# cg-saarland/hagrid

Measured on AMD Instinct MI355X. Metric: Mrays/s (primary traversal) + grid build ms, 1M-tri scene @1/2/4/8 MI355X, higher is better.
Workload: dtype f32

## Files before the change

hagrid_amd/csrc/build.hip:

```cpp
#include "ctx.h"
#include "wave_prims.h"

#include "hagrid/grid.h"
#include "hagrid/prims.h"

#include <cstring>
#include <vector>

using namespace hagrid;
using namespace hagrid_impl;

namespace {

struct BuildK {
    ivec3 dims;
    int shift;
    vec3 bmin, bmax;
    vec3 cell_size;
};

__device__ __forceinline__ Tri load_tri(const float4* __restrict__ tris, int i) {
    const float4* p = tris + 3 * size_t(i);
    const float4 a = p[0], b = p[1], c = p[2];
    return Tri(vec3(a.x, a.y, a.z), a.w, vec3(b.x, b.y, b.z), b.w, vec3(c.x, c.y, c.z), c.w);
}
__device__ __forceinline__ void store_cell(Cell* cells, int i, ivec3 lo, int begin, ivec3 hi, int end) {
    int4* p = reinterpret_cast<int4*>(cells) + 2 * size_t(i);
    p[0] = make_int4(lo.x, lo.y, lo.z, begin);
    p[1] = make_int4(hi.x, hi.y, hi.z, end);
}
__device__ __forceinline__ ivec3 load_cell_min(const Cell* cells, int i) {
    const int4 a = reinterpret_cast<const int4*>(cells)[2 * size_t(i)];
    return ivec3(a.x, a.y, a.z);
}
__device__ __forceinline__ BBox cell_world_box(const BuildK& k, ivec3 lo, ivec3 hi) {
    return BBox(k.bmin + vec3(lo) * k.cell_size, k.bmin + vec3(hi) * k.cell_size);
}

__global__ void __launch_bounds__(kBlock) bbox_partials(const float4* __restrict__ tris, int n, float* __restrict__ partials) {
    __shared__ float lds[kWaves][6];
    float lo[3] = { FLT_MAX, FLT_MAX, FLT_MAX }, hi[3] = { -FLT_MAX, -FLT_MAX, -FLT_MAX };
    for (int i = blockIdx.x * kBlock + threadIdx.x; i < n; i += gridDim.x * kBlock) {
        const BBox b = load_tri(tris, i).bbox();
        lo[0] = min(lo[0], b.min.x); lo[1] = min(lo[1], b.min.y); lo[2] = min(lo[2], b.min.z);
        hi[0] = max(hi[0], b.max.x); hi[1] = max(hi[1], b.max.y); hi[2] = max(hi[2], b.max.z);
    }
#pragma unroll
    for (int c = 0; c < 3; c++) { lo[c] = wave_min_f(lo[c]); hi[c] = wave_max_f(hi[c]); }
    if (lane_id() == 0) for (int c = 0; c < 3; c++) { lds[wave_id()][c] = lo[c]; lds[wave_id()][3 + c] = hi[c]; }
    __syncthreads();
    if (threadIdx.x < 6) {
        float v = lds[0][threadIdx.x];
        for (int w = 1; w < kWaves; w++) v = threadIdx.x < 3 ? min(v, lds[w][threadIdx.x]) : max(v, lds[w][threadIdx.x]);
        partials[blockIdx.x * 6 + threadIdx.x] = v;
    }
}
__global__ void __launch_bounds__(kBlock) bbox_final(const float* __restrict__ partials, int num, float* __restrict__ out) {
    __shared__ float lds[kWaves][6];
    float v[6] = { FLT_MAX, FLT_MAX, FLT_MAX, -FLT_MAX, -FLT_MAX, -FLT_MAX };
    for (int i = threadIdx.x; i < num; i += kBlock)
        for (int c = 0; c < 6; c++) v[c] = c < 3 ? min(v[c], partials[i * 6 + c]) : max(v[c], partials[i * 6 + c]);
#pragma unroll
    for (int c = 0; c < 6; c++) v[c] = c < 3 ? wave_min_f(v[c]) : wave_max_f(v[c]);
    if (lane_id() == 0) for (int c = 0; c < 6; c++) lds[wave_id()][c] = v[c];
    __syncthreads();
    if (threadIdx.x < 6) {
        float r = lds[0][threadIdx.x];
        for (int w = 1; w < kWaves; w++) r = threadIdx.x < 3 ? min(r, lds[w][threadIdx.x]) : max(r, lds[w][threadIdx.x]);
        out[threadIdx.x] = r;
    }
}

constexpr int kCoopCells = 64;


__global__ void __launch_bounds__(kBlock) top_log_dims(const int* __restrict__ refs_per_cell, int num_top, BuildK k, float snd_density,
                                                       int* __restrict__ log_dims, int* __restrict__ max_out) {
    __shared__ int lds[kWaves];
    const int i = blockIdx.x * kBlock + threadIdx.x;
    int ld = 0;
    if (i < num_top) {
        const vec3 ext = BBox(k.bmin, k.bmax).extents() / vec3(k.dims);
        const ivec3 d = compute_grid_dims(BBox(vec3(0, 0, 0), ext), refs_per_cell[i], snd_density);
        const int max_dim = max(d.x, max(d.y, d.z));
        ld = 31 - __clz(max_dim);
        ld = (1 << ld) < max_dim ? ld + 1 : ld;
        log_dims[i] = ld;
    }
    ld = wave_max(ld);
    if (lane_id() == 0) lds[wave_id()] = ld;
    __syncthreads();
    if (threadIdx.x == 0) {
        int m = lds[0];
        for (int w = 1; w < kWaves; w++) m = max(m, lds[w]);
        if (m > 0) atomicMax(max_out, m);
    }
}


__device__ __forceinline__ BuildK with_device_shift(BuildK k, const int* __restrict__ shift_dev, vec3 extents) {
    k.shift = *shift_dev;
    k.cell_size = extents / vec3(k.dims << k.shift);
    return k;
}

struct ChildCountIn {
    const uint32_t* entries;
    __device__ int operator()(int i) const { return (entries[i] & 3u) ? 8 : 0; }
    __device__ void load4(int i, int n, int* v) const {
        if (i + 4 <= n && lb_aligned16(entries + i)) {
            const uint4 e = *reinterpret_cast<const uint4*>(entries + i);
            v[0] = (e.x & 3u) ? 8 : 0; v[1] = (e.y & 3u) ? 8 : 0; v[2] = (e.z & 3u) ? 8 : 0; v[3] = (e.w & 3u) ? 8 : 0;
        } else {
            for (int c = 0; c < 4; c++) v[c] = i + c < n ? (*this)(i + c) : 0;
        }
    }
};
struct UpdateEntriesOut {
    uint32_t* entries;
    __device__ static uint32_t word(uint32_t e, int i, int start) { const uint32_t ld = e & 3u; return ld | (uint32_t(ld ? start : i) << 2); }
    __device__ void operator()(int i, int start) const { entries[i] = word(entries[i], i, start); }
    __device__ void store4(int i, int n, const int* v) const {
        if (i + 4 <= n && lb_aligned16(entries + i)) {
            uint4* p = reinterpret_cast<uint4*>(entries + i);
            const uint4 e = *p;
            *p = make_uint4(word(e.x, i, v[0]), word(e.y, i + 1, v[1]), word(e.z, i + 2, v[2]), word(e.w, i + 3, v[3]));
        } else {
            for (int c = 0; c < 4; c++) if (i + c < n) (*this)(i + c, v[c]);
        }
    }
};

__device__ __forceinline__ int split_mask(const BuildK& k, ivec3 lo, ivec3 hi, const Tri& tri) {
    const vec3 cmin = k.bmin + k.cell_size * vec3(lo);
    const vec3 cmax = k.bmin + k.cell_size * vec3(hi);
    const vec3 mid = (cmin + cmax) * 0.5f;
    int mask = 0xFF;
    const BBox rb = tri.bbox();
    if (rb.min.x > cmax.x || rb.max.x < cmin.x) mask = 0;
    if (rb.min.x > mid.x) mask &= 0xAA;
    if (rb.max.x < mid.x) mask &= 0x55;
    if (rb.min.y > cmax.y || rb.max.y < cmin.y) mask = 0;
    if (rb.min.y > mid.y) mask &= 0xCC;
    if (rb.max.y < mid.y) mask &= 0x33;
    if (rb.min.z > cmax.z || rb.max.z < cmin.z) mask = 0;
    if (rb.min.z > mid.z) mask &= 0xF0;
    if (rb.max.z < mid.z) mask &= 0x0F;
    int todo = mask;
    while (todo) {
        const int i = __ffs(todo) - 1;
        todo &= todo - 1;
        const BBox b(vec3(i & 1 ? mid.x : cmin.x, i & 2 ? mid.y : cmin.y, i & 4 ? mid.z : cmin.z),
                     vec3(i & 1 ? cmax.x : mid.x, i & 2 ? cmax.y : mid.y, i & 4 ? cmax.z : mid.z));
        if (!intersect_prim_cell(tri, b)) mask &= ~(1 << i);
    }
    return mask;
}


struct LeafIn {
    const uint32_t* entries; const int* cell_counts;
    __device__ static Int2 item(uint32_t e, int count) { const bool leaf = (e & 3u) == 0; return Int2{ leaf ? 1 : 0, leaf ? count : 0 }; }
    __device__ Int2 operator()(int i) const { return item(entries[i], cell_counts[i]); }
    __device__ void load4(int i, int n, Int2* v) const {
        if (i + 4 <= n && lb_aligned16(entries + i) && lb_aligned16(cell_counts + i)) {
            const uint4 e = *reinterpret_cast<const uint4*>(entries + i);
            const int4 c = *reinterpret_cast<const int4*>(cell_counts + i);
            v[0] = item(e.x, c.x); v[1] = item(e.y, c.y); v[2] = item(e.z, c.z); v[3] = item(e.w, c.w);
        } else {
            for (int k = 0; k < 4; k++) v[k] = i + k < n ? (*this)(i + k) : Int2{0, 0};
        }
    }
};
struct LeafOut {
    int* start_cell; int* ref_begin;
    __device__ void operator()(int i, Int2 v) const { start_cell[i] = v.a; ref_begin[i] = v.b; }
    __device__ void store4(int i, int n, const Int2* v) const {
        if (i + 4 <= n && lb_aligned16(start_cell + i) && lb_aligned16(ref_begin + i)) {
            *reinterpret_cast<int4*>(start_cell + i) = make_int4(v[0].a, v[1].a, v[2].a, v[3].a);
            *reinterpret_cast<int4*>(ref_begin + i) = make_int4(v[0].b, v[1].b, v[2].b, v[3].b);
        } else {
            for (int k = 0; k < 4; k++) if (i + k < n) (*this)(i + k, v[k]);
        }
    }
};


#ifndef HG_TILE_REFS
#define HG_TILE_REFS 1024
#endif
#ifndef HG_CHUNK_CELLS
#define HG_CHUNK_CELLS 256
#endif
#ifndef HG_EMIT_CHUNK
#define HG_EMIT_CHUNK 256
#endif
#ifndef HG_STAGE
#define HG_STAGE 1024
#endif
constexpr int kTileRefs = HG_TILE_REFS;
constexpr int kChunkCells = HG_CHUNK_CELLS;
constexpr int kEmitChunk = HG_EMIT_CHUNK;
constexpr int kStage = HG_STAGE;

__device__ __forceinline__ void mark_tiles(int* __restrict__ tile_first, int i, int start, int count) {
    for (int t = start / kTileRefs + 1; t <= (start + count) / kTileRefs; t++) tile_first[t] = i + 1;
}
struct SegIn {
    const int* counts;
    __device__ int operator()(int i) const { return counts[i]; }
};
struct SegOut {
    const int* counts; int* seg_begin; int* tile_first;
    Cell* cells; uint32_t* entries; int* cell_counts; const int* log_dims; const int* shift_dev; ivec3 dims;
    __device__ void operator()(int i, int start) const {
        seg_begin[i] = start; mark_tiles(tile_first, i, start, counts[i]);
        const int shift = *shift_dev;
        entries[i] = 0u; cell_counts[i] = 0;
        const int x = i % dims.x, y = (i / dims.x) % dims.y, z = i / (dims.x * dims.y);
        const ivec3 lo(x << shift, y << shift, z << shift);
        store_cell(cells, i, lo, log_dims[i], lo + ivec3(1 << shift), 0);
    }
};
struct ChildSegIn {
    const int* counts; const uint32_t* entries;
    __device__ Int2 operator()(int i) const { return Int2{counts[i], (entries[i] & 3u) ? 8 : 0}; }
    __device__ void load4(int i, int n, Int2* v) const {
        if (i + 4 <= n && lb_aligned16(counts + i) && lb_aligned16(entries + i)) {
            const int4 c = *reinterpret_cast<const int4*>(counts + i);
            const uint4 e = *reinterpret_cast<const uint4*>(entries + i);
            v[0] = Int2{c.x, (e.x & 3u) ? 8 : 0}; v[1] = Int2{c.y, (e.y & 3u) ? 8 : 0}; v[2] = Int2{c.z, (e.z & 3u) ? 8 : 0}; v[3] = Int2{c.w, (e.w & 3u) ? 8 : 0};
        } else {
            for (int k = 0; k < 4; k++) v[k] = i + k < n ? (*this)(i + k) : Int2{0, 0};
        }
    }
};
struct ChildSegOut {
    const int* counts; uint32_t* entries; int* seg_begin; int* tile_first;
    __device__ void operator()(int i, Int2 v) const {
        seg_begin[i] = v.a;
        entries[i] = UpdateEntriesOut::word(entries[i], i, v.b);
        mark_tiles(tile_first, i, v.a, counts[i]);
    }
    __device__ void store4(int i, int n, const Int2* v) const {
        if (i + 4 <= n && lb_aligned16(counts + i) && lb_aligned16(entries + i) && lb_aligned16(seg_begin + i)) {
            const int4 c = *reinterpret_cast<const int4*>(counts + i);
            uint4* pe = reinterpret_cast<uint4*>(entries + i);
            const uint4 e = *pe;
            *reinterpret_cast<int4*>(seg_begin + i) = make_int4(v[0].a, v[1].a, v[2].a, v[3].a);
            *pe = make_uint4(UpdateEntriesOut::word(e.x, i, v[0].b), UpdateEntriesOut::word(e.y, i + 1, v[1].b), UpdateEntriesOut::word(e.z, i + 2, v[2].b), UpdateEntriesOut::word(e.w, i + 3, v[3].b));
            if (v[0].a / kTileRefs != (v[3].a + c.w) / kTileRefs) {
                mark_tiles(tile_first, i, v[0].a, c.x); mark_tiles(tile_first, i + 1, v[1].a, c.y); mark_tiles(tile_first, i + 2, v[2].a, c.z); mark_tiles(tile_first, i + 3, v[3].a, c.w);
            }
        } else {
            for (int k = 0; k < 4; k++) if (i + k < n) (*this)(i + k, v[k]);
        }
    }
};

__global__ void __launch_bounds__(kBlock) top_range_sizes(const float4* __restrict__ tris, int n, BuildK k, int* __restrict__ counts, int* __restrict__ big_list, int* __restrict__ big_count) {
    const int i = blockIdx.x * kBlock + threadIdx.x;
    int size = 0;
    if (i < n) { size = max(0, compute_range(k.dims, BBox(k.bmin, k.bmax), load_tri(tris, i).bbox()).size()); counts[i] = size; }
    const bool big = size >= kCoopCells;
    const int at = wave_append(big ? 1 : 0, big_count);
    if (big) big_list[at] = i;
}
__device__ __forceinline__ int wave_shared_increment(int* __restrict__ counters, int index, bool active) {
    int rank = 0;
    unsigned long long todo = __ballot(active);
    const unsigned long long below = (1ull << lane_id()) - 1ull;
    for (int round = 0; todo && round < 16; round++) {
        const int leader = __ffsll((long long)todo) - 1;
        const int c = __shfl(index, leader, 64);
        const unsigned long long same = __ballot(active && index == c) & todo;
        if (round == 0 && (same & (same - 1)) == 0ull) break;
        int base = 0;
        if (lane_id() == leader) base = atomicAdd(counters + c, __popcll(same));
        base = __shfl(base, leader, 64);
        if ((same >> lane_id()) & 1ull) rank = base + __popcll(same & below);
        todo &= ~same;
    }
    if ((todo >> lane_id()) & 1ull) rank = atomicAdd(counters + index, 1);
    return rank;
}

__global__ void __launch_bounds__(kBlock) count_top_refs(const float4* __restrict__ tris, int n, BuildK k, const int* __restrict__ start_emit,
                                                                int* __restrict__ refs_per_cell, int* __restrict__ pair_rank,
                                                                const int* __restrict__ big_list, const int* __restrict__ big_count, int first_big_block) {
    if (int(blockIdx.x) >= first_big_block) {
        const int nb = *big_count;
        for (int b = int(blockIdx.x) - first_big_block; b < nb; b += int(gridDim.x) - first_big_block) {
            const int prim = big_list[b];
            const Range r = compute_range(k.dims, BBox(k.bmin, k.bmax), load_tri(tris, prim).bbox());
            const int total = r.size(), first = start_emit[prim], sx = r.hx - r.lx + 1, sy = r.hy - r.ly + 1;
            for (int c = threadIdx.x; c < total; c += kBlock) {
                const int x = r.lx + c % sx, y = r.ly + (c / sx) % sy, z = r.lz + c / (sx * sy);
                pair_rank[first + c] = atomicAdd(refs_per_cell + (x + k.dims.x * (y + k.dims.y * z)), 1);
            }
        }
        return;
    }
    const int i = blockIdx.x * kBlock + threadIdx.x;
    Range r(0, 0, 0, -1, -1, -1);
    int size = 0, start = 0;
    if (i < n) {
        r = compute_range(k.dims, BBox(k.bmin, k.bmax), load_tri(tris, i).bbox());
        size = max(0, r.size());
        start = start_emit[i];
    }
    const bool coop = size >= kCoopCells;
    {
        const bool mine = size > 0 && !coop;
        const int c0 = mine ? r.lx + k.dims.x * (r.ly + k.dims.y * r.lz) : -1 - lane_id();
        const unsigned long long any = __ballot(mine);
        const bool crowd = any != 0ull && __popcll(__ballot(c0 == __shfl(c0, __ffsll((long long)any) - 1, 64))) >= 2;
        if (!crowd) {
            if (mine) {
                int cur = start;
                for (int z = r.lz; z <= r.hz; z++)
                    for (int y = r.ly; y <= r.hy; y++)
                        for (int x = r.lx; x <= r.hx; x++) pair_rank[cur++] = atomicAdd(refs_per_cell + (x + k.dims.x * (y + k.dims.y * z)), 1);
            }
        } else {
            const int rounds = wave_max(mine ? size : 0);
            int x = r.lx, y = r.ly, z = r.lz;
            for (int j = 0; j < rounds; j++) {
                const bool act = mine && j < size;
                const int rank = wave_shared_increment(refs_per_cell, act ? x + k.dims.x * (y + k.dims.y * z) : 0, act);
                if (act) pair_rank[start + j] = rank;
                if (++x > r.hx) { x = r.lx; if (++y > r.hy) { y = r.ly; z++; } }
            }
        }
    }
}
__device__ __forceinline__ void place_top_ref(const BuildK& k, const Tri& tri, int prim, int x, int y, int z, int rank, const int* __restrict__ seg_begin,
                                              int2* __restrict__ refs, const int* __restrict__ log_dims, uint32_t* __restrict__ entries) {
    const int inc = 1 << k.shift;
    const ivec3 lo(x << k.shift, y << k.shift, z << k.shift);
    const bool hit = intersect_prim_cell(tri, cell_world_box(k, lo, lo + ivec3(inc)));
    const int cell = x + k.dims.x * (y + k.dims.y * z);
    refs[seg_begin[cell] + rank] = make_int2(hit ? prim : -1, cell);
    if (hit && log_dims[cell] > 0) entries[cell] = 1u;
}
__global__ void __launch_bounds__(kBlock) emit_top_refs(const float4* __restrict__ tris, int n, BuildK k0, const int* __restrict__ shift_dev, vec3 extents,
                                                                const int* __restrict__ start_emit,
                                                                const int* __restrict__ pair_rank, const int* __restrict__ seg_begin, int2* __restrict__ refs,
                                                                const int* __restrict__ log_dims, uint32_t* __restrict__ entries,
                                                                const int* __restrict__ big_list, const int* __restrict__ big_count, int first_big_block) {
    const BuildK k = with_device_shift(k0, shift_dev, extents);
    if (int(blockIdx.x) >= first_big_block) {
        const int nb = *big_count;
        for (int b = int(blockIdx.x) - first_big_block; b < nb; b += int(gridDim.x) - first_big_block) {
            const int prim = big_list[b];
            const Tri t = load_tri(tris, prim);
            const Range r = compute_range(k.dims, BBox(k.bmin, k.bmax), t.bbox());
            const int total = r.size(), first = start_emit[prim], sx = r.hx - r.lx + 1, sy = r.hy - r.ly + 1;
            for (int c = threadIdx.x; c < total; c += kBlock)
                place_top_ref(k, t, prim, r.lx + c % sx, r.ly + (c / sx) % sy, r.lz + c / (sx * sy), pair_rank[first + c], seg_begin, refs, log_dims, entries);
        }
        return;
    }
    const int i = blockIdx.x * kBlock + threadIdx.x;
    Range r(0, 0, 0, -1, -1, -1);
    int size = 0, start = 0;
    Tri tri;
    if (i < n) {
        tri = load_tri(tris, i);
        r = compute_range(k.dims, BBox(k.bmin, k.bmax), tri.bbox());
        size = max(0, r.size());
        start = start_emit[i];
    }
    const bool coop = size >= kCoopCells;
    if (size > 0 && !coop) {
        int cur = start;
        for (int z = r.lz; z <= r.hz; z++)
            for (int y = r.ly; y <= r.hy; y++)
                for (int x = r.lx; x <= r.hx; x++) { place_top_ref(k, tri, i, x, y, z, pair_rank[cur], seg_begin, refs, log_dims, entries); cur++; }
    }
}

struct TileRange { int c0, c1; };
__device__ __forceinline__ TileRange tile_cells(const int* __restrict__ tile_first, int t, int num_tiles, int num_cells) {
    return TileRange{ t == 0 ? 0 : tile_first[t], t + 1 >= num_tiles ? num_cells : tile_first[t + 1] };
}
struct LaneRun { unsigned long long run; int first; bool head; };
__device__ __forceinline__ LaneRun lane_run(int cell) {
    const int l = lane_id();
    const int prev = __shfl_up(cell, 1, 64);
    LaneRun r;
    r.head = l == 0 || prev != cell;
    const unsigned long long heads = __ballot(r.head);
    const unsigned long long upto = heads & (~0ull >> (63 - l));
    r.first = 63 - __clzll((long long)upto);
    const unsigned long long above = l == 63 ? 0ull : heads >> (l + 1);
    const int next = above ? l + 1 + (__ffsll((long long)above) - 1) : 64;
    const unsigned long long below_next = next == 64 ? ~0ull : ((1ull << next) - 1ull);
    r.run = below_next & ~((1ull << r.first) - 1ull);
    return r;
}

#ifndef HG_CLASSIFY_WAVES
#define HG_CLASSIFY_WAVES 8
#endif
__global__ void __launch_bounds__(kBlock, HG_CLASSIFY_WAVES) classify_refs(const int2* __restrict__ refs, const int* __restrict__ seg_begin,
                                                           int num_cells, int num_refs, const int* __restrict__ tile_first, int num_tiles, int top,
                                                           const float4* __restrict__ tris, const Cell* __restrict__ cells, const uint32_t* __restrict__ entries, BuildK k,
                                                           unsigned char* __restrict__ masks, int* __restrict__ cell_counts,
                                                           Cell* __restrict__ new_cells, int* __restrict__ new_counts, uint32_t* __restrict__ new_entries, int* __restrict__ totals) {
    __shared__ int hist[kChunkCells * 9];
    __shared__ int lds[kWaves];
    int kept = 0;
    for (int t = xcd_block(blockIdx.x, gridDim.x); t < num_tiles; t += gridDim.x) {
        const TileRange tr = tile_cells(tile_first, t, num_tiles, num_cells);
        for (int cc = tr.c0; cc < tr.c1; cc += kChunkCells) {
            const int ce = min(cc + kChunkCells, tr.c1);
            const int r0 = seg_begin[cc], r1 = ce >= num_cells ? num_refs : seg_begin[ce];
            if (r0 == r1) continue;
            for (int j = threadIdx.x; j < (ce - cc) * 9; j += kBlock) hist[j] = 0;
            __syncthreads();
            for (int base = r0 + wave_id() * 64; base < r1; base += kBlock) {
                const int i = base + lane_id();
                int2 rc = make_int2(-1, 0x7fffffff);
                if (i < r1) rc = refs[i];
                const int ref = rc.x, c = rc.y;
                int m = 0;
                bool keeps = false;
                if (ref >= 0) {
                    const uint32_t e = entries[c];
                    if ((e & 3u) == 0) keeps = true;
                    else {
                        const int4* p = reinterpret_cast<const int4*>(cells) + 2 * size_t(c);
                        const int4 a = p[0], b = p[1];
                        m = split_mask(k, ivec3(a.x, a.y, a.z), ivec3(b.x, b.y, b.z), load_tri(tris, ref));
                    }
                }
                if (i < r1) masks[i] = (unsigned char)m;
                kept += keeps ? 1 : 0;
                const LaneRun run = lane_run(c);
                int* h = hist + (c - cc) * 9;
                const unsigned long long any = __ballot(m != 0);
                if (any) {
#pragma unroll
                    for (int child = 0; child < 8; child++) {
                        const unsigned long long with = __ballot((m >> child) & 1);
                        if (run.head && i < r1) { const int n = __popcll(with & run.run); if (n) atomicAdd(h + child, n); }
                    }
                }
                if (top) {
                    const unsigned long long with = __ballot(keeps);
                    if (run.head && i < r1) { const int n = __popcll(with & run.run); if (n) atomicAdd(h + 8, n); }
                }
            }
            __syncthreads();
            for (int j = threadIdx.x; j < (ce - cc) * 8; j += kBlock) {
                const int c = cc + (j >> 3), child = j & 7;
                const uint32_t e = entries[c];
                if (e & 3u) {
                    const int n = hist[(j >> 3) * 9 + child];
                    const int4* p = reinterpret_cast<const int4*>(cells) + 2 * size_t(c);
                    const int4 a = p[0], b = p[1];
                    const int inc = (b.x - a.x) >> 1;
                    const ivec3 lo(a.x + (child & 1) * inc, a.y + ((child >> 1) & 1) * inc, a.z + (child >> 2) * inc);
                    store_cell(new_cells, int(e >> 2) + child, lo, a.w - 1, lo + ivec3(inc), 0);
                    new_counts[(e >> 2) + child] = n;
                    new_entries[(e >> 2) + child] = (n > 0 && a.w > 1) ? 1u : 0u;
                } else if (top && child == 0) cell_counts[c] = hist[(j >> 3) * 9 + 8];
            }
            __syncthreads();
        }
    }
    kept = block_sum(kept, lds);
    if (threadIdx.x == 0 && kept) atomicAdd(totals, kept);
}

__global__ void __launch_bounds__(kBlock) emit_child_refs(const int2* __restrict__ refs, const int* __restrict__ seg_begin,
                                                                  int num_cells, int num_refs, const int* __restrict__ tile_first, int num_tiles,
                                                                  const unsigned char* __restrict__ masks, const uint32_t* __restrict__ entries,
                                                                  const int* __restrict__ new_seg_begin, int2* __restrict__ new_refs) {
    __shared__ int cursor[kEmitChunk * 8];
    __shared__ int2 stage[kStage];
    __shared__ int region[2];
    for (int t = blockIdx.x; t < num_tiles; t += gridDim.x) {
        const TileRange tr = tile_cells(tile_first, t, num_tiles, num_cells);
        for (int cc = tr.c0; cc < tr.c1; cc += kEmitChunk) {
            const int ce = min(cc + kEmitChunk, tr.c1);
            const int r0 = seg_begin[cc], r1 = ce >= num_cells ? num_refs : seg_begin[ce];
            if (r0 == r1) continue;
            if (threadIdx.x == 0) { region[0] = 0x7fffffff; region[1] = 0; }
            __syncthreads();
            int lo = 0x7fffffff;
            for (int j = threadIdx.x; j < (ce - cc) * 8; j += kBlock) {
                const uint32_t e = entries[cc + (j >> 3)];
                const int at = (e & 3u) ? new_seg_begin[(e >> 2) + (j & 7)] : 0x7fffffff;
                cursor[j] = at;
                lo = min(lo, at);
            }
            lo = -wave_max(-lo);
            if (lane_id() == 0 && lo != 0x7fffffff) atomicMin(&region[0], lo);
            __syncthreads();
            const int base = region[0];
            int hi = 0;
            for (int rb = r0 + wave_id() * 64; rb < r1; rb += kBlock) {
                const int i = rb + lane_id();
                int m = 0;
                int2 rc = make_int2(-1, 0x7fffffff);
                if (i < r1) { m = masks[i]; rc = refs[i]; }
                if (__ballot(m != 0) == 0ull) continue;
                const int c = rc.y;
                const int first_child = m ? int(entries[c] >> 2) : 0;
                const LaneRun run = lane_run(c);
                int* cur = cursor + (c - cc) * 8;
                const unsigned long long below = (1ull << lane_id()) - 1ull;
#pragma unroll
                for (int child = 0; child < 8; child++) {
                    const unsigned long long with = __ballot((m >> child) & 1);
                    if (!with) continue;
                    int at = 0;
                    if (run.head && i < r1) { const int n = __popcll(with & run.run); if (n) at = atomicAdd(cur + child, n); }
                    at = __shfl(at, run.first, 64);
                    if ((m >> child) & 1) {
                        const int slot = at + __popcll(with & run.run & below);
                        hi = max(hi, slot + 1);
                        const int2 v = make_int2(rc.x, first_child + child);
                        if (slot - base < kStage) stage[slot - base] = v;
                        else new_refs[slot] = v;
                    }
                }
            }
            hi = wave_max(hi);
            if (lane_id() == 0 && hi) atomicMax(&region[1], hi);
            __syncthreads();
            const int staged = min(region[1] - base, kStage);
            for (int q = threadIdx.x; q < staged; q += kBlock) new_refs[base + q] = stage[q];
            __syncthreads();
        }
    }
}

constexpr int kCoopListMin = 9, kCoopListMax = 1024;
__global__ void __launch_bounds__(kBlock) concat_level(const uint32_t* __restrict__ entries, const Cell* __restrict__ cells, const int* __restrict__ cell_counts,
                                                               const int* __restrict__ start_cell, const int* __restrict__ ref_begin, int num_cells, int level_off,
                                                               const int2* __restrict__ refs, const int* __restrict__ seg_begin, int num_refs, int top,
                                                               Cell* __restrict__ out_cells, uint32_t* __restrict__ out_entries, int* __restrict__ out_refs) {
    __shared__ int long_cells[kBlock];
    __shared__ int num_long;
    __shared__ int stage[kWaves][kCoopListMax];
    if (threadIdx.x == 0) num_long = 0;
    __syncthreads();
    const int i = blockIdx.x * kBlock + threadIdx.x;
    if (i < num_cells) {
        const uint32_t e = entries[i];
        if (e & 3u) out_entries[level_off + i] = (e & 3u) | (((e >> 2) + uint32_t(level_off + num_cells)) << 2);
        else {
            const int dst = start_cell[i], cnt = cell_counts[i], rb = ref_begin[i];
            const int4* p = reinterpret_cast<const int4*>(cells) + 2 * size_t(i);
            const int4 a = p[0], b = p[1];
            store_cell(out_cells, dst, ivec3(a.x, a.y, a.z), cnt ? rb : 0, ivec3(b.x, b.y, b.z), cnt ? rb + cnt : 0);
            out_entries[level_off + i] = uint32_t(dst) << 2;
            int* r = out_refs + rb;
            const int2* src = refs + seg_begin[i];
            if (cnt == 0) { }
            else if (!top && cnt <= 4) {
                const int big = 0x7fffffff;
                int v0 = src[0].x, v1 = cnt > 1 ? src[1].x : big, v2 = cnt > 2 ? src[2].x : big, v3 = cnt > 3 ? src[3].x : big;
                int t;
                if (v0 > v1) { t = v0; v0 = v1; v1 = t; }
                if (v2 > v3) { t = v2; v2 = v3; v3 = t; }
                if (v0 > v2) { t = v0; v0 = v2; v2 = t; }
                if (v1 > v3) { t = v1; v1 = v3; v3 = t; }
                if (v1 > v2) { t = v1; v1 = v2; v2 = t; }
                r[0] = v0;
                if (cnt > 1) r[1] = v1;
                if (cnt > 2) r[2] = v2;
                if (cnt > 3) r[3] = v3;
            } else if (cnt >= kCoopListMin && cnt <= kCoopListMax) {
                long_cells[atomicAdd(&num_long, 1)] = i;
            } else {
                int n = 0;
                if (top) { for (int j = 0; n < cnt; j++) { const int v = src[j].x; if (v >= 0) r[n++] = v; } }
                else for (; n < cnt; n++) r[n] = src[n].x;
                if (cnt > 24) {
                    const int gaps[8] = { 1750, 701, 301, 132, 57, 23, 10, 4 };
                    for (int g = 0; g < 8; g++) {
                        const int gap = gaps[g];
                        for (int x = gap; x < cnt; x++) {
                            const int v = r[x];
                            int y = x - gap;
                            while (y >= 0 && r[y] > v) { r[y + gap] = r[y]; y -= gap; }
                            r[y + gap] = v;
                        }
                    }
                }
                for (int x = 1; x < cnt; x++) {
                    const int v = r[x];
                    int y = x - 1;
                    while (y >= 0 && r[y] > v) { r[y + 1] = r[y]; y--; }
                    r[y + 1] = v;
                }
            }
        }
    }
    __syncthreads();
    const int nl = num_long, lane = lane_id();
    int* buf = stage[wave_id()];
    for (int q = wave_id(); q < nl; q += kWaves) {
        const int c = long_cells[q];
        const int cnt = cell_counts[c];
        int* r = out_refs + ref_begin[c];
        const int2* src = refs + seg_begin[c];
        if (top) {
            int found = 0;
            for (int base = 0; found < cnt; base += 64) {
                const int v = seg_begin[c] + base + lane < num_refs ? src[base + lane].x : -1;
                const unsigned long long ok = __ballot(v >= 0);
                const int at = found + __popcll(ok & ((1ull << lane) - 1ull));
                if (v >= 0 && at < cnt) buf[at] = v;
                found += __popcll(ok);
            }
        } else {
            for (int x = lane; x < cnt; x += 64) buf[x] = src[x].x;
        }
        __builtin_amdgcn_wave_barrier();
        for (int x = lane; x < cnt; x += 64) {
            const int v = buf[x];
            int rank = 0;
            for (int y = 0; y < cnt; y++) rank += buf[y] < v ? 1 : 0;
            r[rank] = v;
        }
        __builtin_amdgcn_wave_barrier();
    }
}

struct PlainIn { const int* v; __device__ int operator()(int i) const { return v[i]; } };
struct PlainOut { int* v; __device__ void operator()(int i, int s) const { v[i] = s; } };

using Temps = PoolTemps;

struct GLevel {
    int2* refs = nullptr; int num_refs = 0;
    Cell* cells = nullptr; uint32_t* entries = nullptr; int num_cells = 0;
    int* cell_counts = nullptr;
    int* seg_begin = nullptr;
    int* tile_first = nullptr; int num_tiles = 0;
    int* start_cell = nullptr; int* ref_begin = nullptr;
};

struct Arena {
    hagrid_ctx* ctx; Temps& tmp; char* base = nullptr; size_t size = 0, used = 0, wanted = 0; int num_tris;
    Arena(hagrid_ctx* c, Temps& t, int n_tris) : ctx(c), tmp(t), num_tris(n_tris) {
        size_t want = c->build_arena_hint;
        if (want && c->build_arena_tris > 0 && 2ll * n_tris < c->build_arena_tris)
            want = size_t(double(want) * 1.25 * double(std::max(n_tris, 1)) / double(c->build_arena_tris)) + 4096;
        if (want) {
            base = pool_try_alloc<char>(c, want);
            if (base) { t.ptrs.push_back(base); size = want; }
        }
    }
    ~Arena() { ctx->build_arena_hint = wanted; ctx->build_arena_tris = num_tris; }
    template <typename T> T* get(size_t n) {
        const size_t bytes = (std::max(n, size_t(1)) * sizeof(T) + 255) & ~size_t(255);
        wanted += bytes;
        if (base && used + bytes <= size) { T* p = reinterpret_cast<T*>(base + used); used += bytes; return p; }
        return tmp.get<T>(n);
    }
    void drop(void* p) { if (!base || p < base || p >= base + size) tmp.drop(p); }
};

int build_levels(hagrid_ctx* ctx, const float4* tris, int num_tris, hagrid_grid* grid, BuildK k, const BBox& gb, float snd_density, Temps& tmp) {
    hipStream_t st = ctx->stream;
    int* dsc = ctx->dscratch;
    Arena ar(ctx, tmp, num_tris);
    const ivec3 dims = k.dims;
    const int num_top = dims.x * dims.y * dims.z;

    int* counts = ar.get<int>(size_t(num_tris));
    int* start_emit = ar.get<int>(size_t(num_tris));
    int* refs_per_cell = ar.get<int>(size_t(num_top));
    int* log_dims = ar.get<int>(size_t(num_top));
    int* const partials = nullptr;
    if (!counts || !start_emit || !refs_per_cell || !log_dims) return HAGRID_ENOMEM;
    HG_HIP(ctx, hipMemsetAsync(refs_per_cell, 0, size_t(num_top) * sizeof(int), st));
    int* big_list = ar.get<int>(size_t(num_tris));
    if (!big_list) return HAGRID_ENOMEM;
    top_range_sizes<<<grid_blocks(num_tris, kBlock), kBlock, 0, st>>>(tris, num_tris, k, counts, big_list, dsc + 2); HG_DBG(ctx);
    if (!ctx_scan<int>(ctx, PlainIn{counts}, PlainOut{start_emit}, num_tris, partials, (const int*)nullptr, dsc + 0)) return HAGRID_ENOMEM;
    int R0 = 0, num_big = 0;
    {
        int h[3];
        HG_TRY(read_back(ctx, dsc, h, sizeof(h)));
        R0 = h[0]; num_big = h[2];
    }
    if (R0 < 0 || R0 > 0x3fffffff) HG_FAIL(ctx, HAGRID_ERANGE, "build_grid: too many top-level references");
    ar.drop(counts);
    int* pair_rank = ar.get<int>(size_t(R0) + 1);
    if (!pair_rank) return HAGRID_ENOMEM;
    const int prim_blocks = grid_blocks(num_tris, kBlock), big_blocks = std::min(num_big, 2048);
    count_top_refs<<<prim_blocks + big_blocks, kBlock, 0, st>>>(tris, num_tris, k, start_emit, refs_per_cell, pair_rank, big_list, dsc + 2, prim_blocks); HG_DBG(ctx);
    top_log_dims<<<grid_blocks(num_top, kBlock), kBlock, 0, st>>>(refs_per_cell, num_top, k, snd_density, log_dims, dsc + 1); HG_DBG(ctx);

    std::vector<GLevel> levels;
    GLevel L;
    L.num_refs = R0; L.num_cells = num_top;
    L.num_tiles = grid_blocks(R0, kTileRefs);
    L.refs = ar.get<int2>(size_t(R0) + 1);
    L.cells = ar.get<Cell>(size_t(num_top)); L.entries = ar.get<uint32_t>(size_t(num_top) + 1);
    L.cell_counts = ar.get<int>(size_t(num_top)); L.seg_begin = ar.get<int>(size_t(num_top) + 1);
    L.tile_first = ar.get<int>(size_t(L.num_tiles) + 2);
    L.start_cell = ar.get<int>(size_t(num_top)); L.ref_begin = ar.get<int>(size_t(num_top));
    if (!L.refs || !L.cells || !L.entries || !L.cell_counts || !L.seg_begin || !L.tile_first || !L.start_cell || !L.ref_begin) return HAGRID_ENOMEM;
    if (!ctx_scan<int>(ctx, SegIn{refs_per_cell}, SegOut{refs_per_cell, L.seg_begin, L.tile_first, L.cells, L.entries, L.cell_counts, log_dims, dsc + 1, dims}, num_top, partials,
                       (const int*)nullptr, (int*)nullptr)) return HAGRID_ENOMEM;
    hagrid_build_counts& bc = ctx->counts;
    memset(&bc, 0, sizeof(bc));
    bc.num_tris = num_tris; bc.top_cells = num_top; bc.top_refs = R0;
    emit_top_refs<<<prim_blocks + big_blocks, kBlock, 0, st>>>(tris, num_tris, k, dsc + 1, gb.extents(), start_emit, pair_rank, L.seg_begin, L.refs, log_dims, L.entries, big_list, dsc + 2, prim_blocks); HG_DBG(ctx);
    levels.push_back(L);

    {
        if (!ctx_scan<int>(ctx, ChildCountIn{L.entries}, UpdateEntriesOut{L.entries}, num_top, (int*)nullptr, (const int*)nullptr, dsc + 8)) return HAGRID_ENOMEM;
    }
    int num_new_cells = 0, shift = 0;
    {
        int h[8];
        HG_TRY(read_back(ctx, dsc + 1, h, sizeof(h)));
        shift = h[0]; num_new_cells = h[7];
    }
    if (shift >= 24) HG_FAIL(ctx, HAGRID_ERANGE, "build_grid: too many levels");
    k.shift = shift;
    k.cell_size = gb.extents() / vec3(dims << shift);
    ar.drop(start_emit); ar.drop(pair_rank); ar.drop(refs_per_cell);
    for (int level = 0;; level++) {
        GLevel& P = levels.back();
        int* tot = dsc + 8 + 4 * level;
        if (num_new_cells < 0) HG_FAIL(ctx, HAGRID_ERANGE, "build_grid: level too large");
        if ((int)levels.size() >= 24) HG_FAIL(ctx, HAGRID_ERANGE, "build_grid: too many levels");
        const bool last = num_new_cells == 0;
        if (last && level > 0) {
            if (level < HAGRID_MAX_LEVELS) { bc.level_refs[level] = P.num_refs; bc.level_cells[level] = P.num_cells; bc.level_kept[level] = P.num_refs; bc.num_levels = level + 1; }
            break;
        }
        GLevel N;
        N.num_cells = num_new_cells;
        unsigned char* masks = ar.get<unsigned char>(size_t(P.num_refs) + 1);
        if (!masks) return HAGRID_ENOMEM;
        if (!last) {
            N.cells = ar.get<Cell>(size_t(num_new_cells)); N.entries = ar.get<uint32_t>(size_t(num_new_cells) + 1);
            N.cell_counts = ar.get<int>(size_t(num_new_cells)); N.seg_begin = ar.get<int>(size_t(num_new_cells) + 1);
            N.tile_first = ar.get<int>(size_t(grid_blocks(8ll * P.num_refs, kTileRefs)) + 2);
            N.start_cell = ar.get<int>(size_t(num_new_cells)); N.ref_begin = ar.get<int>(size_t(num_new_cells));
            if (!N.cells || !N.entries || !N.cell_counts || !N.seg_begin || !N.tile_first || !N.start_cell || !N.ref_begin) return HAGRID_ENOMEM;
        }
        if (P.num_refs > 0) {
            classify_refs<<<std::min(P.num_tiles, 4096), kBlock, 0, st>>>(P.refs, P.seg_begin, P.num_cells, P.num_refs, P.tile_first, P.num_tiles, level == 0 ? 1 : 0,
                                                                             tris, P.cells, P.entries, k, masks, P.cell_counts, N.cells, N.cell_counts, N.entries, tot + 1); HG_DBG(ctx);
        }
        Int2* next = reinterpret_cast<Int2*>(tot + 2);
        if (!last) {
            if (!ctx_scan<Int2>(ctx, ChildSegIn{N.cell_counts, N.entries}, ChildSegOut{N.cell_counts, N.entries, N.seg_begin, N.tile_first}, num_new_cells, (Int2*)nullptr,
                                (const Int2*)nullptr, next)) return HAGRID_ENOMEM;
        }
        int h3[3] = {0, 0, 0};
        HG_TRY(read_back(ctx, tot + 1, h3, sizeof(h3)));
        if (level < HAGRID_MAX_LEVELS) { bc.level_refs[level] = P.num_refs; bc.level_cells[level] = P.num_cells; bc.level_kept[level] = h3[0]; bc.num_levels = level + 1; }
        if (last) { ar.drop(masks); break; }
        const int num_children = h3[1];
        if (num_children < 0 || num_children > 0x3fffffff) HG_FAIL(ctx, HAGRID_ERANGE, "build_grid: level too large");
        N.num_refs = num_children; N.num_tiles = grid_blocks(num_children, kTileRefs);
        N.refs = ar.get<int2>(size_t(num_children) + 1);
        if (!N.refs) return HAGRID_ENOMEM;
        if (P.num_refs > 0 && num_children > 0) {
            emit_child_refs<<<std::min(P.num_tiles, 4096), kBlock, 0, st>>>(P.refs, P.seg_begin, P.num_cells, P.num_refs, P.tile_first, P.num_tiles,
                                                                                   masks, P.entries, N.seg_begin, N.refs); HG_DBG(ctx);
        }
        ar.drop(masks);
        num_new_cells = h3[2];
        levels.push_back(N);
    }
    ar.drop(log_dims);

    const int num_levels = (int)levels.size();
    long long total_cells_ll = 0;
    int max_cells = 0;
    for (auto& V : levels) { total_cells_ll += V.num_cells; max_cells = std::max(max_cells, V.num_cells); }
    if (total_cells_ll > 0x3fffffff) HG_FAIL(ctx, HAGRID_ERANGE, "build_grid: too many voxel map entries");
    const int total_cells = int(total_cells_ll);
    Int2* const part2 = nullptr;
    Int2* carry = reinterpret_cast<Int2*>(dsc + 128);
    for (int l = 0; l < num_levels; l++) {
        GLevel& V = levels[l];
        if (!ctx_scan<Int2>(ctx, LeafIn{V.entries, V.cell_counts}, LeafOut{V.start_cell, V.ref_begin}, V.num_cells, part2,
                            l ? carry + (l - 1) : (const Int2*)nullptr, carry + l)) return HAGRID_ENOMEM;
    }
    int hf[2];
    HG_TRY(read_back(ctx, carry + (num_levels - 1), hf, sizeof(hf)));
    const int new_total_cells = hf[0], total_refs = hf[1];
    if (new_total_cells <= 0 || total_refs < 0) HG_FAIL(ctx, HAGRID_ERANGE, "build_grid: inconsistent totals");

    Cell* out_cells = pool_alloc<Cell>(ctx, size_t(new_total_cells));
    uint32_t* out_entries = pool_alloc<uint32_t>(ctx, size_t(total_cells));
    int* out_refs = pool_alloc<int>(ctx, size_t(total_refs));
    if (!out_cells || !out_entries || !out_refs) {
        hagrid_mem_free(ctx, out_cells); hagrid_mem_free(ctx, out_entries); hagrid_mem_free(ctx, out_refs);
        return HAGRID_ENOMEM;
    }
    for (int l = 0, off = 0; l < num_levels; off += levels[l].num_cells, l++) {
        GLevel& V = levels[l];
        concat_level<<<grid_blocks(V.num_cells, kBlock), kBlock, 0, st>>>(V.entries, V.cells, V.cell_counts, V.start_cell, V.ref_begin, V.num_cells, off,
                                                                                  V.refs, V.seg_begin, V.num_refs, l == 0 ? 1 : 0, out_cells, out_entries, out_refs); HG_DBG(ctx);
    }
    hipError_t e = hipGetLastError();
    if (e == hipSuccess) e = hipStreamSynchronize(st);
    if (e != hipSuccess) {
        hagrid_mem_free(ctx, out_cells); hagrid_mem_free(ctx, out_entries); hagrid_mem_free(ctx, out_refs);
        HG_FAIL(ctx, HAGRID_EHIP, hipGetErrorString(e));
    }
    memset(grid, 0, sizeof(*grid));
    grid->entries = out_entries; grid->ref_ids = out_refs; grid->cells = out_cells; grid->small_cells = nullptr;
    grid->bbox_min[0] = gb.min.x; grid->bbox_min[1] = gb.min.y; grid->bbox_min[2] = gb.min.z;
    grid->bbox_max[0] = gb.max.x; grid->bbox_max[1] = gb.max.y; grid->bbox_max[2] = gb.max.z;
    grid->dims[0] = dims.x; grid->dims[1] = dims.y; grid->dims[2] = dims.z;
    grid->num_cells = new_total_cells; grid->num_entries = total_cells; grid->num_refs = total_refs;
    bc.build_cells = new_total_cells; bc.build_entries = total_cells; bc.build_refs = total_refs;
    grid->shift = shift;
    grid->num_offsets = shift + 1;
    for (int i = 0, off = 0; i <= shift; i++) {
        if (i < num_levels) off += levels[i].num_cells;
        grid->offsets[i] = off;
    }
    return HAGRID_OK;
}

}

extern "C" int hagrid_build_grid(hagrid_ctx* ctx, const void* tris_v, int num_tris, hagrid_grid* grid,
                                 float top_density, float snd_density) {
    if (!ctx || !grid) return HAGRID_EINVAL;
    trav_image_drop(ctx);
    if (!tris_v || num_tris <= 0) HG_FAIL(ctx, HAGRID_EINVAL, "build_grid: no triangles");
    HG_HIP(ctx, hipSetDevice(ctx->device));
    const float4* tris = static_cast<const float4*>(tris_v);
    hipStream_t st = ctx->stream;
    Temps tmp(ctx);
    int* dsc = ctx->dscratch;
    HG_HIP(ctx, hipMemsetAsync(dsc, 0, 256 * sizeof(int), st));

    const int bb_blocks = std::min(grid_blocks(num_tris, kBlock), 1024);
    float* bb_part = tmp.get<float>(size_t(bb_blocks) * 6 + 8);
    if (!bb_part) return HAGRID_ENOMEM;
    float* bb_out = bb_part + size_t(bb_blocks) * 6;
    bbox_partials<<<bb_blocks, kBlock, 0, st>>>(tris, num_tris, bb_part); HG_DBG(ctx);
    bbox_final<<<1, kBlock, 0, st>>>(bb_part, bb_blocks, bb_out); HG_DBG(ctx);
    float hb[6];
    HG_TRY(read_back(ctx, bb_out, hb, sizeof(hb)));
    BBox gb(vec3(hb[0], hb[1], hb[2]), vec3(hb[3], hb[4], hb[5]));
    ivec3 dims = compute_grid_dims(gb, num_tris, top_density);
    dims.x += dims.x & 1; dims.y += dims.y & 1; dims.z += dims.z & 1;
    const vec3 ext = gb.extents();
    gb.min -= ext * 0.001f;
    gb.max += ext * 0.001f;
    const long long num_top_ll = (long long)dims.x * dims.y * dims.z;
    if (num_top_ll > 0x3fffffff) HG_FAIL(ctx, HAGRID_ERANGE, "build_grid: top-level grid too large");

    BuildK k;
    k.dims = dims; k.shift = 0; k.bmin = gb.min; k.bmax = gb.max; k.cell_size = vec3(0.0f);

    return build_levels(ctx, tris, num_tris, grid, k, gb, snd_density, tmp);
}
```

hagrid_amd/csrc/ctx.h:

```cpp
#pragma once

#include <hip/hip_runtime.h>

#include <atomic>
#include <cstdio>
#include <memory>
#include <string>
#include <unordered_map>
#include <vector>

#include "hagrid_amd.h"

namespace hagrid_impl {

struct Slot {
    void* ptr = nullptr;
    size_t size = 0;
    bool in_use = false;
    int refs = 0;
};

}

namespace hagrid_impl {

struct TravImageCache {
    void* table = nullptr;
    size_t table_bytes = 0;
    int wide_records = 0;
    void* blocks = nullptr;
    size_t block_bytes = 0;
    bool valid = false;
    bool uniform = false;
    bool general = false;
    int slim = 0;
    int vtop_k = 0;
    uint32_t vtop_base = 0;
    bool detached = false;
    bool borrowed = false;
    std::shared_ptr<std::atomic<bool>> alive;
    const void* entries = nullptr; const void* cells = nullptr; const void* refs = nullptr;
    int num_cells = 0, num_entries = 0, num_refs = 0, shift = 0, dims[3] = {0, 0, 0}, cell_bytes = 32;
    int max_ref = -1;
    void* alt_blocks = nullptr; void* alt_table = nullptr; size_t alt_block_bytes = 0, alt_table_bytes = 0; int alt_wide_records = 0, alt_slim = 0;
};

}

namespace hagrid_impl {
enum MailboxWord : int {
    kMbxRowLen = 300,
    kMbxOrderStale = 304,
    kMbxReadBackEpoch = 310,
    kMbxHeadSuggest = 312,
    kMbxPriorStats = 316,
};
enum ScratchWord : int {
    kScrRowLenBinned = 232,
    kScrRowLen = 236,
    kScrMaxRef = 240,
    kScrBlobFlag = 250,
};
}

struct hagrid_ctx {
    int device = 0;
    hipStream_t stream = nullptr;
    bool keep = false;
    int num_cus = 0;

    std::vector<hagrid_impl::Slot> slots;
    std::unordered_map<void*, int> tracker;
    size_t usage = 0, max_usage = 0;

    hipEvent_t ev_begin = nullptr, ev_end = nullptr;

    int* mailbox = nullptr;
    int* dscratch = nullptr;
    unsigned long long* lb_state = nullptr;
    size_t lb_words = 0;
    unsigned lb_epoch = 0;
    int* row_scores = nullptr;
    int* bin_diff = nullptr;

    int ray_binning = 0;
    int opt_variant = 0;
    int opt_lookback = 1;
    int opt_merge_inplace = 1;
    int opt_merge_inplace_iters = 0;
    int opt_merge_inplace_div = 0;
    int opt_merge_inplace_room = 0;
    int opt_merge_narrow = 1;
    int opt_expand_voxel_map = 1;
    int opt_expand_subset_only = 1;
    int opt_image_width = 0;
    int opt_band_rows = 0;
    int opt_super_log2 = 3;
    int opt_xcd_chunk_log2 = -2;
    int opt_narrow = 1;
    int opt_image_max_mb = 0;
    int opt_quad_head = 20;
    int opt_image_vtop = 1;
    int opt_image_uniform = 1;
    int opt_row_cache = 1;
    struct RayHints {
        const void* key_rays = nullptr; int key_n = 0;
        const void* rowlen_rays = nullptr; int rowlen_n = 0, rowlen_age = 0, rowlen_known = -1, rowlen_seen = 0; bool rows_from_origins = false ;
        hipEvent_t rowlen_evt = nullptr; bool rowlen_pending = false;
        int* lpt_buf = nullptr; int lpt_cap = 0; const void* lpt_rays = nullptr; int lpt_n = 0, lpt_blocks = 0, lpt_age = 0, lpt_period = 32, lpt_rot = 0 ; bool rot_adopted = false ;
        hipEvent_t trial_evt[2] = {nullptr, nullptr}; bool trial_pending = false, trial_with_head = false, head_disabled = false;
        float t_base = 0.0f, t_head = 0.0f; int n_base = 0, n_head = 0, trial_opt = -1 ; unsigned head_serial = 0 ; bool lpt_valid = false;
        int lpt_epoch = 1 , relearn_streak = 0, cooldown = 0, cooldown_len = 64; unsigned long long relearn_clock = 0;
        hipEvent_t share_evt[12][2] = {}; int share_issued = 0, share_done = 0, share_choice = -1 , share_ncand = 0 , share_shape_nc = 0 , share_cands[4] = {0, 0, 0, 0} ,
            share_last = -1 , share_launches = 0; float share_t[4] = {0.0f, 0.0f, 0.0f, 0.0f}; unsigned share_serial = 0 ;
        int trial_kind = 0 , n_all = 0, all_stage = 0 ; float t_all = 0.0f; bool learned_all = false;
        bool learned_once = false;
        unsigned order_serial = 0;
        bool cmp_pending = false, cmp_done = false; int n_conf = 0; float t_conf = 0.0f;
        bool order_loses = false;
        int last_report = -1;
        unsigned long long used = 0;
    };
    static constexpr int kRayHints = 4;
    RayHints hints[kRayHints];
    unsigned long long hint_clock = 0;
    int opt_mailbox = -1;
    int opt_tail = 1;
    int opt_lds_pad = 0;
    int opt_tail_dual = -1;
    int opt_share_trial = 1;
    int opt_order_gate = 1;
    int opt_tile_order = -1;
    int opt_quad_tail = -1;
    int opt_image_slim = 1;
    int opt_image_general = 1;
    int opt_image = 2;

    int opt_id_is_steps = 0;

    hagrid_impl::TravImageCache image;
    unsigned image_serial = 0;
    int readback_epoch = 0;
    int opt_fast_readback = 1;
    int build_arena_tris = 0;
    size_t build_arena_hint = 0;
    hagrid_build_counts counts = {};

    std::string err;
};

namespace hagrid_impl {

inline int fail(hagrid_ctx* ctx, int code, const char* file, int line, const char* msg) {
    if (ctx) {
        char buf[512];
        snprintf(buf, sizeof(buf), "%s(%d): %s", file, line, msg);
        ctx->err = buf;
    }
    return code;
}

#define HG_FAIL(ctx, code, msg) return ::hagrid_impl::fail((ctx), (code), __FILE__, __LINE__, (msg))
#define HG_HIP(ctx, call)                                                                         \
    do {                                                                                          \
        hipError_t e_ = (call);                                                                   \
        if (e_ != hipSuccess) return ::hagrid_impl::fail((ctx), HAGRID_EHIP, __FILE__, __LINE__, hipGetErrorString(e_)); \
    } while (0)
#define HG_TRY(expr)                                                                              \
    do {                                                                                          \
        int rc_ = (expr);                                                                         \
        if (rc_ < 0) return rc_;                                                                  \
    } while (0)

void debug_sync(hagrid_ctx* ctx, const char* file, int line);
#ifdef HAGRID_DEBUG_SYNC
#define HG_DBG(ctx) ::hagrid_impl::debug_sync((ctx), __FILE__, __LINE__)
#else
#define HG_DBG(ctx) do { } while (0)
#endif

template <typename T>
inline T* pool_alloc(hagrid_ctx* ctx, size_t n) {
    return static_cast<T*>(hagrid_mem_alloc(ctx, (n ? n : 1) * sizeof(T)));
}

template <typename T>
inline T* pool_try_alloc(hagrid_ctx* ctx, size_t n) {
    const std::string saved = ctx->err;
    T* p = pool_alloc<T>(ctx, n);
    if (!p) { (void)hipGetLastError(); ctx->err = saved; }
    return p;
}

struct PoolTemps {
    hagrid_ctx* ctx;
    std::vector<void*> ptrs;
    explicit PoolTemps(hagrid_ctx* c) : ctx(c) {}
    PoolTemps(const PoolTemps&) = delete;
    PoolTemps& operator=(const PoolTemps&) = delete;
    template <typename T> T* get(size_t n) { T* p = pool_alloc<T>(ctx, n); if (p) ptrs.push_back(p); return p; }
    void drop(void* p) { for (auto& q : ptrs) if (q == p && p) { hagrid_mem_free(ctx, p); q = nullptr; } }
    void* keep(void* p) { for (auto& q : ptrs) if (q == p) q = nullptr; return p; }
    ~PoolTemps() { for (void* p : ptrs) if (p) hagrid_mem_free(ctx, p); }
};

int pool_split(hagrid_ctx* ctx, void* base, void* const* parts, int n);

int read_back(hagrid_ctx* ctx, const void* dptr, void* hptr, size_t bytes);

inline int grid_blocks(long long n, int block) { return (int)((n + block - 1) / block); }

unsigned long long* lookback_state(hagrid_ctx* ctx, int tiles, int words_per_tile, unsigned* epoch);

int trav_image_build(hagrid_ctx* ctx, const hagrid_grid* grid);
void trav_image_drop(hagrid_ctx* ctx);
bool trav_image_matches(const hagrid_ctx* ctx, const hagrid_grid* grid);
bool trav_image_stale(const hagrid_ctx* ctx);
void trav_image_source_touched(hagrid_ctx* ctx, const void* ptr, size_t bytes);

}
```

hagrid_amd/csrc/ctx.hip:

```cpp
#include "ctx.h"

#include <chrono>

#include <algorithm>
#include <cstring>
#include <iostream>

using namespace hagrid_impl;

extern "C" int hagrid_abi_version(void) { return HAGRID_ABI_VERSION; }

extern "C" int hagrid_ctx_create(hagrid_ctx** out, int device, int keep) {
    if (!out) return HAGRID_EINVAL;
    *out = nullptr;
    int count = 0;
    if (hipGetDeviceCount(&count) != hipSuccess || count <= 0 || device < 0 || device >= count) return HAGRID_ENODEV;
    hagrid_ctx* ctx = new hagrid_ctx();
    ctx->device = device;
    ctx->keep = keep != 0;
    if (hipSetDevice(device) != hipSuccess) { delete ctx; return HAGRID_ENODEV; }
    hipDeviceProp_t prop;
    if (hipGetDeviceProperties(&prop, device) != hipSuccess) { delete ctx; return HAGRID_ENODEV; }
    ctx->num_cus = prop.multiProcessorCount;
    if (hipEventCreate(&ctx->ev_begin) != hipSuccess || hipEventCreate(&ctx->ev_end) != hipSuccess ||
        hipHostMalloc((void**)&ctx->mailbox, 320 * sizeof(int), hipHostMallocDefault) != hipSuccess ||
        hipMalloc((void**)&ctx->dscratch, 256 * sizeof(int)) != hipSuccess) {
        hagrid_ctx_destroy(ctx);
        return HAGRID_EHIP;
    }
    memset(ctx->mailbox, 0, 320 * sizeof(int));
    *out = ctx;
    return HAGRID_OK;
}

extern "C" void hagrid_ctx_destroy(hagrid_ctx* ctx) {
    if (!ctx) return;
    (void)hipSetDevice(ctx->device);
    (void)hipStreamSynchronize(ctx->stream);
    for (auto& h : ctx->hints) h.rowlen_pending = false;
    if (!ctx->image.borrowed && ctx->image.alive) ctx->image.alive->store(false);
    for (auto& s : ctx->slots)
        if (s.ptr) (void)hipFree(s.ptr);
    if (ctx->ev_begin) (void)hipEventDestroy(ctx->ev_begin);
    if (ctx->ev_end) (void)hipEventDestroy(ctx->ev_end);
    for (auto& h : ctx->hints) { if (h.rowlen_evt) (void)hipEventDestroy(h.rowlen_evt); if (h.lpt_buf) (void)hipFree(h.lpt_buf); for (auto& e : h.trial_evt) if (e) (void)hipEventDestroy(e); for (auto& pr : h.share_evt) for (auto& e : pr) if (e) (void)hipEventDestroy(e); }
    if (ctx->mailbox) (void)hipHostFree(ctx->mailbox);
    if (ctx->dscratch) (void)hipFree(ctx->dscratch);
    if (ctx->bin_diff) (void)hipFree(ctx->bin_diff);
    if (ctx->row_scores) (void)hipFree(ctx->row_scores);
    if (ctx->lb_state) (void)hipFree(ctx->lb_state);
    delete ctx;
}

extern "C" int hagrid_ctx_set_stream(hagrid_ctx* ctx, void* stream) {
    if (!ctx) return HAGRID_EINVAL;
    hipStream_t next = static_cast<hipStream_t>(stream);
    if (next == ctx->stream) return HAGRID_OK;
    HG_HIP(ctx, hipSetDevice(ctx->device));
    HG_HIP(ctx, hipStreamSynchronize(ctx->stream));
    ctx->stream = next;
    return HAGRID_OK;
}

extern "C" int hagrid_ctx_synchronize(hagrid_ctx* ctx) {
    if (!ctx) return HAGRID_EINVAL;
    HG_HIP(ctx, hipSetDevice(ctx->device));
    HG_HIP(ctx, hipStreamSynchronize(ctx->stream));
    return HAGRID_OK;
}

extern "C" int hagrid_get_build_counts(const hagrid_ctx* ctx, hagrid_build_counts* out) {
    if (!ctx || !out) return HAGRID_EINVAL;
    *out = ctx->counts;
    return HAGRID_OK;
}

extern "C" const char* hagrid_last_error(const hagrid_ctx* ctx) { return ctx ? ctx->err.c_str() : "no context"; }

extern "C" int hagrid_device_info(const hagrid_ctx* ctx, char* name, int name_len, int* compute_units, int64_t* total_mem) {
    if (!ctx) return HAGRID_EINVAL;
    hipDeviceProp_t prop;
    if (hipGetDeviceProperties(&prop, ctx->device) != hipSuccess) return HAGRID_EHIP;
    if (name && name_len > 0) { strncpy(name, prop.gcnArchName, (size_t)name_len - 1); name[name_len - 1] = 0; }
    if (compute_units) *compute_units = prop.multiProcessorCount;
    if (total_mem) *total_mem = (int64_t)prop.totalGlobalMem;
    return HAGRID_OK;
}


static void release_slot_memory(hagrid_ctx* ctx, Slot& s) {
    if (s.ptr) (void)hipFree(s.ptr);
    ctx->usage -= s.size;
    s.ptr = nullptr;
    s.size = 0;
}

extern "C" void* hagrid_mem_alloc(hagrid_ctx* ctx, size_t bytes) {
    if (!ctx) return nullptr;
    if (bytes == 0) bytes = 4;
    bytes = (bytes + 255) & ~size_t(255);
    int fit = -1, biggest = -1, empty = -1;
    for (int i = 0, n = (int)ctx->slots.size(); i < n; i++) {
        const Slot& s = ctx->slots[i];
        if (s.in_use) continue;
        if (!s.ptr) { if (empty < 0) empty = i; continue; }
        if (s.size >= bytes && (fit < 0 || s.size < ctx->slots[fit].size)) fit = i;
        if (biggest < 0 || s.size > ctx->slots[biggest].size) biggest = i;
    }
    int idx = fit;
    if (idx >= 0 && ctx->slots[idx].size > 4 * bytes && ctx->slots[idx].size > (size_t(64) << 20)) idx = -1;
    if (idx < 0) {
        idx = fit < 0 ? (biggest >= 0 && ctx->keep ? biggest : empty) : empty;
        if (idx < 0) { idx = (int)ctx->slots.size(); ctx->slots.emplace_back(); }
        Slot& s = ctx->slots[idx];
        if (s.ptr) release_slot_memory(ctx, s);
        void* p = nullptr;
        (void)hipSetDevice(ctx->device);
        if (hipMalloc(&p, bytes) != hipSuccess) {
            for (auto& t : ctx->slots) if (!t.in_use && t.ptr) release_slot_memory(ctx, t);
            if (hipMalloc(&p, bytes) != hipSuccess) { fail(ctx, HAGRID_ENOMEM, __FILE__, __LINE__, "hipMalloc failed"); return nullptr; }
        }
        s.ptr = p; s.size = bytes;
        ctx->usage += bytes;
        ctx->max_usage = std::max(ctx->max_usage, ctx->usage);
    }
    Slot& s = ctx->slots[idx];
    s.in_use = true;
    s.refs = 1;
    ctx->tracker[s.ptr] = idx;
    return s.ptr;
}

int hagrid_impl::pool_split(hagrid_ctx* ctx, void* base, void* const* parts, int n) {
    auto it = ctx->tracker.find(base);
    if (it == ctx->tracker.end() || n <= 0) HG_FAIL(ctx, HAGRID_EINVAL, "pool_split: not a pool buffer");
    const int idx = it->second;
    Slot& s = ctx->slots[idx];
    if (s.refs != 1 || s.ptr != base) HG_FAIL(ctx, HAGRID_EINVAL, "pool_split: buffer is already split");
    for (int i = 0; i < n; i++) {
        const char* p = static_cast<const char*>(parts[i]);
        if (p < static_cast<const char*>(base) || p >= static_cast<const char*>(base) + s.size) HG_FAIL(ctx, HAGRID_EINVAL, "pool_split: part outside the buffer");
        for (int j = 0; j < i; j++) if (parts[j] == parts[i]) HG_FAIL(ctx, HAGRID_EINVAL, "pool_split: parts coincide");
    }
    ctx->tracker.erase(it);
    for (int i = 0; i < n; i++) ctx->tracker[parts[i]] = idx;
    s.refs = n;
    return HAGRID_OK;
}

extern "C" int hagrid_mem_free(hagrid_ctx* ctx, void* ptr) {
    if (!ctx) return HAGRID_EINVAL;
    if (!ptr) return HAGRID_OK;
    auto it = ctx->tracker.find(ptr);
    if (it == ctx->tracker.end()) HG_FAIL(ctx, HAGRID_EINVAL, "free of a pointer that does not come from this MemManager");
    trav_image_source_touched(ctx, ptr, 1);
    it = ctx->tracker.find(ptr);
    Slot& s = ctx->slots[it->second];
    ctx->tracker.erase(it);
    if (--s.refs > 0) return HAGRID_OK;
    s.in_use = false;
    if (!ctx->keep) {
        HG_HIP(ctx, hipStreamSynchronize(ctx->stream));
        release_slot_memory(ctx, s);
    }
    return HAGRID_OK;
}

extern "C" int hagrid_mem_copy_h2d(hagrid_ctx* ctx, void* dst, const void* src, size_t bytes) {
    if (!ctx) return HAGRID_EINVAL;
    if (!bytes) return HAGRID_OK;
    trav_image_source_touched(ctx, dst, bytes);
    HG_HIP(ctx, hipSetDevice(ctx->device));
    HG_HIP(ctx, hipMemcpyAsync(dst, src, bytes, hipMemcpyHostToDevice, ctx->stream));
    HG_HIP(ctx, hipStreamSynchronize(ctx->stream));
    return HAGRID_OK;
}
extern "C" int hagrid_mem_copy_d2h(hagrid_ctx* ctx, void* dst, const void* src, size_t bytes) {
    if (!ctx) return HAGRID_EINVAL;
    if (!bytes) return HAGRID_OK;
    HG_HIP(ctx, hipSetDevice(ctx->device));
    HG_HIP(ctx, hipMemcpyAsync(dst, src, bytes, hipMemcpyDeviceToHost, ctx->stream));
    HG_HIP(ctx, hipStreamSynchronize(ctx->stream));
    return HAGRID_OK;
}
extern "C" int hagrid_mem_copy_d2d(hagrid_ctx* ctx, void* dst, const void* src, size_t bytes) {
    if (!ctx) return HAGRID_EINVAL;
    if (!bytes) return HAGRID_OK;
    trav_image_source_touched(ctx, dst, bytes);
    HG_HIP(ctx, hipSetDevice(ctx->device));
    HG_HIP(ctx, hipMemcpyAsync(dst, src, bytes, hipMemcpyDeviceToDevice, ctx->stream));
    return HAGRID_OK;
}
extern "C" int hagrid_mem_zero(hagrid_ctx* ctx, void* ptr, size_t bytes) {
    if (!ctx) return HAGRID_EINVAL;
    if (!bytes) return HAGRID_OK;
    trav_image_source_touched(ctx, ptr, bytes);
    HG_HIP(ctx, hipSetDevice(ctx->device));
    HG_HIP(ctx, hipMemsetAsync(ptr, 0, bytes, ctx->stream));
    return HAGRID_OK;
}
extern "C" int hagrid_mem_one(hagrid_ctx* ctx, void* ptr, size_t bytes) {
    if (!ctx) return HAGRID_EINVAL;
    if (!bytes) return HAGRID_OK;
    trav_image_source_touched(ctx, ptr, bytes);
    HG_HIP(ctx, hipSetDevice(ctx->device));
    HG_HIP(ctx, hipMemsetAsync(ptr, 0xFF, bytes, ctx->stream));
    return HAGRID_OK;
}
extern "C" size_t hagrid_mem_usage(const hagrid_ctx* ctx) { return ctx ? ctx->usage : 0; }
extern "C" size_t hagrid_mem_max_usage(const hagrid_ctx* ctx) { return ctx ? ctx->max_usage : 0; }

extern "C" void hagrid_mem_debug_slots(const hagrid_ctx* ctx) {
    if (!ctx) return;
    size_t total = 0;
    std::cout << "SLOTS: " << std::endl;
    for (const auto& s : ctx->slots) {
        std::cout << "[" << (s.in_use ? 'X' : ' ') << "] " << (double)s.size / (1024.0 * 1024.0) << "MB" << std::endl;
        total += s.size;
    }
    std::cout << (double)total / (1024.0 * 1024.0) << "MB total" << std::endl;
}


extern "C" int hagrid_profile_begin(hagrid_ctx* ctx) {
    if (!ctx) return HAGRID_EINVAL;
    HG_HIP(ctx, hipSetDevice(ctx->device));
    HG_HIP(ctx, hipEventRecord(ctx->ev_begin, ctx->stream));
    return HAGRID_OK;
}
extern "C" float hagrid_profile_end(hagrid_ctx* ctx) {
    if (!ctx) return -1.0f;
    float ms = -1.0f;
    if (hipEventRecord(ctx->ev_end, ctx->stream) != hipSuccess) return -1.0f;
    if (hipEventSynchronize(ctx->ev_end) != hipSuccess) return -1.0f;
    if (hipEventElapsedTime(&ms, ctx->ev_begin, ctx->ev_end) != hipSuccess) return -1.0f;
    return ms;
}

namespace {
typedef float f32x4_t __attribute__((ext_vector_type(4)));
__global__ void __launch_bounds__(256) bw_copy_kernel(const f32x4_t* __restrict__ a, f32x4_t* __restrict__ c, size_t n) {
    const size_t base = size_t(blockIdx.x) * 1024 + threadIdx.x;
    f32x4_t v[4];
#pragma unroll
    for (int j = 0; j < 4; j++) if (base + j * 256 < n) v[j] = __builtin_nontemporal_load(a + base + j * 256);
#pragma unroll
    for (int j = 0; j < 4; j++) if (base + j * 256 < n) __builtin_nontemporal_store(v[j], c + base + j * 256);
}
__global__ void __launch_bounds__(256) bw_triad_kernel(const f32x4_t* __restrict__ a, const f32x4_t* __restrict__ b, f32x4_t* __restrict__ c, size_t n) {
    const size_t base = size_t(blockIdx.x) * 1024 + threadIdx.x;
    f32x4_t v[4], w[4];
#pragma unroll
    for (int j = 0; j < 4; j++) if (base + j * 256 < n) { v[j] = __builtin_nontemporal_load(a + base + j * 256); w[j] = __builtin_nontemporal_load(b + base + j * 256); }
#pragma unroll
    for (int j = 0; j < 4; j++) if (base + j * 256 < n) __builtin_nontemporal_store(v[j] + 3.0f * w[j], c + base + j * 256);
}
}

extern "C" int hagrid_bandwidth_probe(hagrid_ctx* ctx, size_t bytes, int iters, float* copy_gbps, float* triad_gbps) {
    if (!ctx || iters <= 0 || bytes < (size_t(1) << 20)) return HAGRID_EINVAL;
    HG_HIP(ctx, hipSetDevice(ctx->device));
    const size_t n = bytes / 16;
    f32x4_t* a = pool_alloc<f32x4_t>(ctx, n);
    f32x4_t* b = pool_alloc<f32x4_t>(ctx, n);
    f32x4_t* c = pool_alloc<f32x4_t>(ctx, n);
    int rc = HAGRID_OK;
    if (!a || !b || !c) rc = HAGRID_ENOMEM;
    if (rc == HAGRID_OK) {
        (void)hipMemsetAsync(a, 0, n * 16, ctx->stream); (void)hipMemsetAsync(b, 0, n * 16, ctx->stream);
        const int blocks = int((n + 1023) / 1024);
        float best_copy = 0.0f, best_triad = 0.0f;
        for (int it = 0; it < iters + 1 && rc == HAGRID_OK; it++) {
            float ms = -1.0f;
            if (hagrid_profile_begin(ctx) != HAGRID_OK) { rc = HAGRID_EHIP; break; }
            bw_copy_kernel<<<blocks, 256, 0, ctx->stream>>>(a, c, n); HG_DBG(ctx);
            ms = hagrid_profile_end(ctx);
            if (ms > 0.0f && it) best_copy = std::max(best_copy, float(2.0 * double(n) * 16.0 / (double(ms) * 1e6)));
            if (hagrid_profile_begin(ctx) != HAGRID_OK) { rc = HAGRID_EHIP; break; }
            bw_triad_kernel<<<blocks, 256, 0, ctx->stream>>>(a, b, c, n); HG_DBG(ctx);
            ms = hagrid_profile_end(ctx);
            if (ms > 0.0f && it) best_triad = std::max(best_triad, float(3.0 * double(n) * 16.0 / (double(ms) * 1e6)));
        }
        if (copy_gbps) *copy_gbps = best_copy;
        if (triad_gbps) *triad_gbps = best_triad;
        if (hipGetLastError() != hipSuccess) rc = HAGRID_EHIP;
    }
    hagrid_mem_free(ctx, a); hagrid_mem_free(ctx, b); hagrid_mem_free(ctx, c);
    return rc;
}

unsigned long long* hagrid_impl::lookback_state(hagrid_ctx* ctx, int tiles, int words_per_tile, unsigned* epoch) {
    const size_t need = size_t(tiles > 0 ? tiles : 1) * size_t(words_per_tile);
    if (need > ctx->lb_words || ctx->lb_epoch >= (1u << 30) - 2u) {
        (void)hipStreamSynchronize(ctx->stream);
        if (need > ctx->lb_words) {
            if (ctx->lb_state) (void)hipFree(ctx->lb_state);
            ctx->lb_state = nullptr; ctx->lb_words = 0;
            const size_t words = need + need / 2 + 1024;
            if (hipMalloc((void**)&ctx->lb_state, words * sizeof(unsigned long long)) != hipSuccess) { (void)hipGetLastError(); return nullptr; }
            ctx->lb_words = words;
        }
        (void)hipMemsetAsync(ctx->lb_state, 0, ctx->lb_words * sizeof(unsigned long long), ctx->stream);
        ctx->lb_epoch = 0;
    }
    *epoch = ++ctx->lb_epoch;
    return ctx->lb_state;
}

void hagrid_impl::debug_sync(hagrid_ctx* ctx, const char* file, int line) {
    hipError_t e = hipStreamSynchronize(ctx->stream);
    if (e == hipSuccess) e = hipGetLastError();
    if (e != hipSuccess) {
        fprintf(stderr, "%s(%d): %s\n", file, line, hipGetErrorString(e));
        abort();
    }
}

extern "C" int hagrid_debug_sync_enabled(void) {
#ifdef HAGRID_DEBUG_SYNC
    return 1;
#else
    return 0;
#endif
}

namespace {
__global__ void __launch_bounds__(256) publish_words(const int* __restrict__ src, int n, int* dst, int* flag, int epoch) {
    if (int(threadIdx.x) < n) dst[threadIdx.x] = src[threadIdx.x];
    __threadfence_system();
    __syncthreads();
    if (threadIdx.x == 0) __hip_atomic_store(flag, epoch, __ATOMIC_RELEASE, __HIP_MEMORY_SCOPE_SYSTEM);
}
}

int hagrid_impl::read_back(hagrid_ctx* ctx, const void* dptr, void* hptr, size_t bytes) {
    if (ctx->opt_fast_readback && bytes > 0 && bytes <= 256 * sizeof(int) && (bytes & 3u) == 0 && (reinterpret_cast<uintptr_t>(dptr) & 3u) == 0) {
        int* flag = ctx->mailbox + kMbxReadBackEpoch;
        const int epoch = ++ctx->readback_epoch;
        publish_words<<<1, 256, 0, ctx->stream>>>(static_cast<const int*>(dptr), int(bytes / 4), ctx->mailbox, flag, epoch);
        HG_HIP(ctx, hipGetLastError());
        const auto t0 = std::chrono::steady_clock::now();
        for (unsigned spins = 0;; spins++) {
            if (__atomic_load_n(flag, __ATOMIC_ACQUIRE) == epoch) break;
            if ((spins & 1023u) == 1023u && std::chrono::steady_clock::now() - t0 > std::chrono::milliseconds(20)) {
                HG_HIP(ctx, hipStreamSynchronize(ctx->stream));
                if (__atomic_load_n(flag, __ATOMIC_ACQUIRE) != epoch) HG_FAIL(ctx, HAGRID_EHIP, "read_back: the words never arrived");
                break;
            }
        }
        memcpy(hptr, ctx->mailbox, bytes);
        return HAGRID_OK;
    }
    if (bytes <= 256 * sizeof(int)) {
        HG_HIP(ctx, hipMemcpyAsync(ctx->mailbox, dptr, bytes, hipMemcpyDeviceToHost, ctx->stream));
        HG_HIP(ctx, hipStreamSynchronize(ctx->stream));
        memcpy(hptr, ctx->mailbox, bytes);
    } else {
        HG_HIP(ctx, hipMemcpyAsync(hptr, dptr, bytes, hipMemcpyDeviceToHost, ctx->stream));
        HG_HIP(ctx, hipStreamSynchronize(ctx->stream));
    }
    return HAGRID_OK;
}
```

hagrid_amd/csrc/expand.hip:

```cpp
#include "ctx.h"
#include "wave_prims.h"

#include "hagrid/grid.h"
#include "hagrid/prims.h"

using namespace hagrid;
using namespace hagrid_impl;

namespace {

struct ExpandK { ivec3 dims; ivec3 top; int shift; vec3 gmin, cell_size, grid_inv; const int* voxel_cells; };
constexpr int kChanged = 1 << 3;
struct CellRec { ivec3 lo; int begin; ivec3 hi; int end; };

__device__ __forceinline__ CellRec load_cell(const Cell* cells, int i) {
    const int4* p = reinterpret_cast<const int4*>(cells) + 2 * size_t(i);
    const int4 a = p[0], b = p[1];
    CellRec c; c.lo = ivec3(a.x, a.y, a.z); c.begin = a.w; c.hi = ivec3(b.x, b.y, b.z); c.end = b.w;
    return c;
}
__device__ __forceinline__ int comp(const ivec3& v, int axis) { return axis == 0 ? v.x : (axis == 1 ? v.y : v.z); }


__device__ __forceinline__ int lower_bound_in(const int* __restrict__ a, int n, int x) {
    int lo = 0, hi = n;
    while (lo < hi) {
        const int mid = (lo + hi) >> 1;
        if (a[mid] < x) lo = mid + 1; else hi = mid;
    }
    return lo;
}

__device__ __forceinline__ bool contains_all(const int* __restrict__ big, int nbig, const int* __restrict__ small, int nsmall) {
    if (nsmall > nbig) return false;
    if (nsmall == 0) return true;
    if (nbig <= 4) {
        const int b0 = big[0], b1 = nbig > 1 ? big[1] : -1, b2 = nbig > 2 ? big[2] : -1, b3 = nbig > 3 ? big[3] : -1;
        const int s0 = small[0], s1 = nsmall > 1 ? small[1] : s0, s2 = nsmall > 2 ? small[2] : s0, s3 = nsmall > 3 ? small[3] : s0;
        auto in_big = [&](int x) { return (x == b0) | (x == b1) | (x == b2) | (x == b3); };
        return in_big(s0) & in_big(s1) & in_big(s2) & in_big(s3);
    }
    for (int j = 0; j < nsmall; j++) {
        const int x = small[j], at = lower_bound_in(big, nbig, x);
        if (at == nbig || big[at] != x) return false;
    }
    return true;
}

__device__ __forceinline__ Tri load_tri(const float4* __restrict__ tris, int i) {
    const float4* p = tris + 3 * size_t(i);
    const float4 a = p[0], b = p[1], c = p[2];
    return Tri(vec3(a.x, a.y, a.z), a.w, vec3(b.x, b.y, b.z), b.w, vec3(c.x, c.y, c.z), c.w);
}

__global__ void __launch_bounds__(kBlock) fill_voxel_cells(ExpandK k, const Entry* __restrict__ entries, int* __restrict__ voxel_cells, int voxels) {
    const int v = blockIdx.x * kBlock + threadIdx.x;
    if (v >= voxels) return;
    const int s = k.shift, m = (1 << s) - 1, top = v >> (3 * s), local = v & ((1 << (3 * s)) - 1);
    const int tx = top % k.top.x, ty = (top / k.top.x) % k.top.y, tz = top / (k.top.x * k.top.y);
    const ivec3 at((tx << s) + (local & m), (ty << s) + ((local >> s) & m), (tz << s) + (local >> (2 * s)));
    voxel_cells[v] = int(lookup_entry(entries, s, k.top, at));
}
__device__ __forceinline__ int cell_of_voxel(const ExpandK& k, const Entry* __restrict__ entries, const ivec3& at) {
    if (!k.voxel_cells) return int(lookup_entry(entries, k.shift, k.top, at));
    const int s = k.shift, m = (1 << s) - 1;
    const int top = (at.x >> s) + k.top.x * ((at.y >> s) + k.top.y * (at.z >> s));
    return k.voxel_cells[(top << (3 * s)) + (at.x & m) + (((at.y & m) + ((at.z & m) << s)) << s)];
}

template <int AXIS>
__device__ __forceinline__ int room_before_prim(const ExpandK& k, const Tri& prim, const CellRec& cell, const BBox& cross, int room, bool UP) {
    constexpr int A1 = (AXIS + 1) % 3, A2 = (AXIS + 2) % 3;
    const BBox pb = prim.bbox();
    const bool overlaps = get<A1>(pb.min) <= get<A1>(cross.max) && get<A1>(pb.max) >= get<A1>(cross.min) &&
                          get<A2>(pb.min) <= get<A2>(cross.max) && get<A2>(pb.max) >= get<A2>(cross.min);
    if (!overlaps) return room;
    const int layer = int(((UP ? get<AXIS>(pb.min) : get<AXIS>(pb.max)) - get<AXIS>(k.gmin)) * get<AXIS>(k.grid_inv));
    const int free_layers = UP ? layer - comp(cell.hi, AXIS) : comp(cell.lo, AXIS) - layer - 1;
    return max(min(room, free_layers), 0);
}

template <int AXIS, bool SUBSET_ONLY>
__device__ __forceinline__ int face_growth(const ExpandK& k, const Entry* __restrict__ entries, const int* __restrict__ refs, const float4* __restrict__ tris,
                                           const Cell* __restrict__ cells, const CellRec& cell, bool UP, bool& again) {
    constexpr int A1 = (AXIS + 1) % 3, A2 = (AXIS + 2) % 3;
    const int face = UP ? comp(cell.hi, AXIS) : comp(cell.lo, AXIS);
    const int extent = comp(k.dims, AXIS);
    if (UP ? face >= extent : face <= 0) return 0;
    const int layer = UP ? face : face - 1;
    const int lo1 = comp(cell.lo, A1), hi1 = comp(cell.hi, A1), lo2 = comp(cell.lo, A2), hi2 = comp(cell.hi, A2);
    const int own = cell.end - cell.begin;
    int reach = extent, room = extent;
    int u = lo1, v = lo2, row_step = comp(k.dims, A2);
    for (;;) {
        const ivec3 at = AXIS == 0 ? ivec3(layer, u, v) : (AXIS == 1 ? ivec3(v, layer, u) : ivec3(u, v, layer));
        const CellRec nb = load_cell(cells, cell_of_voxel(k, entries, at));
        reach = min(reach, UP ? comp(nb.hi, AXIS) - face : face - comp(nb.lo, AXIS));
        room = min(room, reach);
        const int theirs = nb.end - nb.begin;
        if (SUBSET_ONLY) {
            if (!contains_all(refs + cell.begin, own, refs + nb.begin, theirs)) { room = 0; break; }
        } else if (theirs > 0) {
            const BBox cross(k.gmin + k.cell_size * vec3(cell.lo), k.gmin + k.cell_size * vec3(cell.hi));
            int mine = 0;
            for (int j = 0; j < theirs && room > 0; j++) {
                const int id = refs[nb.begin + j];
                while (mine < own && refs[cell.begin + mine] < id) mine++;
                if (mine < own && refs[cell.begin + mine] == id) continue;
                room = room_before_prim<AXIS>(k, load_tri(tris, id), cell, cross, room, UP);
            }
            if (room == 0) break;
        }
        row_step = min(row_step, comp(nb.hi, A2) - v);
        u = comp(nb.hi, A1);
        if (u >= hi1) {
            u = lo1; v += row_step; row_step = comp(k.dims, A2);
            if (v >= hi2) break;
        }
    }
    again |= room == reach;
    return UP ? room : -room;
}

template <int axis, bool SUBSET_ONLY, bool PAIRED>
__device__ __forceinline__ void grow_cell(const ExpandK& k, const Entry* __restrict__ entries, const int* __restrict__ refs, const float4* __restrict__ tris,
                                          const Cell* __restrict__ cells, Cell* __restrict__ new_cells, unsigned char* __restrict__ cell_flags, int id, int flags, bool up) {
    CellRec cell = load_cell(cells, id);
    bool flag = false;
    int ov1, ov2;
    if (PAIRED) {
        bool again = false;
        const int mine = face_growth<axis, SUBSET_ONLY>(k, entries, refs, tris, cells, cell, up, again);
        const int other = __shfl_xor(mine, 1, 64);
        flag = again | (__shfl_xor(int(again), 1, 64) != 0);
        if (up) return;
        ov1 = mine; ov2 = other;
    } else {
        ov1 = face_growth<axis, SUBSET_ONLY>(k, entries, refs, tris, cells, cell, false, flag);
        ov2 = face_growth<axis, SUBSET_ONLY>(k, entries, refs, tris, cells, cell, true, flag);
    }
    if (axis == 0) { cell.lo.x += ov1; cell.hi.x += ov2; }
    if (axis == 1) { cell.lo.y += ov1; cell.hi.y += ov2; }
    if (axis == 2) { cell.lo.z += ov1; cell.hi.z += ov2; }
    cell_flags[id] = (unsigned char)((flag ? 1 << axis : 0) | (flags & ~((1 << axis) | kChanged)) | ((ov1 | ov2) ? kChanged : 0));
    int4* out = reinterpret_cast<int4*>(new_cells) + 2 * size_t(id);
    out[0] = make_int4(cell.lo.x, cell.lo.y, cell.lo.z, cell.begin);
    out[1] = make_int4(cell.hi.x, cell.hi.y, cell.hi.z, cell.end);
}

template <int axis, bool SUBSET_ONLY>
__global__ void __launch_bounds__(kBlock) overlap_step(ExpandK k, const Entry* __restrict__ entries, const int* __restrict__ refs,
                                                       const float4* __restrict__ tris, const Cell* __restrict__ cells, Cell* __restrict__ new_cells,
                                                       unsigned char* __restrict__ cell_flags, int num_cells) {
    const int id = xcd_block(blockIdx.x, gridDim.x) * kBlock + threadIdx.x;
    if (id >= num_cells) return;
    const int flags = cell_flags[id];
    if ((flags & (1 << axis)) == 0) {
        const int4* p = reinterpret_cast<const int4*>(cells) + 2 * size_t(id);
        int4* out = reinterpret_cast<int4*>(new_cells) + 2 * size_t(id);
        const int4 a = p[0], b = p[1];
        out[0] = a; out[1] = b;
        if (flags & kChanged) cell_flags[id] = (unsigned char)(flags & ~kChanged);
        return;
    }
    grow_cell<axis, SUBSET_ONLY, false>(k, entries, refs, tris, cells, new_cells, cell_flags, id, flags, false);
}

constexpr int kSelectItems = 16;
constexpr int kSelectTile = kBlock * kSelectItems;

template <int axis>
__global__ void __launch_bounds__(kBlock) expand_select(const Cell* __restrict__ cells, Cell* __restrict__ new_cells, unsigned char* __restrict__ cell_flags,
                                                        int num_cells, int* __restrict__ list, int* __restrict__ count) {
    __shared__ int tile_list[kSelectTile];
    __shared__ int tile_count, tile_base;
    if (threadIdx.x == 0) tile_count = 0;
    __syncthreads();
    const int base = blockIdx.x * kSelectTile;
    int fl[kSelectItems];
    #pragma unroll
    for (int j = 0; j < kSelectItems; j++) {
        const int id = base + j * kBlock + threadIdx.x;
        fl[j] = id < num_cells ? cell_flags[id] : 0;
    }
    #pragma unroll
    for (int j = 0; j < kSelectItems; j++) {
        const int id = base + j * kBlock + threadIdx.x;
        const int flags = fl[j];
        const bool listed = (flags & (1 << axis)) != 0;
        const unsigned long long m = __ballot(listed);
        int wbase = 0;
        if (lane_id() == 0 && m) wbase = atomicAdd(&tile_count, __popcll(m));
        wbase = __shfl(wbase, 0, 64);
        if (listed) {
            tile_list[wbase + __popcll(m & ((1ull << lane_id()) - 1ull))] = id;
        } else if (flags & kChanged) {
            const int4* p = reinterpret_cast<const int4*>(cells) + 2 * size_t(id);
            int4* out = reinterpret_cast<int4*>(new_cells) + 2 * size_t(id);
            const int4 a = p[0], b = p[1];
            out[0] = a; out[1] = b;
            cell_flags[id] = (unsigned char)(flags & ~kChanged);
        }
    }
    __syncthreads();
    if (threadIdx.x == 0) tile_base = tile_count ? atomicAdd(count, tile_count) : 0;
    __syncthreads();
    for (int i = threadIdx.x; i < tile_count; i += kBlock) list[tile_base + i] = tile_list[i];
}

template <int axis, bool SUBSET_ONLY>
__global__ void __launch_bounds__(kBlock) expand_listed(ExpandK k, const Entry* __restrict__ entries, const int* __restrict__ refs,
                                                        const float4* __restrict__ tris, const Cell* __restrict__ cells, Cell* __restrict__ new_cells,
                                                        unsigned char* __restrict__ cell_flags, const int* __restrict__ list, const int* __restrict__ count) {
    const int n = *count, active = (2 * n + kBlock - 1) / kBlock;
    if (int(blockIdx.x) >= active) return;
    const int t = xcd_block(blockIdx.x, active) * kBlock + threadIdx.x;
    const int i = t >> 1;
    if (i >= n) return;
    const int id = list[i];
    grow_cell<axis, SUBSET_ONLY, true>(k, entries, refs, tris, cells, new_cells, cell_flags, id, cell_flags[id], (t & 1) != 0);
}

template <int axis, bool SUBSET_ONLY>
void listed_step(hipStream_t st, const ExpandK& k, const Entry* entries, const int* refs, const float4* tris, const Cell* cells, Cell* other,
                 unsigned char* flags, int n, int* list, int* count) {
    expand_select<axis><<<grid_blocks(n, kSelectTile), kBlock, 0, st>>>(cells, other, flags, n, list, count);
    expand_listed<axis, SUBSET_ONLY><<<grid_blocks(2ll * n, kBlock), kBlock, 0, st>>>(k, entries, refs, tris, cells, other, flags, list, count);
}

}

extern "C" int hagrid_expand_grid(hagrid_ctx* ctx, hagrid_grid* grid, const void* tris_v, int iters) {
    if (!ctx || !grid) return HAGRID_EINVAL;
    const bool subset_only = ctx->opt_expand_subset_only != 0;
    if (!subset_only && !tris_v && iters > 0) HG_FAIL(ctx, HAGRID_EINVAL, "expand_grid: the precise mode needs the triangles");
    const float4* tris = static_cast<const float4*>(tris_v);
    if (iters <= 0) return HAGRID_OK;
    if (!grid->cells || !grid->entries || !grid->ref_ids) HG_FAIL(ctx, HAGRID_EINVAL, "expand_grid: incomplete (or compressed) grid");
    trav_image_drop(ctx);
    HG_HIP(ctx, hipSetDevice(ctx->device));
    hipStream_t st = ctx->stream;
    ExpandK k;
    k.top = ivec3(grid->dims[0], grid->dims[1], grid->dims[2]);
    k.dims = k.top << grid->shift;
    k.shift = grid->shift;
    {
        const vec3 lo(grid->bbox_min[0], grid->bbox_min[1], grid->bbox_min[2]), ext = vec3(grid->bbox_max[0], grid->bbox_max[1], grid->bbox_max[2]) - lo;
        k.gmin = lo; k.cell_size = ext / vec3(k.dims); k.grid_inv = vec3(k.dims) / ext;
    }
    const int n = grid->num_cells;
    Cell* cells = static_cast<Cell*>(grid->cells);
    Cell* other = pool_alloc<Cell>(ctx, size_t(n));
    unsigned char* flags = pool_alloc<unsigned char>(ctx, size_t(n));
    if (!other || !flags) { hagrid_mem_free(ctx, other); hagrid_mem_free(ctx, flags); return HAGRID_ENOMEM; }
    (void)hipMemsetAsync(flags, 0xFF, size_t(n), st);
    const Entry* entries = static_cast<const Entry*>(grid->entries);
    const int* refs = static_cast<const int*>(grid->ref_ids);
    const int blocks = grid_blocks(n, kBlock);
    int* list = iters > 1 ? pool_try_alloc<int>(ctx, size_t(n)) : nullptr;
    const long long voxels = (long long)k.dims.x * k.dims.y * k.dims.z;
    int* voxel_cells = (ctx->opt_expand_voxel_map && voxels <= (1ll << 28)) ? pool_try_alloc<int>(ctx, size_t(voxels)) : nullptr;
    k.voxel_cells = voxel_cells;
    if (voxel_cells) { ExpandK kf = k; kf.voxel_cells = nullptr; fill_voxel_cells<<<grid_blocks(voxels, kBlock), kBlock, 0, st>>>(kf, entries, voxel_cells, int(voxels)); HG_DBG(ctx); }
    int* counts = ctx->dscratch + 160;
    const int max_listed = 48;
    if (list) (void)hipMemsetAsync(counts, 0, max_listed * sizeof(int), st);
    int listed = 0;
    for (int it = 0; it < iters; it++) {
        if (it > 0 && list && listed + 3 <= max_listed) {
            if (subset_only) {
                listed_step<0, true>(st, k, entries, refs, tris, cells, other, flags, n, list, counts + listed++); std::swap(cells, other);
                listed_step<1, true>(st, k, entries, refs, tris, cells, other, flags, n, list, counts + listed++); std::swap(cells, other);
                listed_step<2, true>(st, k, entries, refs, tris, cells, other, flags, n, list, counts + listed++); std::swap(cells, other);
            } else {
                listed_step<0, false>(st, k, entries, refs, tris, cells, other, flags, n, list, counts + listed++); std::swap(cells, other);
                listed_step<1, false>(st, k, entries, refs, tris, cells, other, flags, n, list, counts + listed++); std::swap(cells, other);
                listed_step<2, false>(st, k, entries, refs, tris, cells, other, flags, n, list, counts + listed++); std::swap(cells, other);
            }
            continue;
        }
        if (subset_only) {
            overlap_step<0, true><<<blocks, kBlock, 0, st>>>(k, entries, refs, tris, cells, other, flags, n); HG_DBG(ctx); std::swap(cells, other);
            overlap_step<1, true><<<blocks, kBlock, 0, st>>>(k, entries, refs, tris, cells, other, flags, n); HG_DBG(ctx); std::swap(cells, other);
            overlap_step<2, true><<<blocks, kBlock, 0, st>>>(k, entries, refs, tris, cells, other, flags, n); HG_DBG(ctx); std::swap(cells, other);
        } else {
            overlap_step<0, false><<<blocks, kBlock, 0, st>>>(k, entries, refs, tris, cells, other, flags, n); HG_DBG(ctx); std::swap(cells, other);
            overlap_step<1, false><<<blocks, kBlock, 0, st>>>(k, entries, refs, tris, cells, other, flags, n); HG_DBG(ctx); std::swap(cells, other);
            overlap_step<2, false><<<blocks, kBlock, 0, st>>>(k, entries, refs, tris, cells, other, flags, n); HG_DBG(ctx); std::swap(cells, other);
        }
    }
    hipError_t e = hipGetLastError();
    if (e == hipSuccess) e = hipStreamSynchronize(st);
    ctx->counts.expand_passes = 3 * iters; ctx->counts.expand_cells = n;
    hagrid_mem_free(ctx, flags);
    hagrid_mem_free(ctx, other);
    hagrid_mem_free(ctx, list);
    hagrid_mem_free(ctx, voxel_cells);
    grid->cells = cells;
    if (e != hipSuccess) HG_FAIL(ctx, HAGRID_EHIP, hipGetErrorString(e));
    return HAGRID_OK;
}
```

hagrid_amd/csrc/flatten.hip:

```cpp
#include "ctx.h"
#include "wave_prims.h"

#include "hagrid/grid.h"

using namespace hagrid;
using namespace hagrid_impl;

namespace {

constexpr int kFlatLevels = 3;

__global__ void __launch_bounds__(kBlock) collapse_and_depth(uint32_t* __restrict__ entries, int* __restrict__ depths, int first, int num) {
    const int id = blockIdx.x * kBlock + threadIdx.x;
    if (id >= num) return;
    uint32_t e = entries[first + id];
    int d = 0;
    if (e & 3u) {
        const uint4* p = reinterpret_cast<const uint4*>(entries + (e >> 2));
        const uint4 a = p[0], b = p[1];
        if (a.x == a.y && a.x == a.z && a.x == a.w && a.x == b.x && b.x == b.y && b.x == b.z && b.x == b.w) {
            e = a.x;
            entries[first + id] = e;
        }
    }
    if (e & 3u) {
        const int4* q = reinterpret_cast<const int4*>(depths + (e >> 2));
        const int4 a = q[0], b = q[1];
        d = 1 + max(max(max(a.x, b.x), max(a.y, b.y)), max(max(a.z, b.z), max(a.w, b.w)));
    }
    depths[first + id] = d;
}

struct BlockSizeIn {
    const int* depths;
    __device__ int operator()(int i) const { const int d = depths[i]; return d > 0 ? 1 << (min(d, kFlatLevels) * 3) : 0; }
};
struct StartOut {
    int* start;
    __device__ void operator()(int i, int s) const { start[i] = s; }
};

__global__ void __launch_bounds__(kBlock) copy_top(const uint32_t* __restrict__ entries, const int* __restrict__ start, const int* __restrict__ depths,
                                                   uint32_t* __restrict__ out, int num) {
    const int id = blockIdx.x * kBlock + threadIdx.x;
    if (id >= num) return;
    uint32_t e = entries[id];
    if (e & 3u) e = uint32_t(min(depths[id], kFlatLevels)) | (uint32_t(start[id]) << 2);
    out[id] = e;
}

__global__ void __launch_bounds__(kBlock) flatten_level(const uint32_t* __restrict__ entries, const int* __restrict__ start, const int* __restrict__ depths,
                                                        uint32_t* __restrict__ out, int first, int num) {
    const int id = blockIdx.x * kWaves + wave_id();
    if (id >= num) return;
    const int d = min(depths[first + id], kFlatLevels);
    if (d == 0) return;
    const int nsub = 1 << (3 * d);
    const int base = start[first + id];
    const uint32_t root = entries[first + id];
    for (int m = lane_id(); m < nsub; m += 64) {
        int x = 0, y = 0, z = 0, next_id = first + id;
        uint32_t e = root;
        for (int cur = d - 1; cur >= 0; cur--) {
            const int pos = m >> (cur * 3);
            x += (pos & 1) << cur;
            y += ((pos >> 1) & 1) << cur;
            z += ((pos >> 2) & 1) << cur;
            if (e & 3u) { next_id = int(e >> 2) + (pos & 7); e = entries[next_id]; }
        }
        if (e & 3u) e = uint32_t(min(depths[next_id], kFlatLevels)) | (uint32_t(start[next_id]) << 2);
        out[base + x + ((y + (z << d)) << d)] = e;
    }
}

}

extern "C" int hagrid_flatten_grid(hagrid_ctx* ctx, hagrid_grid* grid) {
    if (!ctx || !grid) return HAGRID_EINVAL;
    if (!grid->entries || grid->num_offsets != grid->shift + 1) HG_FAIL(ctx, HAGRID_EINVAL, "flatten_grid: needs the un-flattened voxel map of build_grid/merge_grid");
    trav_image_drop(ctx);
    HG_HIP(ctx, hipSetDevice(ctx->device));
    hipStream_t st = ctx->stream;
    const int shift = grid->shift, num_entries = grid->num_entries;
    uint32_t* entries = static_cast<uint32_t*>(grid->entries);
    auto first_of = [&](int i) { return i > 0 ? grid->offsets[i - 1] : 0; };

    int* depths = pool_alloc<int>(ctx, size_t(num_entries) + 8);
    int* start = pool_alloc<int>(ctx, size_t(num_entries) + 8);
    int max_level = 0;
    for (int i = 0; i <= shift; i++) max_level = std::max(max_level, grid->offsets[i] - first_of(i));
    int* partials = pool_alloc<int>(ctx, size_t(scan_num_tiles(max_level)) + 1);
    auto release = [&]() { hagrid_mem_free(ctx, depths); hagrid_mem_free(ctx, start); hagrid_mem_free(ctx, partials); };
    if (!depths || !start || !partials) { release(); return HAGRID_ENOMEM; }

    for (int i = shift; i >= 0; i--) {
        const int first = first_of(i), num = grid->offsets[i] - first;
        if (num > 0) collapse_and_depth<<<grid_blocks(num, kBlock), kBlock, 0, st>>>(entries, depths, first, num);
    }
    int* carry = ctx->dscratch;
    const int top_entries = grid->offsets[0];
    HG_HIP(ctx, hipMemcpyAsync(carry, &top_entries, sizeof(int), hipMemcpyHostToDevice, st));
    int groups = 0;
    for (int i = 0; i < shift; i += kFlatLevels, groups++) {
        const int first = first_of(i), num = grid->offsets[i] - first;
        if (!ctx_scan<int>(ctx, BlockSizeIn{depths + first}, StartOut{start + first}, num, partials, carry + groups, carry + groups + 1)) { release(); return HAGRID_ENOMEM; }
    }
    int h[HAGRID_MAX_LEVELS + 2];
    int rc = read_back(ctx, carry, h, sizeof(int) * size_t(groups + 1));
    if (rc != HAGRID_OK) { release(); return rc; }
    const int total_entries = h[groups];
    if (total_entries < top_entries || total_entries > 0x3fffffff) { release(); HG_FAIL(ctx, HAGRID_ERANGE, "flatten_grid: voxel map too large"); }

    uint32_t* out = pool_alloc<uint32_t>(ctx, size_t(total_entries));
    if (!out) { release(); return HAGRID_ENOMEM; }
    copy_top<<<grid_blocks(top_entries, kBlock), kBlock, 0, st>>>(entries, start, depths, out, top_entries); HG_DBG(ctx);
    int new_offsets[HAGRID_MAX_LEVELS], num_new = 0;
    for (int i = 0, g = 0; i < shift; i += kFlatLevels, g++) {
        const int first = first_of(i), num = grid->offsets[i] - first;
        if (num > 0) flatten_level<<<grid_blocks(num, kWaves), kBlock, 0, st>>>(entries, start, depths, out, first, num);
        new_offsets[num_new++] = h[g];
    }
    new_offsets[num_new++] = total_entries;
    hipError_t e = hipGetLastError();
    if (e == hipSuccess) e = hipStreamSynchronize(st);
    if (e != hipSuccess) { release(); hagrid_mem_free(ctx, out); HG_FAIL(ctx, HAGRID_EHIP, hipGetErrorString(e)); }
    release();
    hagrid_mem_free(ctx, entries);
    ctx->counts.flatten_entries_in = num_entries; ctx->counts.flatten_entries_out = total_entries;
    grid->entries = out;
    grid->num_entries = total_entries;
    grid->num_offsets = num_new;
    for (int i = 0; i < num_new; i++) grid->offsets[i] = new_offsets[i];
    return HAGRID_OK;
}
```

hagrid_amd/csrc/merge.hip:

```cpp
#include "ctx.h"
#include "wave_prims.h"

#include "hagrid/grid.h"

using namespace hagrid;
using namespace hagrid_impl;

namespace {

struct MergeK {
    ivec3 dims;
    ivec3 top;
    vec3 cell_size;
    int shift;
};

struct CellRec { ivec3 lo; int begin; ivec3 hi; int end; };

template <bool NARROW> struct CellFmt;
template <> struct CellFmt<false> {
    static __device__ __forceinline__ CellRec load(const void* cells, int i) {
        const int4* p = reinterpret_cast<const int4*>(cells) + 2 * size_t(i);
        const int4 a = p[0], b = p[1];
        CellRec c; c.lo = ivec3(a.x, a.y, a.z); c.begin = a.w; c.hi = ivec3(b.x, b.y, b.z); c.end = b.w;
        return c;
    }
    static __device__ __forceinline__ void finish(const void*, int, CellRec&) {}
    static __device__ __forceinline__ void store(void* cells, int i, ivec3 lo, int begin, ivec3 hi, int end) {
        int4* p = reinterpret_cast<int4*>(cells) + 2 * size_t(i);
        p[0] = make_int4(lo.x, lo.y, lo.z, begin);
        p[1] = make_int4(hi.x, hi.y, hi.z, end);
    }
    static __device__ __forceinline__ void store_end(void*, int, int) {}
};
template <> struct CellFmt<true> {
    static __device__ __forceinline__ CellRec load(const void* cells, int i) {
        const uint4 v = reinterpret_cast<const uint4*>(cells)[i];
        CellRec c;
        c.lo = ivec3(int(v.x & 0xffffu), int(v.x >> 16), int(v.y & 0xffffu));
        c.hi = ivec3(int(v.y >> 16), int(v.z & 0xffffu), int(v.z >> 16));
        c.begin = int(v.w); c.end = int(v.w);
        return c;
    }
    static __device__ __forceinline__ void finish(const void* cells, int i, CellRec& c) { c.end = int(reinterpret_cast<const uint4*>(cells)[size_t(i) + 1].w); }
    static __device__ __forceinline__ void store(void* cells, int i, ivec3 lo, int begin, ivec3 hi, int) {
        reinterpret_cast<uint4*>(cells)[i] = make_uint4(uint32_t(lo.x) | uint32_t(lo.y) << 16, uint32_t(lo.z) | uint32_t(hi.x) << 16,
                                                        uint32_t(hi.y) | uint32_t(hi.z) << 16, uint32_t(begin));
    }
    static __device__ __forceinline__ void store_end(void* cells, int num_cells, int num_refs) {
        reinterpret_cast<uint4*>(cells)[num_cells] = make_uint4(0u, 0u, 0u, uint32_t(num_refs));
    }
};
__device__ __forceinline__ int comp(const ivec3& v, int axis) { return axis == 0 ? v.x : (axis == 1 ? v.y : v.z); }
__device__ __forceinline__ float comp(const vec3& v, int axis) { return axis == 0 ? v.x : (axis == 1 ? v.y : v.z); }

__device__ __forceinline__ bool aligned(int axis, const CellRec& c1, const CellRec& c2) {
    const int a1 = (axis + 1) % 3, a2 = (axis + 2) % 3;
    return comp(c1.hi, axis) == comp(c2.lo, axis) &&
           comp(c1.lo, a1) == comp(c2.lo, a1) && comp(c1.lo, a2) == comp(c2.lo, a2) &&
           comp(c1.hi, a1) == comp(c2.hi, a1) && comp(c1.hi, a2) == comp(c2.hi, a2);
}
__device__ __forceinline__ bool merge_allowed(const MergeK& k, int empty_mask, int pos) {
    const int top_level_mask = (1 << k.shift) - 1;
    const int is_shifted = (pos >> k.shift) & empty_mask;
    const bool is_top_level = !(pos & top_level_mask);
    return !is_shifted || !is_top_level;
}
__device__ __forceinline__ ivec3 next_cell_pos(int axis, const ivec3& lo, const ivec3& hi) {
    return ivec3(axis == 0 ? hi.x : lo.x, axis == 1 ? hi.y : lo.y, axis == 2 ? hi.z : lo.z);
}
__device__ __forceinline__ int lower_bound_in(const int* __restrict__ a, int n, int x) {
    int lo = 0, hi = n;
    while (lo < hi) {
        const int mid = (lo + hi) >> 1;
        if (a[mid] < x) lo = mid + 1; else hi = mid;
    }
    return lo;
}
__device__ __forceinline__ int union_size(const int* __restrict__ a, int na, const int* __restrict__ b, int nb) {
    if (na == 0 || nb == 0) return na + nb;
    int common = 0;
    if (na <= 4 && nb <= 4) {
        const int a0 = a[0], a1 = na > 1 ? a[1] : -1, a2 = na > 2 ? a[2] : -1, a3 = na > 3 ? a[3] : -1;
        const int b0 = b[0], b1 = nb > 1 ? b[1] : -2, b2 = nb > 2 ? b[2] : -2, b3 = nb > 3 ? b[3] : -2;
        auto hits = [&](int x) { return int(x == b0) + int(x == b1) + int(x == b2) + int(x == b3); };
        common = hits(a0) + hits(a1) + hits(a2) + hits(a3);
    } else {
        if (nb > na) { const int* t = a; a = b; b = t; const int n = na; na = nb; nb = n; }
        for (int j = 0; j < nb; j++) {
            const int x = b[j], at = lower_bound_in(a, na, x);
            common += at < na && a[at] == x;
        }
    }
    return na + nb - common;
}
__device__ __forceinline__ void write_union(const int* __restrict__ a, int na, const int* __restrict__ b, int nb, int* __restrict__ out, int n_out) {
    const int inf = 0x7fffffff;
    int i = 0, j = 0;
    int x = na > 0 ? a[0] : inf, y = nb > 0 ? b[0] : inf;
    for (int o = 0; o < n_out; o++) {
        const int m = min(x, y);
        out[o] = m;
        if (x == m) { i++; x = i < na ? a[i] : inf; }
        if (y == m) { j++; y = j < nb ? b[j] : inf; }
    }
}

__device__ __forceinline__ int merged_size_if_cheaper(const MergeK& k, int axis, const CellRec& c1, const CellRec& c2, const int* __restrict__ refs) {
    const float unit_cost = 1.0f;
    const vec3 e1 = vec3(c1.hi - c1.lo) * k.cell_size;
    const vec3 e2 = vec3(c2.hi - c2.lo) * k.cell_size;
    const float a1 = e1.x * (e1.y + e1.z) + e1.y * e1.z;
    const float a2 = e2.x * (e2.y + e2.z) + e2.y * e2.z;
    const float a = a1 + a2 - comp(e1, (axis + 1) % 3) * comp(e1, (axis + 2) % 3);
    const int n1 = c1.end - c1.begin, n2 = c2.end - c2.begin;
    const float cc1 = a1 * (n1 + unit_cost), cc2 = a2 * (n2 + unit_cost);
    if (a * (max(n1, n2) + unit_cost) <= cc1 + cc2) {
        const int n = union_size(refs + c1.begin, n1, refs + c2.begin, n2);
        const float c = a * (n + unit_cost);
        if (c <= cc1 + cc2) return n;
    }
    return -1;
}

template <bool NARROW>
__global__ void __launch_bounds__(kBlock) merge_counts_kernel(int axis, MergeK k, const Entry* __restrict__ entries, const void* __restrict__ cells,
                                                              const int* __restrict__ refs, int* __restrict__ merge_counts,
                                                              int* __restrict__ nexts, unsigned char* __restrict__ has_prev, int pass_tag, int empty_mask, int num_cells,
                                                              const int* __restrict__ n_dev) {
    using F = CellFmt<NARROW>;
    const int n = n_dev ? *n_dev : num_cells, active = (n + kBlock - 1) / kBlock;
    if (int(blockIdx.x) >= active) return;
    const int id = xcd_block(blockIdx.x, active) * kBlock + threadIdx.x;
    if (id >= n) return;
    CellRec c1 = F::load(cells, id);
    F::finish(cells, id, c1);
    const ivec3 np = next_cell_pos(axis, c1.lo, c1.hi);
    int count = -(c1.end - c1.begin + 1);
    int next_id = -1;
    if (merge_allowed(k, empty_mask, comp(c1.lo, axis)) && comp(np, axis) < comp(k.dims, axis)) {
        next_id = int(lookup_entry(entries, k.shift, k.top, np));
        CellRec c2 = F::load(cells, next_id);
        if (aligned(axis, c1, c2)) {
            F::finish(cells, next_id, c2);
            const int n = merged_size_if_cheaper(k, axis, c1, c2, refs);
            if (n >= 0) count = n;
        }
    }
    merge_counts[id] = count;
    next_id = count >= 0 ? next_id : -1;
    nexts[id] = next_id;
    if (next_id >= 0) has_prev[next_id] = (unsigned char)pass_tag;
}

__global__ void __launch_bounds__(kBlock) cell_flags_kernel(const int* __restrict__ nexts, const unsigned char* __restrict__ has_prev, int pass_tag,
                                                            unsigned char* __restrict__ cell_flags, int num_cells, const int* __restrict__ n_dev) {
    const int id = (blockIdx.x * kBlock + threadIdx.x) * 4;
    const int n = n_dev ? *n_dev : num_cells;
    if (id >= n) return;
    int hp[4], nx[4];
    if (id + 4 <= n) {
        const uchar4 h = *reinterpret_cast<const uchar4*>(has_prev + id);
        const int4 x = *reinterpret_cast<const int4*>(nexts + id);
        hp[0] = h.x; hp[1] = h.y; hp[2] = h.z; hp[3] = h.w; nx[0] = x.x; nx[1] = x.y; nx[2] = x.z; nx[3] = x.w;
    } else {
        for (int c = 0; c < 4; c++) { hp[c] = id + c < n ? has_prev[id + c] : pass_tag; nx[c] = id + c < n ? nexts[id + c] : -1; }
    }
#pragma unroll
    for (int c = 0; c < 4; c++) {
        if (hp[c] == pass_tag) continue;
        int next_id = nx[c];
        cell_flags[id + c] = 1;
        int count = 1;
        while (next_id >= 0) {
            cell_flags[next_id] = (count & 1) ? 0 : 1;
            next_id = nexts[next_id];
            count++;
        }
    }
}

constexpr int kMergeTile = kBlock;
__device__ __forceinline__ Int2 keep_item(int flag, int count) { return Int2{ flag ? 1 : 0, flag ? (count >= 0 ? count : -(count + 1)) : 0 }; }

__global__ void __launch_bounds__(kBlock) merge_tile_sums(const unsigned char* __restrict__ cell_flags, const int* __restrict__ merge_counts, int num_cells,
                                                          const int* __restrict__ n_dev, Int2* __restrict__ sums, int num_tiles) {
    static_assert(kMergeTile == 64 * 4, "a wavefront covers one tile with four cells per lane");
    const int tile = blockIdx.x * kWaves + wave_id();
    if (tile >= num_tiles) return;
    const int n = n_dev ? min(num_cells, *n_dev) : num_cells;
    const int i = tile * kMergeTile + lane_id() * 4;
    Int2 s{0, 0};
    if (i + 4 <= n) {
        const uchar4 f = *reinterpret_cast<const uchar4*>(cell_flags + i);
        const int4 m = *reinterpret_cast<const int4*>(merge_counts + i);
        s = keep_item(f.x, m.x) + keep_item(f.y, m.y) + keep_item(f.z, m.z) + keep_item(f.w, m.w);
    } else {
        for (int c = 0; c < 4; c++) if (i + c < n) s = s + keep_item(cell_flags[i + c], merge_counts[i + c]);
    }
    s = Int2{wave_sum(s.a), wave_sum(s.b)};
    if (lane_id() == 0) sums[tile] = s;
}
struct SumsIn { const Int2* v; __device__ Int2 operator()(int i) const { return v[i]; } };
struct SumsOut { Int2* v; __device__ void operator()(int i, Int2 s) const { v[i] = s; } };

template <bool IN_NARROW, bool OUT_NARROW>
__global__ void __launch_bounds__(kBlock) merge_kernel(int axis, MergeK k, const Entry* __restrict__ entries, const void* __restrict__ cells,
                                                       const int* __restrict__ refs, const unsigned char* __restrict__ cell_flags,
                                                       const Int2* __restrict__ tile_prefix, const int* __restrict__ merge_counts,
                                                       int* new_cell_ids ,
                                                       void* __restrict__ new_cells, int* __restrict__ new_refs, int num_cells, const int* __restrict__ n_dev,
                                                       const Int2* __restrict__ totals,
                                                       const unsigned char* __restrict__ stamp_in, unsigned char* __restrict__ stamp_out, int stamp) {
    using FI = CellFmt<IN_NARROW>;
    using FO = CellFmt<OUT_NARROW>;
    __shared__ Int2 lds[kWaves];
    const int n = n_dev ? min(num_cells, *n_dev) : num_cells, active = (n + kBlock - 1) / kBlock;
    if (int(blockIdx.x) >= active && blockIdx.x != 0) return;
    const int tile = int(blockIdx.x) < active ? xcd_block(blockIdx.x, active) : 0;
    const int id = tile * kBlock + threadIdx.x;
    if (id == 0) FO::store_end(new_cells, totals->a, totals->b);
    const bool inside = id < n;
    const int flag = inside ? cell_flags[id] : 0;
    const int mc = inside ? merge_counts[id] : 0;
    const Int2 item = keep_item(flag, mc);
    const Int2 incl = wave_inclusive_scan(item);
    if (lane_id() == 63) lds[wave_id()] = incl;
    __syncthreads();
    if (!flag) return;
    Int2 at = tile_prefix[tile];
    for (int w = 0; w < wave_id(); w++) at = at + lds[w];
    const int new_id = at.a + incl.a - item.a, nb = at.b + incl.b - item.b;
    CellRec cell = FI::load(cells, id);
    FI::finish(cells, id, cell);
    const int next_id = new_cell_ids[id];
    new_cell_ids[id] = new_id;
    if (stamp_out) stamp_out[new_id] = (unsigned char)(mc >= 0 ? stamp : (stamp_in ? stamp_in[id] : 0));
    const int n1 = cell.end - cell.begin;
    if (mc >= 0) {
        CellRec nc = FI::load(cells, next_id);
        FI::finish(cells, next_id, nc);
        new_cell_ids[next_id] = new_id;
        FO::store(new_cells, new_id, min(nc.lo, cell.lo), nb, max(nc.hi, cell.hi), nb + mc);
        if (nc.begin < nc.end) {
            write_union(refs + cell.begin, n1, refs + nc.begin, nc.end - nc.begin, new_refs + nb, mc);
            return;
        }
    } else {
        FO::store(new_cells, new_id, cell.lo, nb, cell.hi, nb + n1);
    }
    for (int i = 0; i < n1; i++) new_refs[nb + i] = refs[cell.begin + i];
}


constexpr uint32_t kTombLo = 0xffffu;
__device__ __forceinline__ bool ip_is_tomb(const uint4& v) { return (v.x & 0xffffu) == kTombLo; }
__device__ __forceinline__ int ip_live(const void* cells, int id) {
    for (;;) {
        const uint4 v = reinterpret_cast<const uint4*>(cells)[id];
        if (!ip_is_tomb(v)) return id;
        id = int(v.w);
    }
}
__device__ __forceinline__ CellRec ip_load(const void* cells, const int* list_end, int id) {
    CellRec c = CellFmt<true>::load(cells, id);
    c.end = list_end[id];
    return c;
}

constexpr int kIpPer = 4;
constexpr int kIpTile = kBlock * kIpPer;
__device__ __forceinline__ uint32_t ip_flags4(const unsigned char* __restrict__ f, int id4, int slots) {
    if (id4 + 4 <= slots) return *reinterpret_cast<const uint32_t*>(f + id4);
    uint32_t v = 0;
    for (int c = 0; c < 4; c++) if (id4 + c < slots) v |= uint32_t(f[id4 + c]) << (8 * c);
    return v;
}
__device__ __forceinline__ uint32_t ip_match4(uint32_t flags, int tag) {
    uint32_t m = 0;
    for (int c = 0; c < 4; c++) if (int((flags >> (8 * c)) & 0xffu) == tag) m |= 1u << (8 * c);
    return m;
}

__device__ __forceinline__ int ip_compact_tile(uint32_t mask4 , int id4, int* __restrict__ list, int* __restrict__ count) {
    if (threadIdx.x == 0) *count = 0;
    __syncthreads();
    const int n = int((mask4 & 1u) + ((mask4 >> 8) & 1u) + ((mask4 >> 16) & 1u) + ((mask4 >> 24) & 1u));
    const int incl = wave_inclusive_scan(n);
    const int total = __shfl(incl, 63, 64);
    int base = 0;
    if (lane_id() == 63 && total) base = atomicAdd(count, total);
    base = __shfl(base, 63, 64) + incl - n;
    for (int c = 0; c < 4; c++) if (mask4 & (1u << (8 * c))) list[base++] = id4 + c;
    __syncthreads();
    return *count;
}

__global__ void __launch_bounds__(kBlock) ip_begin(const void* __restrict__ cells, int slots, int* __restrict__ list_end, unsigned char* __restrict__ dirty,
                                                   const unsigned char* __restrict__ stamps, int since_x, int since_y, int since_z,
                                                   unsigned char* __restrict__ evaluated, unsigned char* __restrict__ absorbs, int* __restrict__ books, int num_refs, size_t dstride) {
    const int id = blockIdx.x * kBlock + threadIdx.x;
    if (id == 0) { books[0] = num_refs; books[1] = slots; books[2] = num_refs; books[3] = 0; }
    if (id >= slots) return;
    evaluated[id] = 0; absorbs[id] = 0;
    list_end[id] = int(reinterpret_cast<const uint4*>(cells)[size_t(id) + 1].w);
    const int st = stamps ? stamps[id] : 255;
    dirty[id] = st >= since_x; dirty[dstride + id] = st >= since_y; dirty[2 * dstride + id] = st >= since_z;
}
__global__ void __launch_bounds__(kBlock) ip_mark_entry(MergeK k, const Entry* __restrict__ entries, const void* __restrict__ cells, int slots,
                                                        unsigned char* __restrict__ dirty, const unsigned char* __restrict__ stamps, int since_x, int since_y, int since_z, size_t dstride) {
    __shared__ int list[kIpTile];
    __shared__ int count;
    const int id4 = (blockIdx.x * kBlock + threadIdx.x) * kIpPer;
    const int since_min = min(since_x, min(since_y, since_z));
    uint32_t recent = 0;
    if (id4 < slots) {
        const uint32_t f = ip_flags4(stamps, id4, slots);
        for (int c = 0; c < 4; c++) if (id4 + c < slots && int((f >> (8 * c)) & 0xffu) >= since_min) recent |= 1u << (8 * c);
    }
    const int n = ip_compact_tile(recent, id4, list, &count);
    for (int i = threadIdx.x; i < n; i += kBlock) {
        const int id = list[i], st = stamps[id];
        const CellRec cell = CellFmt<true>::load(cells, id);
        for (int axis = 0; axis < 3; axis++) {
            if (st < (axis == 0 ? since_x : (axis == 1 ? since_y : since_z))) continue;
            ivec3 p = cell.lo;
            if (axis == 0) p.x--; else if (axis == 1) p.y--; else p.z--;
            if (comp(p, axis) < 0) continue;
            dirty[size_t(axis) * dstride + int(lookup_entry(entries, k.shift, k.top, p))] = 1;
        }
    }
}

__device__ __forceinline__ void ip_count_one(int id, int axis, const MergeK& k, const Entry* __restrict__ entries, const void* __restrict__ cells, const int* __restrict__ list_end,
                                             const int* __restrict__ refs, Int2* __restrict__ minfo, int* __restrict__ nexts, unsigned char* __restrict__ evaluated,
                                             unsigned char* __restrict__ has_prev, int pass_tag, int empty_mask) {
    if (ip_is_tomb(reinterpret_cast<const uint4*>(cells)[id])) return;
    const CellRec c1 = ip_load(cells, list_end, id);
    const ivec3 np = next_cell_pos(axis, c1.lo, c1.hi);
    if (!merge_allowed(k, empty_mask, comp(c1.lo, axis)) || comp(np, axis) >= comp(k.dims, axis)) return;
    const int next_id = ip_live(cells, int(lookup_entry(entries, k.shift, k.top, np)));
    const CellRec c2 = ip_load(cells, list_end, next_id);
    if (!aligned(axis, c1, c2)) return;
    const int n = merged_size_if_cheaper(k, axis, c1, c2, refs);
    if (n < 0) return;
    minfo[id] = Int2{ n, (c1.end - c1.begin) + (c2.end - c2.begin) - n };
    nexts[id] = next_id;
    evaluated[id] = (unsigned char)pass_tag;
    has_prev[next_id] = (unsigned char)pass_tag;
}
__global__ void __launch_bounds__(kBlock) ip_counts(int axis, MergeK k, const Entry* __restrict__ entries, const void* __restrict__ cells, const int* __restrict__ list_end,
                                                    const int* __restrict__ refs, int slots, unsigned char* __restrict__ dirty_axis,
                                                    Int2* __restrict__ minfo, int* __restrict__ nexts, unsigned char* __restrict__ evaluated,
                                                    unsigned char* __restrict__ has_prev, int pass_tag, int empty_mask) {
    __shared__ int list[kIpTile];
    __shared__ int count;
    const int id4 = (xcd_block(blockIdx.x, gridDim.x) * kBlock + threadIdx.x) * kIpPer;
    uint32_t mask = 0;
    if (id4 < slots) {
        const uint32_t f = ip_flags4(dirty_axis, id4, slots);
        for (int c = 0; c < 4; c++) if ((f >> (8 * c)) & 0xffu) { mask |= 1u << (8 * c); dirty_axis[id4 + c] = 0; }
    }
    const int n = ip_compact_tile(mask, id4, list, &count);
    for (int i = threadIdx.x; i < n; i += kBlock)
        ip_count_one(list[i], axis, k, entries, cells, list_end, refs, minfo, nexts, evaluated, has_prev, pass_tag, empty_mask);
}

__global__ void __launch_bounds__(kBlock) ip_chains(int slots, const int* __restrict__ nexts, const unsigned char* __restrict__ evaluated,
                                                    const unsigned char* __restrict__ has_prev, unsigned char* __restrict__ absorbs, int pass_tag) {
    const int id4 = (blockIdx.x * kBlock + threadIdx.x) * kIpPer;
    if (id4 >= slots) return;
    const uint32_t heads = ip_match4(ip_flags4(evaluated, id4, slots), pass_tag) & ~ip_match4(ip_flags4(has_prev, id4, slots), pass_tag);
    if (!heads) return;
    for (int c = 0; c < 4; c++) {
        if (!(heads & (1u << (8 * c)))) continue;
        int cur = id4 + c, pos = 0;
        for (;;) {
            const int nxt = evaluated[cur] == pass_tag ? nexts[cur] : -1;
            if (nxt < 0) break;
            if (!(pos & 1)) absorbs[cur] = (unsigned char)pass_tag;
            cur = nxt; pos++;
        }
    }
}

__global__ void __launch_bounds__(kBlock) ip_tile_sums(const unsigned char* __restrict__ absorbs, int pass_tag, const Int2* __restrict__ minfo, int slots,
                                                       Int2* __restrict__ sums, int* __restrict__ removed) {
    __shared__ int lds[kWaves];
    const int id4 = (blockIdx.x * kBlock + threadIdx.x) * kIpPer;
    int need = 0, merges = 0, gone = 0;
    if (id4 < slots) {
        const uint32_t m = ip_match4(ip_flags4(absorbs, id4, slots), pass_tag);
        for (int c = 0; c < 4; c++) if (m & (1u << (8 * c))) { const Int2 v = minfo[id4 + c]; need += v.a; merges++; gone += v.b; }
    }
    need = block_sum(need, lds); merges = block_sum(merges, lds); gone = block_sum(gone, lds);
    if (threadIdx.x == 0) { sums[blockIdx.x] = Int2{need, merges}; removed[blockIdx.x] = gone; }
}

__global__ void __launch_bounds__(kBlock) ip_apply(void* cells, int* list_end, int* refs, const unsigned char* __restrict__ absorbs, int pass_tag,
                                                   const Int2* __restrict__ minfo, const int* __restrict__ nexts, const Int2* __restrict__ tile_prefix,
                                                   int slots, int* __restrict__ books, const Int2* __restrict__ pass_total, int capacity, int axis) {
    __shared__ int lds[kWaves];
    const int id4 = (blockIdx.x * kBlock + threadIdx.x) * kIpPer;
    const int* cursor = books;
    const int overflow = __hip_atomic_load(books + 3, __ATOMIC_RELAXED, __HIP_MEMORY_SCOPE_AGENT);
    if (overflow > 0 || (long long)*cursor + pass_total->a > (long long)capacity) {
        if (id4 == 0 && overflow <= 0) __hip_atomic_store(books + 3, -(1 + axis), __ATOMIC_RELAXED, __HIP_MEMORY_SCOPE_AGENT);
        return;
    }
    const uint32_t mine = id4 < slots ? ip_match4(ip_flags4(absorbs, id4, slots), pass_tag) : 0u;
    int m[4], total = 0;
    for (int c = 0; c < 4; c++) { m[c] = (mine & (1u << (8 * c))) ? minfo[id4 + c].a : 0; total += m[c]; }
    const int incl = wave_inclusive_scan(total);
    if (lane_id() == 63) lds[wave_id()] = incl;
    __syncthreads();
    if (!mine) return;
    int at = *cursor + tile_prefix[blockIdx.x].a + incl - total;
    for (int w = 0; w < wave_id(); w++) at += lds[w];
    for (int c = 0; c < 4; c++) {
        if (!(mine & (1u << (8 * c)))) continue;
        const int id = id4 + c, other = nexts[id];
        const CellRec a = ip_load(cells, list_end, id), n = ip_load(cells, list_end, other);
        write_union(refs + a.begin, a.end - a.begin, refs + n.begin, n.end - n.begin, refs + at, m[c]);
        CellFmt<true>::store(cells, id, min(n.lo, a.lo), at, max(n.hi, a.hi), 0);
        list_end[id] = at + m[c];
        reinterpret_cast<uint4*>(cells)[other] = make_uint4(kTombLo, 0u, 0u, uint32_t(id));
        at += m[c];
    }
}

__global__ void __launch_bounds__(kBlock) ip_mark(MergeK k, const Entry* __restrict__ entries, const void* __restrict__ cells, const unsigned char* __restrict__ absorbs,
                                                  int pass_tag, int slots, unsigned char* __restrict__ dirty, const Int2* __restrict__ pass_total,
                                                  const int* __restrict__ removed, int num_tiles, int* __restrict__ books ,
                                                  int* __restrict__ snap, size_t dstride) {
    __shared__ int lds[kWaves];
    const int id4 = (blockIdx.x * kBlock + threadIdx.x) * kIpPer;
    const int overflow = books[3];
    if (blockIdx.x == 0) {
        int gone = 0;
        for (int i = threadIdx.x; i < num_tiles; i += kBlock) gone += removed[i];
        gone = block_sum(gone, lds);
        if (threadIdx.x == 0) {
            if (overflow == 0) { books[0] += pass_total->a; books[1] -= pass_total->b; books[2] -= gone; }
            else if (overflow < 0) books[3] = -overflow;
            snap[0] = books[1]; snap[1] = books[2];
        }
    }
    __shared__ int list[kIpTile];
    __shared__ int count;
    const uint32_t mine = (overflow == 0 && id4 < slots) ? ip_match4(ip_flags4(absorbs, id4, slots), pass_tag) : 0u;
    const int n = ip_compact_tile(mine, id4, list, &count);
    for (int i = threadIdx.x; i < n; i += kBlock) {
        const int id = list[i];
        const CellRec cell = CellFmt<true>::load(cells, id);
        for (int axis = 0; axis < 3; axis++) {
            dirty[size_t(axis) * dstride + id] = 1;
            ivec3 p = cell.lo;
            if (axis == 0) p.x--; else if (axis == 1) p.y--; else p.z--;
            if (comp(p, axis) < 0) continue;
            dirty[size_t(axis) * dstride + ip_live(cells, int(lookup_entry(entries, k.shift, k.top, p)))] = 1;
        }
    }
}

__global__ void __launch_bounds__(kBlock) ip_live_sums(const void* __restrict__ cells, const int* __restrict__ list_end, int slots, Int2* __restrict__ sums, int num_tiles) {
    const int tile = blockIdx.x * kWaves + wave_id();
    if (tile >= num_tiles) return;
    Int2 s{0, 0};
    for (int c = 0; c < 4; c++) {
        const int i = tile * kMergeTile + c * 64 + lane_id();
        if (i < slots) {
            const uint4 v = reinterpret_cast<const uint4*>(cells)[i];
            if (!ip_is_tomb(v)) s = s + Int2{1, list_end[i] - int(v.w)};
        }
    }
    s = Int2{wave_sum(s.a), wave_sum(s.b)};
    if (lane_id() == 0) sums[tile] = s;
}
__global__ void __launch_bounds__(kBlock) ip_compact(const void* __restrict__ cells, const int* __restrict__ list_end, const int* __restrict__ refs, int slots,
                                                     const Int2* __restrict__ tile_prefix, Cell* __restrict__ out_cells, int* __restrict__ out_refs, int* __restrict__ new_ids) {
    __shared__ Int2 lds[kWaves];
    const int id = blockIdx.x * kBlock + threadIdx.x;
    uint4 v = make_uint4(kTombLo, 0u, 0u, 0u);
    if (id < slots) v = reinterpret_cast<const uint4*>(cells)[id];
    const bool live = id < slots && !ip_is_tomb(v);
    const int end = live ? list_end[id] : 0;
    const Int2 item = live ? Int2{1, end - int(v.w)} : Int2{0, 0};
    const Int2 incl = wave_inclusive_scan(item);
    if (lane_id() == 63) lds[wave_id()] = incl;
    __syncthreads();
    if (id >= slots) return;
    if (!live) { new_ids[id] = -1 - int(v.w); return; }
    Int2 at = tile_prefix[blockIdx.x];
    for (int w = 0; w < wave_id(); w++) at = at + lds[w];
    const int new_id = at.a + incl.a - 1, nb = at.b + incl.b - item.b;
    const CellRec c = CellFmt<true>::load(cells, id);
    CellFmt<false>::store(out_cells, new_id, c.lo, nb, c.hi, nb + item.b);
    for (int i = 0; i < item.b; i++) out_refs[nb + i] = refs[c.begin + i];
    new_ids[id] = new_id;
}
__global__ void __launch_bounds__(kBlock) ip_resolve_tombs(int* __restrict__ new_ids, int slots) {
    const int id = blockIdx.x * kBlock + threadIdx.x;
    if (id >= slots) return;
    int v = new_ids[id];
    if (v >= 0) return;
    int cur = -1 - v;
    for (;;) {
        const int w = __hip_atomic_load(new_ids + cur, __ATOMIC_RELAXED, __HIP_MEMORY_SCOPE_AGENT);
        if (w >= 0) { v = w; break; }
        cur = -1 - w;
    }
    new_ids[id] = v;
}

__global__ void __launch_bounds__(kBlock) widen_cells_kernel(const void* __restrict__ narrow, Cell* __restrict__ cells, const Int2* __restrict__ totals) {
    const int id = blockIdx.x * kBlock + threadIdx.x;
    if (id >= totals->a) return;
    CellRec c = CellFmt<true>::load(narrow, id);
    CellFmt<true>::finish(narrow, id, c);
    CellFmt<false>::store(cells, id, c.lo, c.begin, c.hi, c.end);
}

__global__ void __launch_bounds__(kBlock) remap_entries_kernel(uint32_t* __restrict__ entries, const int* __restrict__ new_cell_ids, int num_entries) {
    const int id = (blockIdx.x * kBlock + threadIdx.x) * 4;
    if (id >= num_entries) return;
    auto remap = [&](uint32_t e) { return (e & 3u) == 0 ? uint32_t(new_cell_ids[e >> 2]) << 2 : e; };
    if (id + 4 <= num_entries && lb_aligned16(entries + id)) {
        uint4* p = reinterpret_cast<uint4*>(entries + id);
        const uint4 e = *p;
        *p = make_uint4(remap(e.x), remap(e.y), remap(e.z), remap(e.w));
    } else {
        for (int i = id; i < min(id + 4, num_entries); i++) entries[i] = remap(entries[i]);
    }
}

}

extern "C" int hagrid_merge_grid(hagrid_ctx* ctx, hagrid_grid* grid, float alpha) {
    if (!ctx || !grid) return HAGRID_EINVAL;
    if (!grid->cells || !grid->entries || !grid->ref_ids) HG_FAIL(ctx, HAGRID_EINVAL, "merge_grid: incomplete (or compressed) grid");
    trav_image_drop(ctx);
    ctx->counts.merge_passes = 0;
    ctx->counts.merged_cells = grid->num_cells; ctx->counts.merged_refs = grid->num_refs;
    if (!(alpha > 0)) return HAGRID_OK;
    HG_HIP(ctx, hipSetDevice(ctx->device));
    hipStream_t st = ctx->stream;

    MergeK k;
    k.top = ivec3(grid->dims[0], grid->dims[1], grid->dims[2]);
    k.dims = k.top << grid->shift;
    k.shift = grid->shift;
    k.cell_size = (vec3(grid->bbox_max[0], grid->bbox_max[1], grid->bbox_max[2]) - vec3(grid->bbox_min[0], grid->bbox_min[1], grid->bbox_min[2])) / vec3(k.dims);

    const size_t nc0 = size_t(grid->num_cells), nr0 = size_t(grid->num_refs);
    Cell* cells_b = pool_alloc<Cell>(ctx, nc0);
    int* refs_b = pool_alloc<int>(ctx, nr0);
    int* merge_counts = pool_alloc<int>(ctx, nc0 + 1);
    int* nexts = pool_alloc<int>(ctx, nc0 + 1);
    unsigned char* prevs = pool_alloc<unsigned char>(ctx, nc0 + 4);
    unsigned char* cell_flags = pool_alloc<unsigned char>(ctx, nc0 + 4);
    const size_t stamp_stride = (nc0 + 4 + 255) & ~size_t(255);
    unsigned char* stamps = pool_alloc<unsigned char>(ctx, 2 * stamp_stride);
    unsigned char* stamps_other = stamps ? stamps + stamp_stride : nullptr;
    unsigned char* const stamps_base = stamps;
    const int max_tiles = grid_blocks(grid->num_cells, kMergeTile);
    Int2* tile_sums = pool_alloc<Int2>(ctx, size_t(max_tiles) + 1);
    Int2* partials = pool_alloc<Int2>(ctx, size_t(scan_num_tiles(max_tiles)) + 1);
    Int2* total = reinterpret_cast<Int2*>(ctx->dscratch);
    auto release = [&]() {
        hagrid_mem_free(ctx, merge_counts); hagrid_mem_free(ctx, nexts); hagrid_mem_free(ctx, prevs); hagrid_mem_free(ctx, cell_flags);
        hagrid_mem_free(ctx, tile_sums); hagrid_mem_free(ctx, partials); hagrid_mem_free(ctx, stamps_base);
    };
    if (!cells_b || !refs_b || !merge_counts || !nexts || !prevs || !cell_flags || !tile_sums || !partials || !stamps) {
        release(); hagrid_mem_free(ctx, cells_b); hagrid_mem_free(ctx, refs_b);
        return HAGRID_ENOMEM;
    }

    void* cells = grid->cells;
    void* cells_other = cells_b;
    int* refs = static_cast<int*>(grid->ref_ids);
    uint32_t* entries = static_cast<uint32_t*>(grid->entries);
    int num_cells = grid->num_cells, num_refs = grid->num_refs;
    const int num_entries = grid->num_entries;
    const bool narrow = ctx->opt_merge_narrow && std::max(k.dims.x, std::max(k.dims.y, k.dims.z)) < 65536;

    int rc = HAGRID_OK;
    int prev_num_cells = 0, iter = 0, pass_tag = 0;
    bool in_narrow = false;
    (void)hipMemsetAsync(prevs, 0, nc0, st);
    hagrid_build_counts& bc = ctx->counts;
    auto record = [&](int c, int r) {
        if (bc.merge_passes < HAGRID_MAX_MERGE_PASSES) { bc.merge_cells[bc.merge_passes] = c; bc.merge_refs[bc.merge_passes] = r; bc.merge_passes++; }
    };

    int global_pass = 0;
    bool have_stamps = false;
    int since[3] = {0, 0, 0};
    bool in_place = false;
    int ip_slots = 0, ip_iters = 0, prev_mask = 0;
    int* list_end = merge_counts;
    Int2* minfo = nullptr; unsigned char* dirty = nullptr; unsigned char* evaluated = nullptr;
    int* books = ctx->dscratch + 16;
    int* snap = ctx->dscratch + 20;
    Int2* ip_total = reinterpret_cast<Int2*>(ctx->dscratch + 26);
    int* tile_removed = nullptr;
    const int ip_capacity = int(std::min<size_t>(nr0, 0x7fffffff));
    size_t ip_dstride = 0;
    auto ip_enter = [&]() -> bool {
        const auto r256 = [](size_t n) { return (n + 255) & ~size_t(255); };
        const size_t slots = size_t(num_cells), dstride = r256(slots);
        const size_t off_dirty = r256(slots * 8), off_eval = off_dirty + 3 * dstride, off_removed = off_eval + r256(slots);
        if (off_removed + r256(size_t(grid_blocks(num_cells, kIpTile)) * sizeof(int)) > nc0 * sizeof(Cell)) return false;
        ip_slots = num_cells; ip_dstride = dstride;
        char* scratch = static_cast<char*>(cells_other);
        minfo = reinterpret_cast<Int2*>(scratch);
        dirty = reinterpret_cast<unsigned char*>(scratch + off_dirty);
        evaluated = reinterpret_cast<unsigned char*>(scratch + off_eval);
        tile_removed = reinterpret_cast<int*>(scratch + off_removed);
        const unsigned char* stp = have_stamps ? stamps : nullptr;
        ip_begin<<<grid_blocks(ip_slots, kBlock), kBlock, 0, st>>>(cells, ip_slots, list_end, dirty, stp, since[0], since[1], since[2],
                                                                   evaluated, cell_flags , books, num_refs, ip_dstride); HG_DBG(ctx);
        if (stp) ip_mark_entry<<<grid_blocks(ip_slots, kIpTile), kBlock, 0, st>>>(k, reinterpret_cast<const Entry*>(entries), cells, ip_slots, dirty, stp, since[0], since[1], since[2], ip_dstride); HG_DBG(ctx);
        in_place = true;
        return true;
    };
    auto ip_leave = [&]() -> int {
        const int tiles = grid_blocks(ip_slots, kMergeTile);
        ip_live_sums<<<grid_blocks(tiles, kWaves), kBlock, 0, st>>>(cells, list_end, ip_slots, tile_sums, tiles); HG_DBG(ctx);
        if (!ctx_scan<Int2>(ctx, SumsIn{tile_sums}, SumsOut{tile_sums}, tiles, partials, (const Int2*)nullptr, ip_total)) return HAGRID_ENOMEM;
        ip_compact<<<tiles, kBlock, 0, st>>>(cells, list_end, refs, ip_slots, tile_sums, static_cast<Cell*>(cells_other), refs_b, nexts); HG_DBG(ctx);
        ip_resolve_tombs<<<grid_blocks(ip_slots, kBlock), kBlock, 0, st>>>(nexts, ip_slots); HG_DBG(ctx);
        remap_entries_kernel<<<grid_blocks((num_entries + 3) / 4, kBlock), kBlock, 0, st>>>(entries, nexts, num_entries); HG_DBG(ctx);
        std::swap(cells, cells_other);
        std::swap(refs, refs_b);
        int h[2];
        HG_TRY(read_back(ctx, ip_total, h, sizeof(h)));
        if (h[0] != num_cells) return fail(ctx, HAGRID_EHIP, __FILE__, __LINE__, "merge_grid: the books of the in-place iterations do not add up");
        num_refs = h[1];
        in_place = false; in_narrow = false; ip_iters = 0;
        have_stamps = false;
        return HAGRID_OK;
    };
    int last_pass_in = 0, last_pass_out = 0;
    auto compacting_passes = [&](int first_axis, int mask) -> int {
        for (int axis = first_axis; axis < 3; axis++) {
            const int blocks = grid_blocks(num_cells, kBlock);
            Int2* tot = total + axis;
            const int* n_dev = axis > first_axis ? &total[axis - 1].a : nullptr;
            const Entry* ent = reinterpret_cast<const Entry*>(entries);
            if (++pass_tag == 256) { pass_tag = 1; (void)hipMemsetAsync(prevs, 0, nc0, st); }
            if (in_narrow) merge_counts_kernel<true><<<blocks, kBlock, 0, st>>>(axis, k, ent, cells, refs, merge_counts, nexts, prevs, pass_tag, mask, num_cells, n_dev);
            else           merge_counts_kernel<false><<<blocks, kBlock, 0, st>>>(axis, k, ent, cells, refs, merge_counts, nexts, prevs, pass_tag, mask, num_cells, n_dev);
            HG_DBG(ctx);
            cell_flags_kernel<<<grid_blocks((num_cells + 3) / 4, kBlock), kBlock, 0, st>>>(nexts, prevs, pass_tag, cell_flags, num_cells, n_dev); HG_DBG(ctx);
            const int tiles = grid_blocks(num_cells, kMergeTile);
            merge_tile_sums<<<grid_blocks(tiles, kWaves), kBlock, 0, st>>>(cell_flags, merge_counts, num_cells, n_dev, tile_sums, tiles); HG_DBG(ctx);
            if (!ctx_scan<Int2>(ctx, SumsIn{tile_sums}, SumsOut{tile_sums}, tiles, partials, (const Int2*)nullptr, tot)) return HAGRID_ENOMEM;
            global_pass++;
            const bool stamping = global_pass < 250 && (have_stamps || global_pass == 1);
            const unsigned char* st_in = stamping && have_stamps ? stamps : nullptr;
            unsigned char* st_out = stamping ? stamps_other : nullptr;
            if (in_narrow)   merge_kernel<true, true><<<tiles, kBlock, 0, st>>>(axis, k, ent, cells, refs, cell_flags, tile_sums, merge_counts, nexts, cells_other, refs_b, num_cells, n_dev, tot, st_in, st_out, global_pass);
            else if (narrow) merge_kernel<false, true><<<tiles, kBlock, 0, st>>>(axis, k, ent, cells, refs, cell_flags, tile_sums, merge_counts, nexts, cells_other, refs_b, num_cells, n_dev, tot, st_in, st_out, global_pass);
            else             merge_kernel<false, false><<<tiles, kBlock, 0, st>>>(axis, k, ent, cells, refs, cell_flags, tile_sums, merge_counts, nexts, cells_other, refs_b, num_cells, n_dev, tot, st_in, st_out, global_pass);
            HG_DBG(ctx);
            have_stamps = stamping; since[axis] = global_pass;
            std::swap(stamps, stamps_other);
            in_narrow = narrow;
            remap_entries_kernel<<<grid_blocks((num_entries + 3) / 4, kBlock), kBlock, 0, st>>>(entries, nexts, num_entries); HG_DBG(ctx);
            std::swap(cells, cells_other);
            std::swap(refs, refs_b);
        }
        int h[6];
        HG_TRY(read_back(ctx, total, h, sizeof(int) * 6));
        for (int axis = first_axis; axis < 3; axis++) {
            record(num_cells, num_refs);
            if (axis == 2) { last_pass_in = num_cells; last_pass_out = h[4]; }
            num_cells = h[2 * axis]; num_refs = h[2 * axis + 1];
        }
        return HAGRID_OK;
    };

    do {
        prev_num_cells = num_cells;
        const int mask = iter > 3 ? 0 : (1 << (iter + 1)) - 1;
        if (in_place && ctx->opt_merge_inplace_iters > 0 && ip_iters >= ctx->opt_merge_inplace_iters) {
            rc = ip_leave();
            if (rc != HAGRID_OK) break;
        }
        int first_compacting_axis = 0;
        if (in_place) {
            if (prev_mask & ~mask) (void)hipMemsetAsync(dirty, 1, 3 * ip_dstride, st);
            const int blocks = grid_blocks(ip_slots, kIpTile), tiles = blocks;
            const Entry* ent = reinterpret_cast<const Entry*>(entries);
            for (int axis = 0; axis < 3 && rc == HAGRID_OK; axis++) {
                global_pass++;
                if (++pass_tag == 256) {
                    pass_tag = 1;
                    (void)hipMemsetAsync(prevs, 0, nc0, st); (void)hipMemsetAsync(evaluated, 0, size_t(ip_slots), st); (void)hipMemsetAsync(cell_flags, 0, size_t(ip_slots), st);
                }
                ip_counts<<<blocks, kBlock, 0, st>>>(axis, k, ent, cells, list_end, refs, ip_slots, dirty + size_t(axis) * ip_dstride, minfo, nexts, evaluated, prevs, pass_tag, mask); HG_DBG(ctx);
                ip_chains<<<blocks, kBlock, 0, st>>>(ip_slots, nexts, evaluated, prevs, cell_flags, pass_tag); HG_DBG(ctx);
                ip_tile_sums<<<tiles, kBlock, 0, st>>>(cell_flags, pass_tag, minfo, ip_slots, tile_sums, tile_removed); HG_DBG(ctx);
                if (!ctx_scan<Int2>(ctx, SumsIn{tile_sums}, SumsOut{tile_sums}, tiles, partials, (const Int2*)nullptr, ip_total)) { rc = HAGRID_ENOMEM; break; }
                ip_apply<<<tiles, kBlock, 0, st>>>(cells, list_end, refs, cell_flags, pass_tag, minfo, nexts, tile_sums, ip_slots, books, ip_total,
                                                    ctx->opt_merge_inplace_room > 0 ? std::min(ip_capacity, ctx->opt_merge_inplace_room) : ip_capacity, axis); HG_DBG(ctx);
                ip_mark<<<blocks, kBlock, 0, st>>>(k, ent, cells, cell_flags, pass_tag, ip_slots, dirty, ip_total, tile_removed, tiles, books, snap + 2 * axis, ip_dstride); HG_DBG(ctx);
            }
            if (rc != HAGRID_OK) break;
            int h[10];
            rc = read_back(ctx, books, h, sizeof(h));
            if (rc != HAGRID_OK) break;
            const int applied = h[3] > 0 ? h[3] - 1 : 3;
            for (int axis = 0; axis < applied; axis++) { record(num_cells, num_refs); num_cells = h[4 + 2 * axis]; num_refs = h[5 + 2 * axis]; }
            ip_iters++;
            if (applied < 3) {
                rc = ip_leave();
                if (rc != HAGRID_OK) break;
                first_compacting_axis = applied;
            }
        }
        if (!in_place) {
            if (first_compacting_axis < 3) rc = compacting_passes(first_compacting_axis, mask);
            if (rc != HAGRID_OK) break;
            const int div = ctx->opt_merge_inplace_div > 0 ? ctx->opt_merge_inplace_div : 2;
            if (in_narrow && ctx->opt_merge_inplace && (long long)div * (prev_num_cells - num_cells) < prev_num_cells && num_cells < alpha * prev_num_cells) (void)ip_enter();
        }
        prev_mask = mask;
        iter++;
    } while (rc == HAGRID_OK && num_cells < alpha * prev_num_cells);
    if (rc == HAGRID_OK && in_place) rc = ip_leave();
    else if (rc == HAGRID_OK && in_narrow) {
        widen_cells_kernel<<<grid_blocks(num_cells, kBlock), kBlock, 0, st>>>(cells, static_cast<Cell*>(cells_other), total + 2); HG_DBG(ctx);
        std::swap(cells, cells_other);
    }

    if (rc == HAGRID_OK) {
        hipError_t e = hipGetLastError();
        if (e != hipSuccess) rc = fail(ctx, HAGRID_EHIP, __FILE__, __LINE__, hipGetErrorString(e));
    }
    release();
    hagrid_mem_free(ctx, cells_other);
    hagrid_mem_free(ctx, refs_b);
    if (rc != HAGRID_OK) {
        (void)hipStreamSynchronize(st);
        hagrid_mem_free(ctx, cells); hagrid_mem_free(ctx, refs);
        grid->cells = nullptr; grid->ref_ids = nullptr; grid->num_cells = 0; grid->num_refs = 0;
        return rc;
    }
    grid->cells = cells; grid->ref_ids = refs;
    grid->num_cells = num_cells; grid->num_refs = num_refs;
    ctx->counts.merged_cells = num_cells; ctx->counts.merged_refs = num_refs;
    return rc;
}
```

hagrid_amd/csrc/wave_prims.h:

```cpp
#pragma once
#include "ctx.h"

#include <hip/hip_runtime.h>
#include <stdint.h>

#include <algorithm>

namespace hagrid_impl {

constexpr int kBlock = 256;
constexpr int kWaves = kBlock / 64;
constexpr int kScanItems = 8;
constexpr int kScanTile = kBlock * kScanItems;

__device__ __forceinline__ int lane_id() { return threadIdx.x & 63; }
__device__ __forceinline__ int wave_id() { return threadIdx.x >> 6; }

#ifndef HG_XCD_CHUNK_LOG2
#define HG_XCD_CHUNK_LOG2 6
#endif
constexpr int kXcdChunkLog2 = HG_XCD_CHUNK_LOG2;
__device__ __forceinline__ int xcd_block(int b, int nb) {
    if (kXcdChunkLog2 < 0) return b;
    const int full = (nb >> (kXcdChunkLog2 + 3)) << (kXcdChunkLog2 + 3);
    if (b >= full) return b;
    const int xcd = b & 7, j = b >> 3;
    return ((((j >> kXcdChunkLog2) << 3) + xcd) << kXcdChunkLog2) + (j & ((1 << kXcdChunkLog2) - 1));
}

struct Int2 { int a, b; };
__host__ __device__ inline Int2 operator+(Int2 x, Int2 y) { return Int2{x.a + y.a, x.b + y.b}; }
__host__ __device__ inline int zero_of(int) { return 0; }
__host__ __device__ inline Int2 zero_of(Int2) { return Int2{0, 0}; }

__device__ __forceinline__ int shfl_up_v(int v, int d) { return __shfl_up(v, d, 64); }
__device__ __forceinline__ Int2 shfl_up_v(Int2 v, int d) { return Int2{__shfl_up(v.a, d, 64), __shfl_up(v.b, d, 64)}; }
__device__ __forceinline__ int shfl_xor_v(int v, int d) { return __shfl_xor(v, d, 64); }
__device__ __forceinline__ Int2 shfl_xor_v(Int2 v, int d) { return Int2{__shfl_xor(v.a, d, 64), __shfl_xor(v.b, d, 64)}; }
__device__ __forceinline__ int shfl_v(int v, int l) { return __shfl(v, l, 64); }
__device__ __forceinline__ Int2 shfl_v(Int2 v, int l) { return Int2{__shfl(v.a, l, 64), __shfl(v.b, l, 64)}; }

template <typename V>
__device__ __forceinline__ V wave_inclusive_scan(V v) {
    const int l = lane_id();
#pragma unroll
    for (int d = 1; d < 64; d <<= 1) {
        V o = shfl_up_v(v, d);
        if (l >= d) v = v + o;
    }
    return v;
}

__device__ __forceinline__ int wave_sum(int v) {
#pragma unroll
    for (int d = 32; d > 0; d >>= 1) v += __shfl_xor(v, d, 64);
    return v;
}
__device__ __forceinline__ int wave_max(int v) {
#pragma unroll
    for (int d = 32; d > 0; d >>= 1) { int o = __shfl_xor(v, d, 64); v = o > v ? o : v; }
    return v;
}
__device__ __forceinline__ float wave_min_f(float v) {
#pragma unroll
    for (int d = 32; d > 0; d >>= 1) { float o = __shfl_xor(v, d, 64); v = o < v ? o : v; }
    return v;
}
__device__ __forceinline__ float wave_max_f(float v) {
#pragma unroll
    for (int d = 32; d > 0; d >>= 1) { float o = __shfl_xor(v, d, 64); v = o > v ? o : v; }
    return v;
}

__device__ __forceinline__ int block_sum(int v, int* lds) {
    v = wave_sum(v);
    __syncthreads();
    if (lane_id() == 0) lds[wave_id()] = v;
    __syncthreads();
    int r = 0;
#pragma unroll
    for (int w = 0; w < kWaves; w++) r += lds[w];
    return r;
}

__device__ __forceinline__ int wave_append(int n, int* counter) {
    const int incl = wave_inclusive_scan(n);
    const int total = __shfl(incl, 63, 64);
    int base = 0;
    if (lane_id() == 63 && total > 0) base = atomicAdd(counter, total);
    base = __shfl(base, 63, 64);
    return base + incl - n;
}


template <typename V, typename In>
__global__ void __launch_bounds__(kBlock) scan_partials(In in, int n, V* partials) {
    __shared__ V lds[kWaves];
    const int base = blockIdx.x * kScanTile;
    V s = zero_of(V());
#pragma unroll
    for (int j = 0; j < kScanItems; j++) {
        const int i = base + j * kBlock + threadIdx.x;
        if (i < n) s = s + in(i);
    }
    s = wave_inclusive_scan(s);
    if (lane_id() == 63) lds[wave_id()] = s;
    __syncthreads();
    if (threadIdx.x == 0) {
        V t = lds[0];
        for (int w = 1; w < kWaves; w++) t = t + lds[w];
        partials[blockIdx.x] = t;
    }
}

template <typename V>
__global__ void __launch_bounds__(kBlock) scan_spine(V* partials, int num_partials, const V* carry_in, V* total_out) {
    __shared__ V lds[kWaves];
    __shared__ V running;
    if (threadIdx.x == 0) running = carry_in ? *carry_in : zero_of(V());
    __syncthreads();
    for (int base = 0; base < num_partials; base += kBlock) {
        const int i = base + threadIdx.x;
        const V v = i < num_partials ? partials[i] : zero_of(V());
        const V incl = wave_inclusive_scan(v);
        if (lane_id() == 63) lds[wave_id()] = incl;
        __syncthreads();
        V excl = running;
        for (int w = 0; w < wave_id(); w++) excl = excl + lds[w];
        const V prev = shfl_up_v(incl, 1);
        if (lane_id() > 0) excl = excl + prev;
        if (i < num_partials) partials[i] = excl;
        __syncthreads();
        if (threadIdx.x == 0) {
            V t = running;
            for (int w = 0; w < kWaves; w++) t = t + lds[w];
            running = t;
        }
        __syncthreads();
    }
    if (threadIdx.x == 0 && total_out) *total_out = running;
}

template <typename V, typename In, typename Out>
__global__ void __launch_bounds__(kBlock) scan_apply(In in, Out out, int n, const V* partials) {
    __shared__ V lds[kWaves];
    __shared__ V running;
    if (threadIdx.x == 0) running = partials[blockIdx.x];
    __syncthreads();
    const int base = blockIdx.x * kScanTile;
#pragma unroll 1
    for (int j = 0; j < kScanItems; j++) {
        const int i = base + j * kBlock + threadIdx.x;
        if (base + j * kBlock >= n) break;
        const V v = i < n ? in(i) : zero_of(V());
        const V incl = wave_inclusive_scan(v);
        if (lane_id() == 63) lds[wave_id()] = incl;
        __syncthreads();
        V excl = running;
        for (int w = 0; w < wave_id(); w++) excl = excl + lds[w];
        const V prev = shfl_up_v(incl, 1);
        if (lane_id() > 0) excl = excl + prev;
        if (i < n) out(i, excl);
        __syncthreads();
        if (threadIdx.x == 0) {
            V t = running;
            for (int w = 0; w < kWaves; w++) t = t + lds[w];
            running = t;
        }
        __syncthreads();
    }
}

constexpr int kLbVec = 4;
constexpr int kLbItems = 8;
constexpr int kLbWindows = 4;
constexpr int kLbTile = kBlock * kLbItems;
constexpr unsigned kLbAggregate = 1u, kLbPrefix = 2u;

__device__ __forceinline__ unsigned long long lb_pack(unsigned epoch, unsigned flag, int value) {
    return ((unsigned long long)epoch << 34) | ((unsigned long long)flag << 32) | (unsigned)value;
}
__device__ __forceinline__ void lb_store(unsigned long long* p, unsigned long long w) {
    __hip_atomic_store(p, w, __ATOMIC_RELAXED, __HIP_MEMORY_SCOPE_AGENT);
}
__device__ __forceinline__ unsigned long long lb_load(const unsigned long long* p) {
    return __hip_atomic_load(p, __ATOMIC_RELAXED, __HIP_MEMORY_SCOPE_AGENT);
}
__device__ __forceinline__ void lb_publish(unsigned long long* state, int tile, unsigned epoch, unsigned flag, int v) { lb_store(state + tile, lb_pack(epoch, flag, v)); }
__device__ __forceinline__ void lb_publish(unsigned long long* state, int tile, unsigned epoch, unsigned flag, Int2 v) {
    lb_store(state + 2 * size_t(tile), lb_pack(epoch, flag, v.a));
    lb_store(state + 2 * size_t(tile) + 1, lb_pack(epoch, flag, v.b));
}
__device__ __forceinline__ unsigned lb_wait(const unsigned long long* state, int t, unsigned epoch, int& v) {
    unsigned long long w;
    do { w = lb_load(state + t); } while ((unsigned)(w >> 34) != epoch || ((w >> 32) & 3u) == 0u);
    v = int(unsigned(w));
    return unsigned(w >> 32) & 3u;
}
__device__ __forceinline__ unsigned lb_wait(const unsigned long long* state, int t, unsigned epoch, Int2& v) {
    int a, b;
    unsigned fa, fb;
    do {
        fa = lb_wait(state, 2 * t, epoch, a);
        fb = lb_wait(state, 2 * t + 1, epoch, b);
    } while (fa != fb);
    v = Int2{a, b};
    return fa;
}
__device__ __forceinline__ bool lb_try(const unsigned long long* state, int t, unsigned epoch, int& v, unsigned& flag) {
    const unsigned long long w = lb_load(state + t);
    v = int(unsigned(w)); flag = unsigned(w >> 32) & 3u;
    return (unsigned)(w >> 34) == epoch && flag != 0u;
}
__device__ __forceinline__ bool lb_try(const unsigned long long* state, int t, unsigned epoch, Int2& v, unsigned& flag) {
    const unsigned long long a = lb_load(state + 2 * size_t(t)), b = lb_load(state + 2 * size_t(t) + 1);
    v = Int2{int(unsigned(a)), int(unsigned(b))}; flag = unsigned(a >> 32) & 3u;
    return (unsigned)(a >> 34) == epoch && (unsigned)(b >> 34) == epoch && flag != 0u && flag == (unsigned(b >> 32) & 3u);
}
template <typename V> constexpr int lb_words() { return int(sizeof(V) / sizeof(int)); }

__device__ __forceinline__ bool lb_aligned16(const void* p) { return (reinterpret_cast<uintptr_t>(p) & 15u) == 0; }
template <typename V, typename In> __device__ __forceinline__ auto lb_load_row(const In& in, int i, int n, V* v, int) -> decltype(in.load4(i, n, v), void()) { in.load4(i, n, v); }
template <typename V, typename In> __device__ __forceinline__ void lb_load_row(const In& in, int i, int n, V* v, long) {
#pragma unroll
    for (int c = 0; c < kLbVec; c++) v[c] = i + c < n ? in(i + c) : zero_of(V());
}
template <typename V, typename Out> __device__ __forceinline__ auto lb_store_row(const Out& out, int i, int n, const V* v, int) -> decltype(out.store4(i, n, v), void()) { out.store4(i, n, v); }
template <typename V, typename Out> __device__ __forceinline__ void lb_store_row(const Out& out, int i, int n, const V* v, long) {
#pragma unroll
    for (int c = 0; c < kLbVec; c++) if (i + c < n) out(i + c, v[c]);
}

template <typename V, typename In, typename Out>
__global__ void __launch_bounds__(kBlock) scan_lookback(In in, Out out, int n, int tiles, unsigned long long* state, unsigned epoch, unsigned help_after, const V* carry_in, V* total_out) {
    __shared__ V lds[kWaves];
    __shared__ V tile_prefix;
    constexpr int kWaveItems = kLbItems * 64, kRows = kLbItems / kLbVec;
    for (int tile = blockIdx.x; tile < tiles; tile += gridDim.x) {
        const int base = tile * kLbTile + wave_id() * kWaveItems + lane_id() * kLbVec;
        V v[kLbItems];
#pragma unroll
        for (int r = 0; r < kRows; r++) lb_load_row<V>(in, base + r * 64 * kLbVec, n, v + r * kLbVec, 0);
        V run = zero_of(V());
#pragma unroll
        for (int r = 0; r < kRows; r++) {
            V mine = zero_of(V());
#pragma unroll
            for (int c = 0; c < kLbVec; c++) { const V x = v[r * kLbVec + c]; v[r * kLbVec + c] = mine; mine = mine + x; }
            const V incl = wave_inclusive_scan(mine);
            const V before = shfl_up_v(incl, 1);
            const V lane_off = lane_id() > 0 ? run + before : run;
#pragma unroll
            for (int c = 0; c < kLbVec; c++) v[r * kLbVec + c] = v[r * kLbVec + c] + lane_off;
            run = run + V(shfl_v(incl, 63));
        }
        __syncthreads();
        if (lane_id() == 0) lds[wave_id()] = run;
        __syncthreads();
        if (wave_id() == 0) {
            V agg = lds[0];
            for (int w = 1; w < kWaves; w++) agg = agg + lds[w];
            V excl = zero_of(V());
            if (tile == 0) {
                if (carry_in) excl = *carry_in;
            } else {
                if (lane_id() == 0) lb_publish(state, tile, epoch, kLbAggregate, agg);
                int p = tile - 1;
                for (;;) {
                    V pv[kLbWindows];
                    unsigned flag[kLbWindows];
                    bool ok[kLbWindows];
#pragma unroll
                    for (int w = 0; w < kLbWindows; w++) {
                        pv[w] = zero_of(V()); flag[w] = kLbPrefix;
                        ok[w] = p - w * 64 - lane_id() < 0;
                    }
                    for (unsigned polls = 0;; polls++) {
                        bool all = true;
#pragma unroll
                        for (int w = 0; w < kLbWindows; w++) {
                            if (!ok[w]) {
                                ok[w] = lb_try(state, p - w * 64 - lane_id(), epoch, pv[w], flag[w]);
                                if (!ok[w] && polls >= help_after) {
                                    const int t = p - w * 64 - lane_id();
                                    const int first = t * kLbTile, last = min(n, first + kLbTile);
                                    V sum = zero_of(V());
                                    for (int i = first; i < last; i++) sum = sum + in(i);
                                    if (t == 0 && carry_in) sum = sum + *carry_in;
                                    pv[w] = sum; flag[w] = t == 0 ? kLbPrefix : kLbAggregate; ok[w] = true;
                                    __builtin_amdgcn_fence(__ATOMIC_ACQUIRE, "agent");
                                    V pub = zero_of(V()); unsigned pflag = 0u;
                                    if (lb_try(state, t, epoch, pub, pflag)) { pv[w] = pub; flag[w] = pflag; }
                                }
                            }
                            all = all && ok[w];
                        }
                        if (all) break;
                    }
                    unsigned long long is_prefix[kLbWindows];
#pragma unroll
                    for (int w = 0; w < kLbWindows; w++) is_prefix[w] = __ballot(flag[w] == kLbPrefix);
                    bool found = false;
#pragma unroll
                    for (int w = 0; w < kLbWindows; w++) {
                        if (found) break;
                        const int first = __ffsll((long long)is_prefix[w]) - 1;
                        if (first < 0 || lane_id() <= first) excl = excl + pv[w];
                        found = first >= 0;
                    }
                    if (found) break;
                    p -= 64 * kLbWindows;
                }
#pragma unroll
                for (int d = 32; d > 0; d >>= 1) excl = excl + V(shfl_xor_v(excl, d));
            }
            if (lane_id() == 0) {
                lb_publish(state, tile, epoch, kLbPrefix, excl + agg);
#if !defined(__gfx950__) && !defined(__gfx942__) && !defined(__gfx90a__) && defined(__HIP_DEVICE_COMPILE__)
#error "scan_lookback: the in-place ordering relies on gfx9's vmcnt counting stores; use a release fence on this target"
#endif
                asm volatile("s_waitcnt vmcnt(0)" ::: "memory");
                tile_prefix = excl;
                if (total_out && tile == tiles - 1) *total_out = excl + agg;
            }
        }
        __syncthreads();
        V offset = tile_prefix;
        for (int w = 0; w < wave_id(); w++) offset = offset + lds[w];
#pragma unroll
        for (int r = 0; r < kRows; r++) {
#pragma unroll
            for (int c = 0; c < kLbVec; c++) v[r * kLbVec + c] = offset + v[r * kLbVec + c];
            lb_store_row<V>(out, base + r * 64 * kLbVec, n, v + r * kLbVec, 0);
        }
    }
    if (tiles == 0 && blockIdx.x == 0 && threadIdx.x == 0 && total_out) *total_out = carry_in ? *carry_in : zero_of(V());
}

inline int scan_num_tiles(int n) { return (n + kScanTile - 1) / kScanTile; }

template <typename V, typename In, typename Out>
inline void device_scan_lookback(hipStream_t stream, int num_cus, In in, Out out, int n, unsigned long long* state, unsigned epoch, unsigned help_after, const V* carry_in, V* total_out) {
    static const int per_cu = [] {
        int n = 0;
        if (hipOccupancyMaxActiveBlocksPerMultiprocessor(&n, scan_lookback<V, In, Out>, kBlock, 0) != hipSuccess) { (void)hipGetLastError(); n = 2; }
        return std::max(1, std::min(n - 1, 8));
    }();
    const int tiles = (n + kLbTile - 1) / kLbTile;
    const int blocks = std::max(1, std::min(tiles, std::max(num_cus, 1) * per_cu));
    scan_lookback<V, In, Out><<<blocks, kBlock, 0, stream>>>(in, out, n, tiles, state, epoch, help_after, carry_in, total_out);
}

template <typename V, typename In, typename Out>
inline void device_scan(hipStream_t stream, In in, Out out, int n, V* partials, const V* carry_in, V* total_out) {
    const int tiles = scan_num_tiles(n);
    if (tiles > 0) scan_partials<V, In><<<tiles, kBlock, 0, stream>>>(in, n, partials);
    scan_spine<V><<<1, kBlock, 0, stream>>>(partials, tiles, carry_in, total_out);
    if (tiles > 0) scan_apply<V, In, Out><<<tiles, kBlock, 0, stream>>>(in, out, n, partials);
}

template <typename V, typename In, typename Out>
inline bool ctx_scan(hagrid_ctx* ctx, In in, Out out, int n, V* partials, const V* carry_in, V* total_out) {
#ifdef HG_SCAN_THREE_KERNELS
    if (!ctx->opt_lookback) { device_scan<V>(ctx->stream, in, out, n, partials, carry_in, total_out); HG_DBG(ctx); return true; }
#endif
    unsigned epoch = 0;
    unsigned long long* state = lookback_state(ctx, scan_num_tiles(n), lb_words<V>(), &epoch);
    if (!state) return false;
    device_scan_lookback<V>(ctx->stream, ctx->num_cus, in, out, n, state, epoch, ctx->opt_lookback == 2 ? 0u : 4096u, carry_in, total_out);
    HG_DBG(ctx);
    return true;
}

}
```

Baseline: 7711.

## Fuse readback publishing into scan/bbox kernels and replace memsets with kernel clears

Measured after the change: 7715 (median of 6 runs). No clear change (+0.0%).

```diff
diff --git a/hagrid_amd/csrc/build.hip b/hagrid_amd/csrc/build.hip
--- a/hagrid_amd/csrc/build.hip
+++ b/hagrid_amd/csrc/build.hip
@@ -55,8 +55,9 @@
         partials[blockIdx.x * 6 + threadIdx.x] = v;
     }
 }
-__global__ void __launch_bounds__(kBlock) bbox_final(const float* __restrict__ partials, int num, float* __restrict__ out) {
+__global__ void __launch_bounds__(kBlock) bbox_final(const float* __restrict__ partials, int num, float* __restrict__ out, int* __restrict__ zero, int nz, Publish pub) {
     __shared__ float lds[kWaves][6];
+    if (int(threadIdx.x) < nz) zero[threadIdx.x] = 0;
     float v[6] = { FLT_MAX, FLT_MAX, FLT_MAX, -FLT_MAX, -FLT_MAX, -FLT_MAX };
     for (int i = threadIdx.x; i < num; i += kBlock)
         for (int c = 0; c < 6; c++) v[c] = c < 3 ? min(v[c], partials[i * 6 + c]) : max(v[c], partials[i * 6 + c]);
@@ -68,6 +69,11 @@
         float r = lds[0][threadIdx.x];
         for (int w = 1; w < kWaves; w++) r = threadIdx.x < 3 ? min(r, lds[w][threadIdx.x]) : max(r, lds[w][threadIdx.x]);
         out[threadIdx.x] = r;
+        if (pub.n) pub.dst[threadIdx.x] = __float_as_int(r);
+    }
+    if (pub.n && threadIdx.x < 64) {
+        __threadfence_system();
+        if (threadIdx.x == 0) __hip_atomic_store(pub.flag, pub.epoch, __ATOMIC_RELEASE, __HIP_MEMORY_SCOPE_SYSTEM);
     }
 }
 
@@ -258,8 +264,10 @@
     }
 };
 
-__global__ void __launch_bounds__(kBlock) top_range_sizes(const float4* __restrict__ tris, int n, BuildK k, int* __restrict__ counts, int* __restrict__ big_list, int* __restrict__ big_count) {
+__global__ void __launch_bounds__(kBlock) top_range_sizes(const float4* __restrict__ tris, int n, BuildK k, int* __restrict__ counts, int* __restrict__ big_list, int* __restrict__ big_count,
+                                                          int* __restrict__ refs_per_cell, int num_top) {
     const int i = blockIdx.x * kBlock + threadIdx.x;
+    for (int c = i; c < num_top; c += gridDim.x * kBlock) refs_per_cell[c] = 0;
     int size = 0;
     if (i < n) { size = max(0, compute_range(k.dims, BBox(k.bmin, k.bmax), load_tri(tris, i).bbox()).size()); counts[i] = size; }
     const bool big = size >= kCoopCells;
@@ -680,15 +688,15 @@
     int* log_dims = ar.get<int>(size_t(num_top));
     int* const partials = nullptr;
     if (!counts || !start_emit || !refs_per_cell || !log_dims) return HAGRID_ENOMEM;
-    HG_HIP(ctx, hipMemsetAsync(refs_per_cell, 0, size_t(num_top) * sizeof(int), st));
     int* big_list = ar.get<int>(size_t(num_tris));
     if (!big_list) return HAGRID_ENOMEM;
-    top_range_sizes<<<grid_blocks(num_tris, kBlock), kBlock, 0, st>>>(tris, num_tris, k, counts, big_list, dsc + 2); HG_DBG(ctx);
-    if (!ctx_scan<int>(ctx, PlainIn{counts}, PlainOut{start_emit}, num_tris, partials, (const int*)nullptr, dsc + 0)) return HAGRID_ENOMEM;
+    top_range_sizes<<<grid_blocks(num_tris, kBlock), kBlock, 0, st>>>(tris, num_tris, k, counts, big_list, dsc + 2, refs_per_cell, num_top); HG_DBG(ctx);
     int R0 = 0, num_big = 0;
     {
         int h[3];
-        HG_TRY(read_back(ctx, dsc, h, sizeof(h)));
+        const Publish pub = publish_arm(ctx, dsc, sizeof(h));
+        if (!ctx_scan<int>(ctx, PlainIn{counts}, PlainOut{start_emit}, num_tris, partials, (const int*)nullptr, dsc + 0, pub)) return HAGRID_ENOMEM;
+        HG_TRY(read_back_armed(ctx, pub, dsc, h, sizeof(h)));
         R0 = h[0]; num_big = h[2];
     }
     if (R0 < 0 || R0 > 0x3fffffff) HG_FAIL(ctx, HAGRID_ERANGE, "build_grid: too many top-level references");
@@ -717,13 +725,12 @@
     emit_top_refs<<<prim_blocks + big_blocks, kBlock, 0, st>>>(tris, num_tris, k, dsc + 1, gb.extents(), start_emit, pair_rank, L.seg_begin, L.refs, log_dims, L.entries, big_list, dsc + 2, prim_blocks); HG_DBG(ctx);
     levels.push_back(L);
 
-    {
-        if (!ctx_scan<int>(ctx, ChildCountIn{L.entries}, UpdateEntriesOut{L.entries}, num_top, (int*)nullptr, (const int*)nullptr, dsc + 8)) return HAGRID_ENOMEM;
-    }
     int num_new_cells = 0, shift = 0;
     {
         int h[8];
-        HG_TRY(read_back(ctx, dsc + 1, h, sizeof(h)));
+        const Publish pub = publish_arm(ctx, dsc + 1, sizeof(h));
+        if (!ctx_scan<int>(ctx, ChildCountIn{L.entries}, UpdateEntriesOut{L.entries}, num_top, (int*)nullptr, (const int*)nullptr, dsc + 8, pub)) return HAGRID_ENOMEM;
+        HG_TRY(read_back_armed(ctx, pub, dsc + 1, h, sizeof(h)));
         shift = h[0]; num_new_cells = h[7];
     }
     if (shift >= 24) HG_FAIL(ctx, HAGRID_ERANGE, "build_grid: too many levels");
@@ -756,12 +763,14 @@
                                                                              tris, P.cells, P.entries, k, masks, P.cell_counts, N.cells, N.cell_counts, N.entries, tot + 1); HG_DBG(ctx);
         }
         Int2* next = reinterpret_cast<Int2*>(tot + 2);
+        int h3[3] = {0, 0, 0};
+        Publish pub;
         if (!last) {
+            pub = publish_arm(ctx, tot + 1, sizeof(h3));
             if (!ctx_scan<Int2>(ctx, ChildSegIn{N.cell_counts, N.entries}, ChildSegOut{N.cell_counts, N.entries, N.seg_begin, N.tile_first}, num_new_cells, (Int2*)nullptr,
-                                (const Int2*)nullptr, next)) return HAGRID_ENOMEM;
-        }
-        int h3[3] = {0, 0, 0};
-        HG_TRY(read_back(ctx, tot + 1, h3, sizeof(h3)));
+                                (const Int2*)nullptr, next, pub)) return HAGRID_ENOMEM;
+        }
+        HG_TRY(read_back_armed(ctx, pub, tot + 1, h3, sizeof(h3)));
         if (level < HAGRID_MAX_LEVELS) { bc.level_refs[level] = P.num_refs; bc.level_cells[level] = P.num_cells; bc.level_kept[level] = h3[0]; bc.num_levels = level + 1; }
         if (last) { ar.drop(masks); break; }
         const int num_children = h3[1];
@@ -787,13 +796,15 @@
     const int total_cells = int(total_cells_ll);
     Int2* const part2 = nullptr;
     Int2* carry = reinterpret_cast<Int2*>(dsc + 128);
+    int hf[2];
+    Publish pub_total;
     for (int l = 0; l < num_levels; l++) {
         GLevel& V = levels[l];
+        if (l == num_levels - 1) pub_total = publish_arm(ctx, carry + l, sizeof(hf));
         if (!ctx_scan<Int2>(ctx, LeafIn{V.entries, V.cell_counts}, LeafOut{V.start_cell, V.ref_begin}, V.num_cells, part2,
-                            l ? carry + (l - 1) : (const Int2*)nullptr, carry + l)) return HAGRID_ENOMEM;
-    }
-    int hf[2];
-    HG_TRY(read_back(ctx, carry + (num_levels - 1), hf, sizeof(hf)));
+                            l ? carry + (l - 1) : (const Int2*)nullptr, carry + l, l == num_levels - 1 ? pub_total : Publish())) return HAGRID_ENOMEM;
+    }
+    HG_TRY(read_back_armed(ctx, pub_total, carry + (num_levels - 1), hf, sizeof(hf)));
     const int new_total_cells = hf[0], total_refs = hf[1];
     if (new_total_cells <= 0 || total_refs < 0) HG_FAIL(ctx, HAGRID_ERANGE, "build_grid: inconsistent totals");
 
@@ -843,16 +854,17 @@
     hipStream_t st = ctx->stream;
     Temps tmp(ctx);
     int* dsc = ctx->dscratch;
-    HG_HIP(ctx, hipMemsetAsync(dsc, 0, 256 * sizeof(int), st));
+    static_assert(kBlock >= 256, "bbox_final clears a word per thread");
 
     const int bb_blocks = std::min(grid_blocks(num_tris, kBlock), 1024);
     float* bb_part = tmp.get<float>(size_t(bb_blocks) * 6 + 8);
     if (!bb_part) return HAGRID_ENOMEM;
     float* bb_out = bb_part + size_t(bb_blocks) * 6;
     bbox_partials<<<bb_blocks, kBlock, 0, st>>>(tris, num_tris, bb_part); HG_DBG(ctx);
-    bbox_final<<<1, kBlock, 0, st>>>(bb_part, bb_blocks, bb_out); HG_DBG(ctx);
     float hb[6];
-    HG_TRY(read_back(ctx, bb_out, hb, sizeof(hb)));
+    const Publish pub_bb = publish_arm(ctx, bb_out, sizeof(hb));
+    bbox_final<<<1, kBlock, 0, st>>>(bb_part, bb_blocks, bb_out, dsc, 256, pub_bb); HG_DBG(ctx);
+    HG_TRY(read_back_armed(ctx, pub_bb, bb_out, hb, sizeof(hb)));
     BBox gb(vec3(hb[0], hb[1], hb[2]), vec3(hb[3], hb[4], hb[5]));
     ivec3 dims = compute_grid_dims(gb, num_tris, top_density);
     dims.x += dims.x & 1; dims.y += dims.y & 1; dims.z += dims.z & 1;
diff --git a/hagrid_amd/csrc/ctx.h b/hagrid_amd/csrc/ctx.h
--- a/hagrid_amd/csrc/ctx.h
+++ b/hagrid_amd/csrc/ctx.h
@@ -206,9 +206,24 @@
 
 int pool_split(hagrid_ctx* ctx, void* base, void* const* parts, int n);
 
-int read_back(hagrid_ctx* ctx, const void* dptr, void* hptr, size_t bytes);
+struct Publish;
+int read_back(hagrid_ctx* ctx, const void* dptr, void* hptr, size_t bytes, const Publish* armed = nullptr);
+
+struct Publish { const int* src = nullptr; int n = 0; int* dst = nullptr; int* flag = nullptr; int epoch = 0; };
+Publish publish_arm(hagrid_ctx* ctx, const void* dptr, size_t bytes);
+void publish_launch(hagrid_ctx* ctx, const Publish& p);
+int read_back_armed(hagrid_ctx* ctx, const Publish& p, const void* dptr, void* hptr, size_t bytes);
+#ifdef __HIPCC__
+__device__ __forceinline__ void publish_by_thread(const Publish& p) {
+    for (int i = 0; i < p.n; i++) p.dst[i] = __hip_atomic_load(p.src + i, __ATOMIC_RELAXED, __HIP_MEMORY_SCOPE_AGENT);
+    __threadfence_system();
+    __hip_atomic_store(p.flag, p.epoch, __ATOMIC_RELEASE, __HIP_MEMORY_SCOPE_SYSTEM);
+}
+#endif
 
 inline int grid_blocks(long long n, int block) { return (int)((n + block - 1) / block); }
+
+void fill_bytes(hagrid_ctx* ctx, void* a, size_t na, int va, void* b = nullptr, size_t nb = 0, int vb = 0);
 
 unsigned long long* lookback_state(hagrid_ctx* ctx, int tiles, int words_per_tile, unsigned* epoch);
 
diff --git a/hagrid_amd/csrc/ctx.hip b/hagrid_amd/csrc/ctx.hip
--- a/hagrid_amd/csrc/ctx.hip
+++ b/hagrid_amd/csrc/ctx.hip
@@ -307,6 +307,30 @@
     return ctx->lb_state;
 }
 
+namespace {
+__device__ __forceinline__ void fill_span(unsigned char* p, size_t n, unsigned v, size_t tid, size_t threads) {
+    const size_t head = std::min(n, size_t((16u - unsigned(reinterpret_cast<uintptr_t>(p) & 15u)) & 15u));
+    const size_t vecs = (n - head) / 16, done = head + vecs * 16;
+    const unsigned w = (v & 0xffu) * 0x01010101u;
+    uint4* q = reinterpret_cast<uint4*>(p + head);
+    for (size_t i = tid; i < vecs; i += threads) q[i] = make_uint4(w, w, w, w);
+    if (tid < head) p[tid] = (unsigned char)v;
+    if (tid < n - done) p[done + tid] = (unsigned char)v;
+}
+__global__ void __launch_bounds__(256) fill_bytes_kernel(unsigned char* a, size_t na, unsigned va, unsigned char* b, size_t nb, unsigned vb) {
+    const size_t tid = size_t(blockIdx.x) * 256 + threadIdx.x, threads = size_t(gridDim.x) * 256;
+    fill_span(a, na, va, tid, threads);
+    if (nb) fill_span(b, nb, vb, tid, threads);
+}
+}
+
+void hagrid_impl::fill_bytes(hagrid_ctx* ctx, void* a, size_t na, int va, void* b, size_t nb, int vb) {
+    if (!na && !nb) return;
+    const int blocks = int(std::min<size_t>(std::max<size_t>((std::max(na, nb) / 16 + 255) / 256, 1), 4096));
+    fill_bytes_kernel<<<blocks, 256, 0, ctx->stream>>>(static_cast<unsigned char*>(a), na, unsigned(va), static_cast<unsigned char*>(b), nb, unsigned(vb));
+    HG_DBG(ctx);
+}
+
 void hagrid_impl::debug_sync(hagrid_ctx* ctx, const char* file, int line) {
     hipError_t e = hipStreamSynchronize(ctx->stream);
     if (e == hipSuccess) e = hipGetLastError();
@@ -333,11 +357,29 @@
 }
 }
 
-int hagrid_impl::read_back(hagrid_ctx* ctx, const void* dptr, void* hptr, size_t bytes) {
+hagrid_impl::Publish hagrid_impl::publish_arm(hagrid_ctx* ctx, const void* dptr, size_t bytes) {
+    Publish p;
     if (ctx->opt_fast_readback && bytes > 0 && bytes <= 256 * sizeof(int) && (bytes & 3u) == 0 && (reinterpret_cast<uintptr_t>(dptr) & 3u) == 0) {
-        int* flag = ctx->mailbox + kMbxReadBackEpoch;
-        const int epoch = ++ctx->readback_epoch;
-        publish_words<<<1, 256, 0, ctx->stream>>>(static_cast<const int*>(dptr), int(bytes / 4), ctx->mailbox, flag, epoch);
+        p.src = static_cast<const int*>(dptr); p.n = int(bytes / 4); p.dst = ctx->mailbox; p.flag = ctx->mailbox + kMbxReadBackEpoch; p.epoch = ++ctx->readback_epoch;
+    }
+    return p;
+}
+void hagrid_impl::publish_launch(hagrid_ctx* ctx, const Publish& p) {
+    if (p.n) publish_words<<<1, 256, 0, ctx->stream>>>(p.src, p.n, p.dst, p.flag, p.epoch);
+}
+
+int hagrid_impl::read_back_armed(hagrid_ctx* ctx, const Publish& p, const void* dptr, void* hptr, size_t bytes) {
+    if (!p.n) return read_back(ctx, dptr, hptr, bytes);
+    return read_back(ctx, dptr, hptr, bytes, &p);
+}
+
+int hagrid_impl::read_back(hagrid_ctx* ctx, const void* dptr, void* hptr, size_t bytes, const Publish* armed) {
+    Publish p;
+    if (armed) p = *armed;
+    else { p = publish_arm(ctx, dptr, bytes); publish_launch(ctx, p); }
+    if (p.n) {
+        int* flag = p.flag;
+        const int epoch = p.epoch;
         HG_HIP(ctx, hipGetLastError());
         const auto t0 = std::chrono::steady_clock::now();
         for (unsigned spins = 0;; spins++) {
diff --git a/hagrid_amd/csrc/expand.hip b/hagrid_amd/csrc/expand.hip
--- a/hagrid_amd/csrc/expand.hip
+++ b/hagrid_amd/csrc/expand.hip
@@ -53,8 +53,11 @@
     return Tri(vec3(a.x, a.y, a.z), a.w, vec3(b.x, b.y, b.z), b.w, vec3(c.x, c.y, c.z), c.w);
 }
 
-__global__ void __launch_bounds__(kBlock) fill_voxel_cells(ExpandK k, const Entry* __restrict__ entries, int* __restrict__ voxel_cells, int voxels) {
+__global__ void __launch_bounds__(kBlock) fill_voxel_cells(ExpandK k, const Entry* __restrict__ entries, int* __restrict__ voxel_cells, int voxels,
+                                                           unsigned char* __restrict__ flags, int num_cells, int* __restrict__ counts, int num_counts) {
     const int v = blockIdx.x * kBlock + threadIdx.x;
+    for (int i = v; i < num_cells; i += gridDim.x * kBlock) flags[i] = 0xFF;
+    if (v < num_counts) counts[v] = 0;
     if (v >= voxels) return;
     const int s = k.shift, m = (1 << s) - 1, top = v >> (3 * s), local = v & ((1 << (3 * s)) - 1);
     const int tx = top % k.top.x, ty = (top / k.top.x) % k.top.y, tz = top / (k.top.x * k.top.y);
@@ -253,7 +256,6 @@
     Cell* other = pool_alloc<Cell>(ctx, size_t(n));
     unsigned char* flags = pool_alloc<unsigned char>(ctx, size_t(n));
     if (!other || !flags) { hagrid_mem_free(ctx, other); hagrid_mem_free(ctx, flags); return HAGRID_ENOMEM; }
-    (void)hipMemsetAsync(flags, 0xFF, size_t(n), st);
     const Entry* entries = static_cast<const Entry*>(grid->entries);
     const int* refs = static_cast<const int*>(grid->ref_ids);
     const int blocks = grid_blocks(n, kBlock);
@@ -261,10 +263,12 @@
     const long long voxels = (long long)k.dims.x * k.dims.y * k.dims.z;
     int* voxel_cells = (ctx->opt_expand_voxel_map && voxels <= (1ll << 28)) ? pool_try_alloc<int>(ctx, size_t(voxels)) : nullptr;
     k.voxel_cells = voxel_cells;
-    if (voxel_cells) { ExpandK kf = k; kf.voxel_cells = nullptr; fill_voxel_cells<<<grid_blocks(voxels, kBlock), kBlock, 0, st>>>(kf, entries, voxel_cells, int(voxels)); HG_DBG(ctx); }
     int* counts = ctx->dscratch + 160;
     const int max_listed = 48;
-    if (list) (void)hipMemsetAsync(counts, 0, max_listed * sizeof(int), st);
+    if (voxel_cells) {
+        ExpandK kf = k; kf.voxel_cells = nullptr;
+        fill_voxel_cells<<<grid_blocks(std::max<long long>(voxels, max_listed), kBlock), kBlock, 0, st>>>(kf, entries, voxel_cells, int(voxels), flags, n, counts, list ? max_listed : 0); HG_DBG(ctx);
+    } else fill_bytes(ctx, flags, size_t(n), 0xFF, counts, list ? max_listed * sizeof(int) : 0, 0);
     int listed = 0;
     for (int it = 0; it < iters; it++) {
         if (it > 0 && list && listed + 3 <= max_listed) {
diff --git a/hagrid_amd/csrc/flatten.hip b/hagrid_amd/csrc/flatten.hip
--- a/hagrid_amd/csrc/flatten.hip
+++ b/hagrid_amd/csrc/flatten.hip
@@ -10,8 +10,9 @@
 
 constexpr int kFlatLevels = 3;
 
-__global__ void __launch_bounds__(kBlock) collapse_and_depth(uint32_t* __restrict__ entries, int* __restrict__ depths, int first, int num) {
+__global__ void __launch_bounds__(kBlock) collapse_and_depth(uint32_t* __restrict__ entries, int* __restrict__ depths, int first, int num, int* __restrict__ word, int value) {
     const int id = blockIdx.x * kBlock + threadIdx.x;
+    if (word && id == 0) *word = value;
     if (id >= num) return;
     uint32_t e = entries[first + id];
     int d = 0;
@@ -93,20 +94,22 @@
     auto release = [&]() { hagrid_mem_free(ctx, depths); hagrid_mem_free(ctx, start); hagrid_mem_free(ctx, partials); };
     if (!depths || !start || !partials) { release(); return HAGRID_ENOMEM; }
 
+    int* carry = ctx->dscratch;
+    const int top_entries = grid->offsets[0];
     for (int i = shift; i >= 0; i--) {
         const int first = first_of(i), num = grid->offsets[i] - first;
-        if (num > 0) collapse_and_depth<<<grid_blocks(num, kBlock), kBlock, 0, st>>>(entries, depths, first, num);
+        if (num > 0 || i == 0) collapse_and_depth<<<std::max(grid_blocks(num, kBlock), 1), kBlock, 0, st>>>(entries, depths, first, num, i == 0 ? carry : nullptr, top_entries);
     }
-    int* carry = ctx->dscratch;
-    const int top_entries = grid->offsets[0];
-    HG_HIP(ctx, hipMemcpyAsync(carry, &top_entries, sizeof(int), hipMemcpyHostToDevice, st));
     int groups = 0;
+    const int num_groups = (shift + kFlatLevels - 1) / kFlatLevels;
+    Publish pub;
     for (int i = 0; i < shift; i += kFlatLevels, groups++) {
         const int first = first_of(i), num = grid->offsets[i] - first;
-        if (!ctx_scan<int>(ctx, BlockSizeIn{depths + first}, StartOut{start + first}, num, partials, carry + groups, carry + groups + 1)) { release(); return HAGRID_ENOMEM; }
+        if (groups == num_groups - 1) pub = publish_arm(ctx, carry, sizeof(int) * size_t(num_groups + 1));
+        if (!ctx_scan<int>(ctx, BlockSizeIn{depths + first}, StartOut{start + first}, num, partials, carry + groups, carry + groups + 1, pub)) { release(); return HAGRID_ENOMEM; }
     }
     int h[HAGRID_MAX_LEVELS + 2];
-    int rc = read_back(ctx, carry, h, sizeof(int) * size_t(groups + 1));
+    int rc = read_back_armed(ctx, pub, carry, h, sizeof(int) * size_t(groups + 1));
     if (rc != HAGRID_OK) { release(); return rc; }
     const int total_entries = h[groups];
     if (total_entries < top_entries || total_entries > 0x3fffffff) { release(); HG_FAIL(ctx, HAGRID_ERANGE, "flatten_grid: voxel map too large"); }
diff --git a/hagrid_amd/csrc/merge.hip b/hagrid_amd/csrc/merge.hip
--- a/hagrid_amd/csrc/merge.hip
+++ b/hagrid_amd/csrc/merge.hip
@@ -587,7 +587,7 @@
     int rc = HAGRID_OK;
     int prev_num_cells = 0, iter = 0, pass_tag = 0;
     bool in_narrow = false;
-    (void)hipMemsetAsync(prevs, 0, nc0, st);
+    fill_bytes(ctx, prevs, nc0, 0);
     hagrid_build_counts& bc = ctx->counts;
     auto record = [&](int c, int r) {
         if (bc.merge_passes < HAGRID_MAX_MERGE_PASSES) { bc.merge_cells[bc.merge_passes] = c; bc.merge_refs[bc.merge_passes] = r; bc.merge_passes++; }
@@ -648,7 +648,7 @@
             Int2* tot = total + axis;
             const int* n_dev = axis > first_axis ? &total[axis - 1].a : nullptr;
             const Entry* ent = reinterpret_cast<const Entry*>(entries);
-            if (++pass_tag == 256) { pass_tag = 1; (void)hipMemsetAsync(prevs, 0, nc0, st); }
+            if (++pass_tag == 256) { pass_tag = 1; fill_bytes(ctx, prevs, nc0, 0); }
             if (in_narrow) merge_counts_kernel<true><<<blocks, kBlock, 0, st>>>(axis, k, ent, cells, refs, merge_counts, nexts, prevs, pass_tag, mask, num_cells, n_dev);
             else           merge_counts_kernel<false><<<blocks, kBlock, 0, st>>>(axis, k, ent, cells, refs, merge_counts, nexts, prevs, pass_tag, mask, num_cells, n_dev);
             HG_DBG(ctx);
@@ -690,14 +690,14 @@
         }
         int first_compacting_axis = 0;
         if (in_place) {
-            if (prev_mask & ~mask) (void)hipMemsetAsync(dirty, 1, 3 * ip_dstride, st);
+            if (prev_mask & ~mask) fill_bytes(ctx, dirty, 3 * ip_dstride, 1);
             const int blocks = grid_blocks(ip_slots, kIpTile), tiles = blocks;
             const Entry* ent = reinterpret_cast<const Entry*>(entries);
             for (int axis = 0; axis < 3 && rc == HAGRID_OK; axis++) {
                 global_pass++;
                 if (++pass_tag == 256) {
                     pass_tag = 1;
-                    (void)hipMemsetAsync(prevs, 0, nc0, st); (void)hipMemsetAsync(evaluated, 0, size_t(ip_slots), st); (void)hipMemsetAsync(cell_flags, 0, size_t(ip_slots), st);
+                    fill_bytes(ctx, prevs, nc0, 0); fill_bytes(ctx, evaluated, size_t(ip_slots), 0, cell_flags, size_t(ip_slots), 0);
                 }
                 ip_counts<<<blocks, kBlock, 0, st>>>(axis, k, ent, cells, list_end, refs, ip_slots, dirty + size_t(axis) * ip_dstride, minfo, nexts, evaluated, prevs, pass_tag, mask); HG_DBG(ctx);
                 ip_chains<<<blocks, kBlock, 0, st>>>(ip_slots, nexts, evaluated, prevs, cell_flags, pass_tag); HG_DBG(ctx);
diff --git a/hagrid_amd/csrc/wave_prims.h b/hagrid_amd/csrc/wave_prims.h
--- a/hagrid_amd/csrc/wave_prims.h
+++ b/hagrid_amd/csrc/wave_prims.h
@@ -232,7 +232,7 @@
 }
 
 template <typename V, typename In, typename Out>
-__global__ void __launch_bounds__(kBlock) scan_lookback(In in, Out out, int n, int tiles, unsigned long long* state, unsigned epoch, unsigned help_after, const V* carry_in, V* total_out) {
+__global__ void __launch_bounds__(kBlock) scan_lookback(In in, Out out, int n, int tiles, unsigned long long* state, unsigned epoch, unsigned help_after, const V* carry_in, V* total_out, Publish pub) {
     __shared__ V lds[kWaves];
     __shared__ V tile_prefix;
     constexpr int kWaveItems = kLbItems * 64, kRows = kLbItems / kLbVec;
@@ -333,14 +333,19 @@
             for (int c = 0; c < kLbVec; c++) v[r * kLbVec + c] = offset + v[r * kLbVec + c];
             lb_store_row<V>(out, base + r * 64 * kLbVec, n, v + r * kLbVec, 0);
         }
-    }
-    if (tiles == 0 && blockIdx.x == 0 && threadIdx.x == 0 && total_out) *total_out = carry_in ? *carry_in : zero_of(V());
+        if (pub.n && tile == tiles - 1 && threadIdx.x == 0) publish_by_thread(pub);
+    }
+    if (tiles == 0 && blockIdx.x == 0 && threadIdx.x == 0) {
+        if (total_out) *total_out = carry_in ? *carry_in : zero_of(V());
+        if (pub.n) publish_by_thread(pub);
+    }
 }
 
 inline int scan_num_tiles(int n) { return (n + kScanTile - 1) / kScanTile; }
 
 template <typename V, typename In, typename Out>
-inline void device_scan_lookback(hipStream_t stream, int num_cus, In in, Out out, int n, unsigned long long* state, unsigned epoch, unsigned help_after, const V* carry_in, V* total_out) {
+inline void device_scan_lookback(hipStream_t stream, int num_cus, In in, Out out, int n, unsigned long long* state, unsigned epoch, unsigned help_after, const V* carry_in, V* total_out,
+                                 const Publish& pub = Publish()) {
     static const int per_cu = [] {
         int n = 0;
         if (hipOccupancyMaxActiveBlocksPerMultiprocessor(&n, scan_lookback<V, In, Out>, kBlock, 0) != hipSuccess) { (void)hipGetLastError(); n = 2; }
@@ -348,7 +353,7 @@
     }();
     const int tiles = (n + kLbTile - 1) / kLbTile;
     const int blocks = std::max(1, std::min(tiles, std::max(num_cus, 1) * per_cu));
-    scan_lookback<V, In, Out><<<blocks, kBlock, 0, stream>>>(in, out, n, tiles, state, epoch, help_after, carry_in, total_out);
+    scan_lookback<V, In, Out><<<blocks, kBlock, 0, stream>>>(in, out, n, tiles, state, epoch, help_after, carry_in, total_out, pub);
 }
 
 template <typename V, typename In, typename Out>
@@ -360,14 +365,14 @@
 }
 
 template <typename V, typename In, typename Out>
-inline bool ctx_scan(hagrid_ctx* ctx, In in, Out out, int n, V* partials, const V* carry_in, V* total_out) {
+inline bool ctx_scan(hagrid_ctx* ctx, In in, Out out, int n, V* partials, const V* carry_in, V* total_out, const Publish& pub = Publish()) {
 #ifdef HG_SCAN_THREE_KERNELS
-    if (!ctx->opt_lookback) { device_scan<V>(ctx->stream, in, out, n, partials, carry_in, total_out); HG_DBG(ctx); return true; }
+    if (!ctx->opt_lookback) { device_scan<V>(ctx->stream, in, out, n, partials, carry_in, total_out); publish_launch(ctx, pub); HG_DBG(ctx); return true; }
 #endif
     unsigned epoch = 0;
     unsigned long long* state = lookback_state(ctx, scan_num_tiles(n), lb_words<V>(), &epoch);
     if (!state) return false;
-    device_scan_lookback<V>(ctx->stream, ctx->num_cus, in, out, n, state, epoch, ctx->opt_lookback == 2 ? 0u : 4096u, carry_in, total_out);
+    device_scan_lookback<V>(ctx->stream, ctx->num_cus, in, out, n, state, epoch, ctx->opt_lookback == 2 ? 0u : 4096u, carry_in, total_out, pub);
     HG_DBG(ctx);
     return true;
 }
```
